# ChicyChen/LOCO-Edit

Measured on AMD Instinct MI355X. Metric: edit-directions/sec (top-5 PMP-Jacobian SVD @256^2) + vT cos-sim vs ref, higher is better.
Workload: dtype bf16x3 (split-bf16 MFMA operands, fp32 accumulate + fp32 storage); 1 GPU; CelebA-HQ DDPM 256x256 top-5 local basis (l_eye-sized mask, L=2400), t=0.6T, 12 power iterations, one GPU; multi_gpu_form=single, probes_total=5, probes_per_gpu=5, kept=5, n_iter=12, mask_L=2400, weights=synthetic seed 0, streams=2

## Files before the change

loco-edit_amd/csrc/conv_bf16.hip:

```cpp
#include "kernels.h"
#include <cstdio>
#include <cstdlib>

namespace loco {

enum : int { PR_BF16X3 = 0, PR_F16 = 1 };
template <int PR, int TAPS, int MODE> void launch_tile_b(const ConvArgs& a, hipStream_t st);
template <int PR, int MODE> void launch_kcat_b(const ConvArgs& a, hipStream_t st);
template <int PR, int MODE> void launch_pair_b(const ConvArgs& a, hipStream_t st);
template <int PR, int MODE> void launch_dual_b(const ConvArgs& a, hipStream_t st);
void launch_conv_gemm(const ConvArgs& a, hipStream_t st);

template <int PR>
static void launch_lowp(const ConvArgs& a, int taps, hipStream_t st) {
#ifdef LOCO_DIAG
    if (a.cot_d && (taps != 1 || a.gemm || a.nsplit > 1 || a.Cin2 > 0 || (a.Cout % conv_bf16_tile_couts(a)) != 0 || a.st_kind == ST_TAN || a.st_kind == ST_COT)) {
        fprintf(stderr, "loco: ConvArgs::cot_d on a launch whose epilogue has no norm-cotangent term (taps %d, gemm %d, nsplit %d, Cout %d, st_kind %d)\n",
                taps, a.gemm, a.nsplit, a.Cout, a.st_kind);
        abort();
    }
#endif
    if constexpr (PR == PR_BF16X3) {
        if (taps == 1 && a.gemm) { launch_conv_gemm(a, st); return; }
    }
    if (taps == 9 && a.Cin2 > 0) {
        if (a.mode == CM_GN_SILU) launch_kcat_b<PR, CM_GN_SILU>(a, st);
        else if (a.mode == CM_GN_GELU) launch_kcat_b<PR, CM_GN_GELU>(a, st);
        else launch_kcat_b<PR, CM_TAN_SILU>(a, st);
        return;
    }
#ifdef LOCO_DIAG
    if constexpr (PR == PR_BF16X3) {
        if (taps == 9 && a.dual) {
            switch (a.mode) {
                case CM_NONE: launch_dual_b<PR, CM_NONE>(a, st); break;
                case CM_GN_SILU: launch_dual_b<PR, CM_GN_SILU>(a, st); break;
                case CM_TAN_SILU: launch_dual_b<PR, CM_TAN_SILU>(a, st); break;
                default: launch_dual_b<PR, CM_COT_SILU>(a, st); break;
            }
            return;
        }
    }
#endif
    if constexpr (PR == PR_BF16X3) {
        if (taps == 9 && a.pair) {
            switch (a.mode) {
                case CM_NONE: launch_pair_b<PR, CM_NONE>(a, st); break;
                case CM_GN_SILU: launch_pair_b<PR, CM_GN_SILU>(a, st); break;
                case CM_TAN_SILU: launch_pair_b<PR, CM_TAN_SILU>(a, st); break;
                default: launch_pair_b<PR, CM_COT_SILU>(a, st); break;
            }
            return;
        }
    }
    if (taps == 9) {
        switch (a.mode) {
            case CM_NONE: launch_tile_b<PR, 9, CM_NONE>(a, st); break;
            case CM_GN_SILU: launch_tile_b<PR, 9, CM_GN_SILU>(a, st); break;
            case CM_GN_GELU: launch_tile_b<PR, 9, CM_GN_GELU>(a, st); break;
            case CM_TAN_SILU: launch_tile_b<PR, 9, CM_TAN_SILU>(a, st); break;
            case CM_COT_SILU: launch_tile_b<PR, 9, CM_COT_SILU>(a, st); break;
            default: launch_tile_b<PR, 9, CM_GN>(a, st); break;
        }
    } else {
        switch (a.mode) {
            case CM_NONE: launch_tile_b<PR, 1, CM_NONE>(a, st); break;
            default: launch_tile_b<PR, 1, CM_GN>(a, st); break;
        }
    }
}
void launch_conv_bf16x3(const ConvArgs& a, int taps, hipStream_t st) { launch_lowp<PR_BF16X3>(a, taps, st); }
void launch_conv_f16(const ConvArgs& a, int taps, hipStream_t st) { launch_lowp<PR_F16>(a, taps, st); }

}
```

loco-edit_amd/csrc/conv_bf16_kernel.h:

```cpp
#pragma once
#include "kernels.h"
#include <cstdlib>
#include <type_traits>

namespace loco {


typedef float f32x16 __attribute__((ext_vector_type(16)));
typedef float f32x4 __attribute__((ext_vector_type(4)));
typedef f32x4 f32x4_u __attribute__((aligned(4)));
typedef float f32x2 __attribute__((ext_vector_type(2)));
typedef f32x2 f32x2_u __attribute__((aligned(4)));
typedef __bf16 bf16x8 __attribute__((ext_vector_type(8)));
typedef _Float16 f16x8 __attribute__((ext_vector_type(8)));
typedef short s16x8 __attribute__((ext_vector_type(8)));

enum : int { PR_BF16X3 = 0, PR_F16 = 1 };

constexpr int BKC = 16;
constexpr bool LIVE_MASK = true;
constexpr bool EARLY_W = true;
constexpr int NDUMMY = 8;

__device__ __forceinline__ float sigmoidf2_(float y) { return __builtin_amdgcn_rcpf(1.0f + __expf(-y)); }

__device__ __forceinline__ int idiv_small(int n, int d) {
    int q = (int)((float)n * __builtin_amdgcn_rcpf((float)d));
    const int r = n - q * d;
    q += (r >= d) ? 1 : ((r < 0) ? -1 : 0);
    return q;
}
__device__ __forceinline__ void idivmod_small(int n, int d, int& q, int& r) { q = idiv_small(n, d); r = n - q * d; }

template <int PR>
__device__ __forceinline__ int rec_off(int p, int q) {
    if constexpr (PR == PR_F16) return p * 32 + ((q ^ ((p >> 3) & 1)) << 4);
    else return p * 64 + ((q ^ ((p >> 2) & 3)) << 4);
}
template <int PR> constexpr int halo_pitch() { return PR == PR_F16 ? 48 : 80; }
template <int PR> constexpr int rec_bytes() { return PR == PR_F16 ? 32 : 64; }
template <int PR>
__device__ __forceinline__ int hrec_off(int p, int q) { return p * halo_pitch<PR>() + (q << 4); }

template <int PR>
__device__ __forceinline__ void cvt2(float a, float b, unsigned& hi, unsigned& lo) {
    if constexpr (PR == PR_F16) {
        _Float16 ha = (_Float16)a, hb = (_Float16)b;
        hi = (unsigned)__builtin_bit_cast(unsigned short, ha) | ((unsigned)__builtin_bit_cast(unsigned short, hb) << 16);
        lo = 0;
    } else {
        typedef float f32x2_ __attribute__((ext_vector_type(2)));
        typedef __bf16 bf16x2_ __attribute__((ext_vector_type(2)));
        hi = __builtin_bit_cast(unsigned, __builtin_convertvector((f32x2_){a, b}, bf16x2_));
        const float ha = __builtin_bit_cast(float, hi << 16), hb = __builtin_bit_cast(float, hi & 0xffff0000u);
        float da = a - ha;
        asm volatile("" : "+v"(da));
        const float db = b - hb;
        lo = __builtin_bit_cast(unsigned, __builtin_convertvector((f32x2_){da, db}, bf16x2_));
    }
}

template <int PR>
__device__ __forceinline__ void split8(const float* v, uint4& hi, uint4& lo) {
    cvt2<PR>(v[0], v[1], hi.x, lo.x);
    cvt2<PR>(v[2], v[3], hi.y, lo.y);
    cvt2<PR>(v[4], v[5], hi.z, lo.z);
    cvt2<PR>(v[6], v[7], hi.w, lo.w);
}

constexpr int max_halo(int NT, int taps, bool s2) {
    if (taps == 1) return NT;
    if (NT >= 128) {
        int th = NT / 32;
        return s2 ? (2 * th + 1) * 65 : (th + 2) * 34;
    }
    return s2 ? 5 * 65 : 4 * 34;
}

constexpr int rs_steps(int n, int lw) { int s = 0; while ((1 << s) < lw && (n >> s) > 1) ++s; return s; }
template <int N, int M, int LW>
__device__ __forceinline__ void rs_reduce(float* av, const int lane) {
    if constexpr (M < LW && N > 1) {
        constexpr int H = N / 2;
        const bool up = (lane & M) != 0;
#pragma unroll
        for (int i = 0; i < H; ++i) {
            const float keep = up ? av[i + H] : av[i];
            const float send = up ? av[i] : av[i + H];
            av[i] = keep + __shfl_xor(send, M, 64);
        }
        rs_reduce<H, M * 2, LW>(av, lane);
    } else if constexpr (M < LW) {
#pragma unroll
        for (int i = 0; i < N; ++i) av[i] += __shfl_xor(av[i], M, 64);
        rs_reduce<N, M * 2, LW>(av, lane);
    }
}

constexpr int EPI_COT1 = 1, EPI_STATS = 2;
template <int WM, int WN, int TM, int TN, int EPI = EPI_STATS, class StageRound>
__device__ __forceinline__ void conv_lowp_epilogue_staged(const ConvArgs& a, StageRound&& stage_round, unsigned char* smem_b, const int co0,
                                                          const int oy0, const int ox0, const int TW, const int tile_id, const int b,
                                                          const int split);
template <int WM, int WN, int TM, int TN>
__device__ __forceinline__ void conv_lowp_epilogue_direct(const ConvArgs& a, f32x16 (&acc)[TM][TN], const int co0, const int oy0,
                                                          const int ox0, const int TW, const int b, const int split);
template <int WM, int WN, int TM, int TN, int EPI = EPI_STATS>
__device__ __forceinline__ void conv_lowp_epilogue(const ConvArgs& a, f32x16 (&acc)[TM][TN], unsigned char* smem_b, const int co0,
                                                   const int oy0, const int ox0, const int TW, const int tile_id, const int b,
                                                   const int split) {
    constexpr int NT = WN * TN * 32;
    const int lane = threadIdx.x & 63, wave = threadIdx.x >> 6;
    const int l31 = lane & 31, khalf = lane >> 5, wm = wave / WN, wn = wave % WN;
    if (co0 + WM * TM * 32 <= a.Cout) {
        conv_lowp_epilogue_staged<WM, WN, TM, TN, EPI>(a, [&](const int h, float* S) {
#pragma unroll
            for (int j = 0; j < TN; ++j)
#pragma unroll
                for (int r = 0; r < 16; ++r)
                    S[(wm * 32 + (r & 3) + 8 * (r >> 2) + 4 * khalf) * NT + (wn * TN + j) * 32 + l31] = acc[h][j][r];
        }, smem_b, co0, oy0, ox0, TW, tile_id, b, split);
        return;
    }
    conv_lowp_epilogue_direct<WM, WN, TM, TN>(a, acc, co0, oy0, ox0, TW, b, split);
}
template <int WM, int WN, int TM, int TN, int EPI, class StageRound>
__device__ __forceinline__ void conv_lowp_epilogue_staged(const ConvArgs& a, StageRound&& stage_round, unsigned char* smem_b, const int co0,
                                                          const int oy0, const int ox0, const int TW, const int tile_id, const int b,
                                                          const int split) {
    constexpr int NTHR = WM * WN * 64;
    constexpr bool COT1 = (EPI & EPI_COT1) != 0, STATS = (EPI & EPI_STATS) != 0;
    constexpr int MT = WM * TM * 32;
    constexpr int NT = WN * TN * 32;
    const int tid = threadIdx.x;
    const int lane = tid & 63;
    const int wave = tid >> 6;
    const int l31 = lane & 31;
    const int khalf = lane >> 5;
    const int wm = wave / WN, wn = wave % WN;
    const long out_plane = (long)a.Hout * a.Wout;
    {
        constexpr int SROWS = WM * 32, NQ = NT / 4, NTASK = (SROWS * NQ) / NTHR;
        static_assert((SROWS * NQ) % NTHR == 0 && (NQ & (NQ - 1)) == 0, "epilogue task split");
        float* const S = reinterpret_cast<float*>(smem_b);
        const bool part = a.nsplit > 1;
        float* const ob = part ? a.partial + (((long)split * a.B + b) * a.Cout) * out_plane : a.out + (long)b * a.out_bs;
        const float* const rb = (!part && a.res) ? a.res + (long)b * a.res_bs : nullptr;
        const float* const b2 = (!part && a.bias2) ? a.bias2 + (long)b * a.bias2_bs : nullptr;
        const float* const b1 = part ? nullptr : a.bias;
        const bool accu = !part && a.accumulate;
        const int twsh = 31 - __builtin_clz((unsigned)TW);
        const bool lin_st = STATS && (a.st_kind == ST_TAN || a.st_kind == ST_COT) && !part;
        const bool lin_cot = a.st_kind == ST_COT;
        const bool cot_ep = COT1 && a.cot_d && !part && !lin_st;
        const float* const cot_db = cot_ep ? a.cot_d + (long)b * a.cot_d_bs : nullptr;
        const f32x2* const cot_tb = cot_ep ? reinterpret_cast<const f32x2*>(a.cot_tc + (long)b * a.cot_tc_bs) : nullptr;
        constexpr int RSTEP = NTHR / NQ;
        static_assert(NTHR % NQ == 0 && 32 % RSTEP == 0, "epilogue task rows");
        const int row0 = tid / NQ, quad0 = tid & (NQ - 1);
        const unsigned pix0 = (unsigned)((oy0 + ((quad0 * 4) >> twsh)) * a.Wout + ox0 + ((quad0 * 4) & (TW - 1)));
        auto co_of = [&](int h, int q) -> int { return co0 + row0 + (((q * RSTEP) >> 5) * TM + h) * 32 + ((q * RSTEP) & 31); };
        auto off_of = [&](int h, int q) -> unsigned {
            const unsigned crow = (unsigned)((((q * RSTEP) >> 5) * TM + h) * 32 + ((q * RSTEP) & 31));
            return (unsigned)(co0 + row0) * (unsigned)out_plane + pix0 + crow * (unsigned)out_plane;
        };
        constexpr int NV = 2 * TM * NTASK;
        float av[STATS ? NV : 1];
#pragma unroll
        for (int h = 0; h < TM; ++h) {
            if (h > 0) {
                asm volatile("s_waitcnt lgkmcnt(0)" ::: "memory");
                __builtin_amdgcn_s_barrier();
            }
            stage_round(h, S);
            f32x4 xs[(STATS || COT1) ? NTASK : 1][2];
            f32x4 cd[COT1 ? NTASK : 1];
            if constexpr (COT1) {
                if (cot_ep) {
#pragma unroll
                    for (int q = 0; q < NTASK; ++q) {
                        const unsigned o = off_of(h, q);
                        cd[q] = *reinterpret_cast<const f32x4*>(cot_db + o);
                        const f32x4* sp4 = reinterpret_cast<const f32x4*>(a.cot_sx + o);
                        xs[q][0] = sp4[0];
                        xs[q][1] = sp4[1];
                    }
                }
            }
            if constexpr (STATS) if (lin_st) {
#pragma unroll
                for (int q = 0; q < NTASK; ++q) {
                    const unsigned o = off_of(h, q);
                    if (lin_cot) {
                        const f32x4* sp4 = reinterpret_cast<const f32x4*>(a.st_sx + o);
                        xs[q][0] = sp4[0];
                        xs[q][1] = sp4[1];
                    } else {
                        xs[q][0] = *reinterpret_cast<const f32x4*>(a.st_x + o);
                    }
                }
            }
            asm volatile("s_waitcnt lgkmcnt(0)" ::: "memory");
            __builtin_amdgcn_s_barrier();
            f32x4 v[NTASK], rv[NTASK];
#pragma unroll
            for (int q = 0; q < NTASK; ++q) v[q] = *reinterpret_cast<const f32x4*>(&S[(q * RSTEP + row0) * NT + quad0 * 4]);
            if (rb || accu) {
#pragma unroll
                for (int q = 0; q < NTASK; ++q) {
                    f32x4 t4 = {0.f, 0.f, 0.f, 0.f};
                    if (rb) t4 = a.res_scale * *reinterpret_cast<const f32x4*>(rb + off_of(h, q));
                    if (accu) t4 += *reinterpret_cast<const f32x4*>(ob + off_of(h, q));
                    rv[q] = t4;
                }
#pragma unroll
                for (int q = 0; q < NTASK; ++q) v[q] += rv[q];
            }
            if constexpr (COT1) {
                if (cot_ep) {
#pragma unroll
                    for (int q = 0; q < NTASK; ++q) {
                        const f32x2 tc2 = cot_tb[co_of(h, q)];
                        const float c1 = tc2[0], c2 = tc2[1];
                        v[q][0] += fmaf(xs[q][0][0], cd[q][0], -fmaf(xs[q][0][1], c2, c1));
                        v[q][1] += fmaf(xs[q][0][2], cd[q][1], -fmaf(xs[q][0][3], c2, c1));
                        v[q][2] += fmaf(xs[q][1][0], cd[q][2], -fmaf(xs[q][1][1], c2, c1));
                        v[q][3] += fmaf(xs[q][1][2], cd[q][3], -fmaf(xs[q][1][3], c2, c1));
                    }
                }
            }
#pragma unroll
            for (int q = 0; q < NTASK; ++q) {
                float add = 0.f;
                if (b1) add += b1[co_of(h, q)];
                if (b2) add += b2[co_of(h, q)];
                v[q] += add;
                __builtin_nontemporal_store(v[q], reinterpret_cast<f32x4*>(ob + off_of(h, q)));
            }
            if constexpr (STATS) if (lin_st) {
#pragma unroll
                for (int q = 0; q < NTASK; ++q) {
                    const f32x4 vv = v[q];
                    float s1, s2;
                    if (!lin_cot) {
                        const f32x4 xv = xs[q][0];
                        s1 = (vv[0] + vv[1]) + (vv[2] + vv[3]);
                        s2 = fmaf(xv[0], vv[0], xv[1] * vv[1]) + fmaf(xv[2], vv[2], xv[3] * vv[3]);
                    } else {
                        const float z0 = xs[q][0][0] * vv[0], z1 = xs[q][0][2] * vv[1], z2 = xs[q][1][0] * vv[2], z3 = xs[q][1][2] * vv[3];
                        s1 = (z0 + z1) + (z2 + z3);
                        s2 = fmaf(xs[q][0][1], z0, xs[q][0][3] * z1) + fmaf(xs[q][1][1], z2, xs[q][1][3] * z3);
                    }
                    av[(h * NTASK + q) * 2] = s1;
                    av[(h * NTASK + q) * 2 + 1] = s2;
                }
            }
            if (STATS && a.st_kind == ST_FWD && !part) {
                const int ntile = (a.Hout * a.Wout) / NT;
                float* const sp = a.st_part + (long)b * a.Cout * ntile * 2;
#pragma unroll
                for (int q = 0; q < NTASK; ++q) {
                    const float pivot = __shfl(v[q][0], lane & ~(NQ - 1) & 63, 64);
                    const float d0 = v[q][0] - pivot, d1 = v[q][1] - pivot, d2 = v[q][2] - pivot, d3 = v[q][3] - pivot;
                    float s1 = (d0 + d1) + (d2 + d3);
                    float s2 = (d0 * d0 + d1 * d1) + (d2 * d2 + d3 * d3);
#pragma unroll
                    for (int m = 1; m < (NQ < 64 ? NQ : 64); m <<= 1) {
                        s1 += __shfl_xor(s1, m, 64);
                        s2 += __shfl_xor(s2, m, 64);
                    }
                    const float m = s1 * (1.0f / NT);
                    const int t = q * NTHR + tid;
                    if ((t & (NQ - 1)) == 0)
                        *reinterpret_cast<f32x2*>(sp + ((long)co_of(h, q) * ntile + tile_id) * 2) = f32x2{pivot + m, s2 - s1 * m};
                }
            }
        }
        if constexpr (STATS) if (lin_st) {
            constexpr int LW = NQ < 64 ? NQ : 64, STEPS = rs_steps(NV, LW), LEFT = NV >> STEPS;
            static_assert((NV & (NV - 1)) == 0, "row sums per lane");
            rs_reduce<NV, 1, LW>(av, lane);
            const int gl = lane & (LW - 1);
            if (gl < (1 << STEPS)) {
                int base = 0;
#pragma unroll
                for (int sb = 0; sb < STEPS; ++sb) base += ((gl >> sb) & 1) * (NV >> (sb + 1));
                const int ntile = (a.Hout * a.Wout) / NT;
                float* const sp = a.st_part + (long)b * a.Cout * ntile * 2;
#pragma unroll
                for (int i = 0; i < LEFT; ++i) {
                    const int idx = base + i, hq = idx >> 1;
                    const int h = hq / NTASK, q = hq - h * NTASK;
                    const int row = (q * NTHR + tid) / NQ;
                    const int co = co0 + ((row >> 5) * TM + h) * 32 + (row & 31);
                    sp[((long)co * ntile + tile_id) * 2 + (idx & 1)] = av[i];
                }
            }
        }
    }
}
template <int WM, int WN, int TM, int TN>
__device__ __forceinline__ void conv_lowp_epilogue_direct(const ConvArgs& a, f32x16 (&acc)[TM][TN], const int co0, const int oy0,
                                                          const int ox0, const int TW, const int b, const int split) {
    const int lane = threadIdx.x & 63, wave = threadIdx.x >> 6;
    const int l31 = lane & 31, khalf = lane >> 5, wm = wave / WN, wn = wave % WN;
    const long out_plane = (long)a.Hout * a.Wout;
    const bool full_co = false;
#pragma unroll
    for (int j = 0; j < TN; ++j) {
        int p = (wn * TN + j) * 32 + l31;
        int ty = p / TW, tx = p - ty * TW;
        int oy = oy0 + ty, ox = ox0 + tx;
        const unsigned pix = (unsigned)(oy * a.Wout + ox);
#pragma unroll
        for (int i = 0; i < TM; ++i) {
            const int cob = co0 + (wm * TM + i) * 32 + 4 * khalf;
            if (a.nsplit > 1) {
                float* pb = a.partial + (((long)split * a.B + b) * a.Cout) * out_plane;
#pragma unroll
                for (int r = 0; r < 16; ++r) {
// ... 55 lines not shown
    const float* const rb = a.res ? a.res + (long)b * a.res_bs : nullptr;
    const float* const b2 = a.bias2 ? a.bias2 + (long)b * a.bias2_bs : nullptr;
    const bool accu = a.accumulate != 0;
    const int twsh = TW == 32 ? 5 : (TW == 16 ? 4 : 3);
    const int ntile = (a.Hout * a.Wout) / NT;
    float* const sp = (a.st_kind == ST_FWD) ? a.st_part + (long)b * a.Cout * ntile * 2 : nullptr;
#pragma unroll
    for (int h = 0; h < TM; ++h) {
#pragma unroll
        for (int g0 = 0; g0 < 4; g0 += NRB) {
#pragma unroll
            for (int j = 0; j < TN; ++j)
#pragma unroll
                for (int g = 0; g < NRB; ++g)
#pragma unroll
                    for (int r3 = 0; r3 < 4; ++r3)
                        S[(wm * RPW + g * 8 + 4 * khalf + r3) * NT + (wn * TN + j) * 32 + l31] = acc[h][j][(g0 + g) * 4 + r3];
            asm volatile("s_waitcnt lgkmcnt(0)" ::: "memory");
            __builtin_amdgcn_s_barrier();
            f32x4 v[NTASK];
            unsigned off[NTASK];
            int cos_[NTASK];
#pragma unroll
            for (int q = 0; q < NTASK; ++q) {
                const int t = q * NTHR + tid;
                const int srow = t / NQ, quad = t & (NQ - 1);
                v[q] = *reinterpret_cast<const f32x4*>(&S[srow * NT + quad * 4]);
                const int co = co0 + ((srow / RPW) * TM + h) * 32 + g0 * 8 + (srow % RPW);
                const int p = quad * 4;
                cos_[q] = co;
                off[q] = (unsigned)co * out_plane + (unsigned)((oy0 + (p >> twsh)) * a.Wout + ox0 + (p & (TW - 1)));
            }
            if (rb || accu) {
                f32x4 rv[NTASK];
#pragma unroll
                for (int q = 0; q < NTASK; ++q) {
                    f32x4 t4 = {0.f, 0.f, 0.f, 0.f};
                    if (rb) t4 = a.res_scale * *reinterpret_cast<const f32x4*>(rb + off[q]);
                    if (accu) t4 += *reinterpret_cast<const f32x4*>(ob + off[q]);
                    rv[q] = t4;
                }
#pragma unroll
                for (int q = 0; q < NTASK; ++q) v[q] += rv[q];
            }
#pragma unroll
            for (int q = 0; q < NTASK; ++q) {
                float add = 0.f;
                if (a.bias) add += a.bias[cos_[q]];
                if (b2) add += b2[cos_[q]];
                v[q] += add;
                __builtin_nontemporal_store(v[q], reinterpret_cast<f32x4*>(ob + off[q]));
            }
            if (sp) {
#pragma unroll
                for (int q = 0; q < NTASK; ++q) {
                    const float pivot = __shfl(v[q][0], 0, 64);
                    const float d0 = v[q][0] - pivot, d1 = v[q][1] - pivot, d2 = v[q][2] - pivot, d3 = v[q][3] - pivot;
                    float s1 = (d0 + d1) + (d2 + d3);
                    float s2 = (d0 * d0 + d1 * d1) + (d2 * d2 + d3 * d3);
#pragma unroll
                    for (int m = 1; m < 64; m <<= 1) {
                        s1 += __shfl_xor(s1, m, 64);
                        s2 += __shfl_xor(s2, m, 64);
                    }
                    const float m = s1 * (1.0f / NT);
                    if (lane == 0)
                        *reinterpret_cast<f32x2*>(sp + ((long)cos_[q] * ntile + tile_id) * 2) = f32x2{pivot + m, s2 - s1 * m};
                }
            }
            asm volatile("s_waitcnt lgkmcnt(0)" ::: "memory");
            __builtin_amdgcn_s_barrier();
        }
    }
}

template <int PR, int TAPS, int WM, int WN, int TM, int TN, int MODE, int STG, int PHASE = 0>
__device__ __forceinline__ void conv_lowp_body(const ConvArgs& a, f32x16 (&acc)[TM][TN]) {
    constexpr int NTHR = WM * WN * 64;
    constexpr int HP = halo_pitch<PR>();
    constexpr int RB = rec_bytes<PR>();
    constexpr int NPC = RB / 16;
    constexpr int MT = WM * TM * 32;
    constexpr int NT = WN * TN * 32;
    constexpr int KS = (TAPS == 9) ? 3 : 1;
    constexpr int NTS = KS;
    constexpr int NROW = (TAPS == 9) ? 3 : 1;
    constexpr bool NEEDP = (MODE == CM_TAN_SILU || MODE == CM_COT_SILU);
    constexpr bool PERS = (PHASE == 3);
    constexpr bool GEN = (STG == 1 || STG == 2);
    constexpr bool COMPACT = (STG == 3);
    constexpr int NITEM = GEN ? (2 * max_halo(NT, TAPS, STG == 2) + NTHR - 1) / NTHR : 1;
    constexpr int WTOT = NTS * MT * NPC;
    constexpr int NWV = (WTOT + NTHR - 1) / NTHR;
    constexpr bool XPF = (TAPS == 9 && STG != 2 && STG != 3);
    constexpr int NWB = XPF ? 3 : 2;
    constexpr bool DEEP1 = (TAPS == 1 && STG == 1 && !NEEDP);
    constexpr int DEEP_D = 4;

    extern __shared__ __attribute__((aligned(16))) unsigned char smem_b[];
#ifdef LOCO_DUAL_STAMP
#define LP_STAMP(i) do { if (threadIdx.x == 0 && PHASE == 0) reinterpret_cast<unsigned long long*>(a.partial)[blockIdx.x * 8 + (i)] = __builtin_amdgcn_s_memtime(); } while (0)
#else
#define LP_STAMP(i) do { } while (0)
#endif
    LP_STAMP(0);
    constexpr int WBYTES = NTS * MT * RB;
    unsigned char* const Wsb = smem_b;
    unsigned char* Hsb;
    unsigned char* Ws = smem_b;
    unsigned char* Hs = smem_b;

    const int tid = threadIdx.x;
    const int lane = tid & 63;
    const int wave = tid >> 6;
    const int l31 = lane & 31;
    const int khalf = lane >> 5;
    const int wm = wave / WN, wn = wave % WN;

    const int S = a.stride;
    const int TW = (TAPS == 1 && PHASE == 0 && a.stride == 1 && !a.upsample && !a.zins && (a.Wout & (a.Wout - 1)) == 0)
                       ? (a.Wout < NT ? a.Wout : NT) : (a.Wout < 32 ? a.Wout : 32);
    const int TH = NT / TW;
    const int tiles_x = a.Wout / TW;
    int tile_id, cot_id, zid;
    {
        const int ntile = (a.Hout * a.Wout) / NT, ncot = (a.Cout + MT - 1) / MT, Z = PERS ? a.pers_groups : a.B * a.nsplit;
        const int NTC = ntile * ncot, L = blockIdx.x;
        int T = 0;
        if ((ntile & 7) == 0) {
            int q = L >> 3, q2, t8;
            idivmod_small(q, ncot, q2, cot_id);
            idivmod_small(q2, Z, t8, zid);
            tile_id = t8 * 8 + (L & 7);
        } else {
            if ((NTC & 7) == 0) { int q = L >> 3, t8; idivmod_small(q, Z, t8, zid); T = t8 * 8 + (L & 7); }
            else idivmod_small(L, Z, T, zid);
            idivmod_small(T, ntile, cot_id, tile_id);
        }
        tile_id = __builtin_amdgcn_readfirstlane(tile_id);
        cot_id = __builtin_amdgcn_readfirstlane(cot_id);
        zid = __builtin_amdgcn_readfirstlane(zid);
    }
    int ty0_, tx0_;
    idivmod_small(tile_id, tiles_x, ty0_, tx0_);
    const int oy0 = __builtin_amdgcn_readfirstlane(ty0_ * TH);
    const int ox0 = __builtin_amdgcn_readfirstlane(tx0_ * TW);
    const int co0 = cot_id * MT;
    int zb_, zs_;
    idivmod_small(zid, a.nsplit, zb_, zs_);
    const int b = PERS ? zid : __builtin_amdgcn_readfirstlane(zb_);
    const int split = PERS ? 0 : __builtin_amdgcn_readfirstlane(zs_);
    const int pstep = PERS ? a.pers_groups : 1;
    const int np = PERS ? (a.B - b + pstep - 1) / pstep : 1;
    int pq = 0;

    if constexpr (XPF && PHASE != 2 && EARLY_W) {
        const int nchunks_ = (a.Cin + BKC - 1) / BKC;
        const int cps_ = __builtin_amdgcn_readfirstlane((nchunks_ + a.nsplit - 1) / a.nsplit);
        const int cbeg_ = split * cps_;
        const int cend_ = (cbeg_ + cps_ < nchunks_) ? cbeg_ + cps_ : nchunks_;
        if (cend_ > cbeg_) {
            typedef __attribute__((address_space(3))) unsigned char lds_u8_;
            typedef const __attribute__((address_space(1))) unsigned char glb_u8_;
            const int wpitch_ = (a.Cout + 31) & ~31;
            const unsigned char* wbase0 = reinterpret_cast<const unsigned char*>(a.wb) +
                                          (unsigned)(cbeg_ * TAPS) * ((unsigned)wpitch_ * (unsigned)RB);
#pragma unroll
            for (int st_ = 0; st_ < 2; ++st_)
#pragma unroll
                for (int i = 0; i < NWV; ++i) {
                    int e = tid + i * NTHR;
                    if (e >= WTOT) e = WTOT - 1;
                    const int tap = e / (MT * NPC), rem = e - tap * (MT * NPC);
                    int rec = co0 + rem / NPC;
                    if (rec >= wpitch_) rec = wpitch_ - 1;
                    const unsigned rel = (unsigned)(((st_ * NTS + tap) * wpitch_ + rec) * NPC + (rem % NPC)) * 16u;
                    const int e0 = wave * 64 + i * NTHR;
                    if ((WTOT % NTHR) == 0 || e0 < WTOT)
                        __builtin_amdgcn_global_load_lds((glb_u8_*)(wbase0 + rel), (lds_u8_*)(smem_b + st_ * WBYTES + e0 * 16), 16, 0, 0);
                }
        }
    }
    const int halo_w = (TW - 1) * S + KS;
    const int halo_h = (TH - 1) * S + KS;
    const int halo_sz = halo_h * halo_w;
    const int HBYTES = COMPACT ? halo_sz * HP + RB : (halo_sz + NDUMMY) * HP;
    Hsb = smem_b + NWB * WBYTES;

    const int LH = (a.upsample || a.zins) ? a.Hin * 2 : a.Hin;
    const int LW = (a.upsample || a.zins) ? a.Win * 2 : a.Win;
    const long in_plane = (long)a.Hin * a.Win;

    int ipos[NITEM], ioct[NITEM];
    unsigned ivoff[NITEM];
    bool ival[NITEM];
#pragma unroll
    for (int i = 0; i < NITEM; ++i) {
        int it = tid + i * NTHR;
        int oct, pos;
        idivmod_small(it, halo_sz, oct, pos);
        int off = -1;
        if (it < 2 * halo_sz) {
            int hy, hx;
            idivmod_small(pos, halo_w, hy, hx);
            int Y = oy0 * S - a.pad + hy, X = ox0 * S - a.pad + hx;
            if (Y >= 0 && Y < LH && X >= 0 && X < LW) {
                if (a.upsample) off = (Y >> 1) * a.Win + (X >> 1);
                else if (a.zins) off = ((Y | X) & 1) ? -1 : (Y >> 1) * a.Win + (X >> 1);
                else off = Y * a.Win + X;
            }
        } else {
            pos = -1; oct = 0;
        }
        ipos[i] = pos; ioct[i] = oct;
        ival[i] = off >= 0;
        ivoff[i] = (unsigned)(oct * 8 * (int)in_plane + (off >= 0 ? off : 0));
    }

    const int nseg = (halo_w + 3) >> 2;
    int v_q4 = 0, v_pos0 = -1, v_voff = 0, v_cnt = 0;
    unsigned v_pm = 0;
    int v_rec[4] = {0, 0, 0, 0};
    unsigned v_goff = 0;
    if constexpr (!GEN) {
        const int per_q = halo_h * nseg;
        const int nsg4 = (nseg + 3) >> 2, nhy2 = (halo_h + 1) >> 1;
        bool have = false;
        int hy = 0, sg = 0;
        if (32 * nsg4 * nhy2 <= NTHR) {
            const int hi = tid >> 5;
            v_q4 = (tid >> 3) & 3;
            int hq_, hr_;
            idivmod_small(hi, nsg4, hq_, hr_);
            sg = hr_ * 4 + (tid & 3);
            hy = hq_ * 2 + ((tid >> 2) & 1);
            have = hi < nsg4 * nhy2 && sg < nseg && hy < halo_h;
            if (!have) v_q4 = 0;
        } else if (tid < 4 * per_q) {
            int rem;
            idivmod_small(tid, per_q, v_q4, rem);
            idivmod_small(rem, nseg, hy, sg);
            have = true;
        }
        if (have) {
            int Y = oy0 - a.pad + hy, X0 = ox0 - a.pad + 4 * sg;
            bool rowok = (Y >= 0 && Y < a.Hin);
            v_pos0 = hy * halo_w + 4 * sg;
            v_cnt = halo_w - 4 * sg < 4 ? halo_w - 4 * sg : 4;
            v_voff = rowok ? Y * a.Win + X0 : 0;
#pragma unroll
            for (int pxi = 0; pxi < 4; ++pxi)
                if (rowok && X0 + pxi >= 0 && X0 + pxi < a.Win && pxi < v_cnt) v_pm |= 1u << pxi;
        }
#pragma unroll
        for (int pxi = 0; pxi < 4; ++pxi)
            v_rec[pxi] = (v_pos0 >= 0 && pxi < v_cnt) ? v_pos0 + pxi : (COMPACT ? halo_sz : halo_sz + (tid & (NDUMMY - 1)));
        v_goff = (unsigned)(((long)v_q4 * 4 * in_plane + v_voff + 16) * 4);
    }

    int hoff[TN];
#pragma unroll
    for (int j = 0; j < TN; ++j) {
        int p = (wn * TN + j) * 32 + l31;
        int ty, tx;
        idivmod_small(p, TW, ty, tx);
        hoff[j] = ty * S * halo_w + tx * S;
    }
    int hbyte[TN];
#pragma unroll
    for (int j = 0; j < TN; ++j) hbyte[j] = hrec_off<PR>(hoff[j], khalf);
    int aoff_hi[TM], aoff_lo[TM];
#pragma unroll
    for (int i = 0; i < TM; ++i) {
        int p = (wm * TM + i) * 32 + l31;
        aoff_hi[i] = rec_off<PR>(p, khalf);
        aoff_lo[i] = PR == PR_F16 ? 0 : rec_off<PR>(p, 2 + khalf);
    }

    if constexpr (PHASE != 2) {
#pragma unroll
        for (int i = 0; i < TM; ++i)
#pragma unroll
            for (int j = 0; j < TN; ++j)
#pragma unroll
                for (int r = 0; r < 16; ++r) acc[i][j][r] = 0.0f;
    }

    const int nchunks = (a.Cin + BKC - 1) / BKC;
    const int cps = __builtin_amdgcn_readfirstlane((nchunks + a.nsplit - 1) / a.nsplit);
    const int cbeg = split * cps;
    const int cend = (cbeg + cps < nchunks) ? cbeg + cps : nchunks;

    const float* inb = a.in + (long)b * a.in_bs;
    const float2* sxb = NEEDP ? a.sx : nullptr;
    const float* scb = (MODE == CM_GN_SILU || MODE == CM_GN || MODE == CM_GN_GELU) ? a.sc + (long)b * a.scsh_bs : nullptr;
    const float* shb = (MODE == CM_GN_SILU || MODE == CM_GN || MODE == CM_GN_GELU) ? a.sh + (long)b * a.scsh_bs : nullptr;
    const int wpitch = (a.Cout + 31) & ~31;
    const uint4* wg = reinterpret_cast<const uint4*>(a.wb);

    float hv[NITEM][8];
    float2 pv[NEEDP ? NITEM : 1][8];
    float cA[(MODE == CM_NONE) ? 1 : 16], cB[(MODE == CM_NONE) ? 1 : 16];
    const float* tcb = NEEDP ? a.tc + (long)b * a.tc_bs : nullptr;

    constexpr int NPART = (!GEN && NROW == 3) ? 2 : 1;
    constexpr int KP = 4 / NPART;
    struct HaloRegs {
        f32x4 dq[GEN ? 1 : KP];
        f32x4 sq[(!GEN && NEEDP) ? KP : 1][2];
        f32x4 cq[(!GEN && MODE != CM_NONE) ? (KP == 4 ? 2 : 1) : 1];
    };
    auto cq_a = [&](const HaloRegs& R, int kk) -> float {
        if constexpr (GEN || MODE == CM_NONE) return 0.f;
        else if constexpr (NEEDP) { if constexpr (KP == 4) return R.cq[kk >> 1][(kk & 1) * 2]; else return R.cq[0][kk * 2]; }
        else return R.cq[0][kk];
    };
    auto cq_b = [&](const HaloRegs& R, int kk) -> float {
        if constexpr (GEN || MODE == CM_NONE) return 0.f;
        else if constexpr (NEEDP) { if constexpr (KP == 4) return R.cq[kk >> 1][(kk & 1) * 2 + 1]; else return R.cq[0][kk * 2 + 1]; }
        else if constexpr (KP == 4) return R.cq[1][kk];
        else return R.cq[0][2 + kk];
    };
    HaloRegs hr;
    bool pf_live = true, dma_live = true;
    int pf_dq = 0;
#ifdef LOCO_DUAL_STAMP
    const bool wi_halo = (a.no_deep & 2) != 0, wi_dma = (a.no_deep & 4) != 0, wi_novalu = (a.no_deep & 8) != 0;
#endif
    auto prefetch_hv = [&](HaloRegs& R, int chunk, int part) {
        const unsigned cb = (unsigned)chunk * ((unsigned)(BKC * 4) * (unsigned)in_plane);
        const long pofs = PERS ? (long)(pq + pf_dq) * pstep : 0;
        const char* pk = reinterpret_cast<const char*>(inb + pofs * a.in_bs - 16) + cb;
        const char* sk = reinterpret_cast<const char*>(reinterpret_cast<const float*>(sxb) - 32) + 2u * cb;
        const unsigned pl = (unsigned)in_plane * 4u;
#pragma unroll
        for (int kk = 0; kk < KP; ++kk) {
#ifdef LOCO_DUAL_STAMP
            const unsigned po = (pf_live && !wi_halo) ? v_goff + (unsigned)(part * KP + kk) * pl : 64u;
#else
            const unsigned po = pf_live ? v_goff + (unsigned)(part * KP + kk) * pl : 64u;
#endif
            R.dq[kk] = *reinterpret_cast<const f32x4_u*>(pk + po);
            if constexpr (NEEDP) {
                R.sq[kk][0] = *reinterpret_cast<const f32x4_u*>(sk + 2u * po);
                R.sq[kk][1] = *reinterpret_cast<const f32x4_u*>(sk + 2u * po + 16);
            }
        }
        const int c0 = chunk * BKC + v_q4 * 4 + part * KP;
        if constexpr (MODE != CM_NONE) {
            if constexpr (NEEDP) {
                const float* tq = tcb + pofs * a.tc_bs;
                R.cq[0] = *reinterpret_cast<const f32x4_u*>(tq + 2 * c0);
                if constexpr (KP == 4) R.cq[1] = *reinterpret_cast<const f32x4_u*>(tq + 2 * c0 + 4);
            } else if constexpr (KP == 4) {
                R.cq[0] = *reinterpret_cast<const f32x4_u*>(scb + pofs * a.scsh_bs + c0);
                R.cq[1] = *reinterpret_cast<const f32x4_u*>(shb + pofs * a.scsh_bs + c0);
            } else {
                const float* sq_ = scb + pofs * a.scsh_bs;
                const float* hq_ = shb + pofs * a.scsh_bs;
                const f32x2 sa = *reinterpret_cast<const f32x2_u*>(sq_ + c0), sb = *reinterpret_cast<const f32x2_u*>(hq_ + c0);
                R.cq[0] = f32x4{sa[0], sa[1], sb[0], sb[1]};
            }
        }
    };
    auto stage_hv = [&](const HaloRegs& R, int part) {
#ifdef LOCO_DUAL_STAMP
        if (wi_novalu) return;
#endif
        const int oct = v_q4 >> 1, half = v_q4 & 1;
#pragma unroll
        for (int pxi = 0; pxi < 4; ++pxi) {
            float r[KP];
#pragma unroll
            for (int kk = 0; kk < KP; ++kk) {
                float d = R.dq[kk][pxi];
                float v = d;
                if constexpr (MODE == CM_GN_SILU) {
                    float y = fmaf(cq_a(R, kk), d, cq_b(R, kk));
                    v = y * sigmoidf2_(y);
                } else if constexpr (MODE == CM_GN_GELU) {
                    v = act_fwd(fmaf(cq_a(R, kk), d, cq_b(R, kk)), ACT_GELU);
                } else if constexpr (MODE == CM_GN) {
                    v = fmaf(cq_a(R, kk), d, cq_b(R, kk));
                } else if constexpr (NEEDP) {
                    const float Sv = R.sq[kk][pxi >> 1][(pxi & 1) * 2], xh = R.sq[kk][pxi >> 1][(pxi & 1) * 2 + 1];
                    if constexpr (MODE == CM_TAN_SILU) v = Sv * fmaf(-xh, cq_b(R, kk), d - cq_a(R, kk));
                    else v = fmaf(-xh, cq_b(R, kk), fmaf(Sv, d, -cq_a(R, kk)));
                }
                r[kk] = ((v_pm >> pxi) & 1u) ? v : 0.0f;
            }
            unsigned char* dst = Hs + hrec_off<PR>(v_rec[pxi], oct) + half * 8 + part * (KP * 2);
            if constexpr (KP == 4) {
                uint2 h, l;
                cvt2<PR>(r[0], r[1], h.x, l.x);
                cvt2<PR>(r[2], r[3], h.y, l.y);
                *reinterpret_cast<uint2*>(dst) = h;
                if constexpr (PR == PR_BF16X3) *reinterpret_cast<uint2*>(dst + 32) = l;
            } else {
                unsigned h, l;
                cvt2<PR>(r[0], r[1], h, l);
                *reinterpret_cast<unsigned*>(dst) = h;
                if constexpr (PR == PR_BF16X3) *reinterpret_cast<unsigned*>(dst + 32) = l;
            }
        }
    };
    auto load_consts = [&](int chunk) {
        const int c0 = chunk * BKC;
        if constexpr (MODE != CM_NONE) {
#pragma unroll
            for (int kk = 0; kk < 16; ++kk) {
                int c = c0 + kk < a.Cin ? c0 + kk : a.Cin - 1;
                if constexpr (NEEDP) { cA[kk] = tcb[2 * c]; cB[kk] = tcb[2 * c + 1]; }
                else { cA[kk] = scb[c]; cB[kk] = shb[c]; }
            }
        }
    };
    auto load_regs = [&](float (&hvd)[NITEM][8], int chunk) {
        const int c0 = chunk * BKC;
        if (c0 + BKC <= a.Cin) {
            if constexpr (TAPS == 9 && !NEEDP) {
                const unsigned lm = pf_live ? 0xffffffffu : 0u;
                const long pb4 = in_plane * 4;
                const unsigned char* pk = reinterpret_cast<const unsigned char*>(inb) + (long)c0 * pb4;
#pragma unroll
                for (int k = 0; k < 8; ++k) {
#pragma unroll
                    for (int i = 0; i < NITEM; ++i) hvd[i][k] = *reinterpret_cast<const float*>(pk + ((ivoff[i] * 4u) & lm));
                    pk += pb4;
                }
            } else {
#pragma unroll
            for (int k = 0; k < 8; ++k) {
                const float* pk = inb + (long)(c0 + k) * in_plane;
                const float2* sk = NEEDP ? sxb + (long)(c0 + k) * in_plane : nullptr;
#pragma unroll
                for (int i = 0; i < NITEM; ++i) {
                    hvd[i][k] = pk[pf_live ? ivoff[i] : 0u];
                    if constexpr (NEEDP) pv[i][k] = sk[pf_live ? ivoff[i] : 0u];
                }
            }
            }
        } else {
#pragma unroll
            for (int i = 0; i < NITEM; ++i) {
#pragma unroll
                for (int k = 0; k < 8; ++k) {
                    int c = c0 + ioct[i] * 8 + k;
                    int cc = c < a.Cin ? c : a.Cin - 1;
                    unsigned vo = ivoff[i] - (unsigned)(ioct[i] * 8 * (int)in_plane);
                    float v = inb[(long)cc * in_plane + vo];
                    hvd[i][k] = c < a.Cin ? v : 0.0f;
                    if constexpr (NEEDP) {
                        float2 pp = sxb[(long)cc * in_plane + vo];
                        pv[i][k] = c < a.Cin ? pp : make_float2(0.f, 0.f);
                    }
                }
            }
        }
    };
    auto prefetch_h = [&](int chunk, int part) {
        if constexpr (!GEN) { prefetch_hv(hr, chunk, part); return; }
        load_consts(chunk);
        load_regs(hv, chunk);
    };
    unsigned wrel[NWV];
#pragma unroll
    for (int i = 0; i < NWV; ++i) {
        int e = tid + i * NTHR;
        if (e >= WTOT) e = WTOT - 1;
        int tap = e / (MT * NPC), rem = e - tap * (MT * NPC);
        int rec = co0 + rem / NPC;
        if (rec >= wpitch) rec = wpitch - 1;
        wrel[i] = (unsigned)((tap * wpitch + rec) * NPC + (rem % NPC)) * 16u;
    }
    typedef __attribute__((address_space(3))) unsigned char lds_u8;
    typedef const __attribute__((address_space(1))) unsigned char glb_u8;
    auto dma_w = [&](int chunk, int row, unsigned char* Wdst) {
        const unsigned char* wbase = reinterpret_cast<const unsigned char*>(wg) +
                                     (unsigned)(chunk * TAPS + row * NTS) * ((unsigned)wpitch * (unsigned)RB);
#pragma unroll
        for (int i = 0; i < NWV; ++i) {
            const int e0 = (wave * 64 + i * NTHR);
            if ((WTOT % NTHR) == 0 || e0 < WTOT)
#ifdef LOCO_DUAL_STAMP
                __builtin_amdgcn_global_load_lds((glb_u8*)(wbase + ((dma_live && !wi_dma) ? wrel[i] : 0u)), (lds_u8*)(Wdst + e0 * 16), 16, 0, 0);
#else
                __builtin_amdgcn_global_load_lds((glb_u8*)(wbase + (dma_live ? wrel[i] : 0u)), (lds_u8*)(Wdst + e0 * 16), 16, 0, 0);
#endif
        }
    };
    auto stage_regs = [&](const float (&hvs)[NITEM][8], int chunk, unsigned char* Hd, auto whole_tag) {
        constexpr bool WHOLE = decltype(whole_tag)::value;
        const int c0 = chunk * BKC;
#pragma unroll
        for (int i = 0; i < NITEM; ++i) {
            if (ipos[i] < 0) continue;
            float v[8];
#pragma unroll
            for (int k = 0; k < 8; ++k) {
                int c = c0 + ioct[i] * 8 + k;
                float r = 0.0f;
                if (ival[i] && (WHOLE || c < a.Cin)) {
                    float d = hvs[i][k];
                    if constexpr (MODE == CM_NONE) {
                        r = d;
                    } else {
                        const float ca = ioct[i] ? cA[8 + k] : cA[k];
                        const float cb = ioct[i] ? cB[8 + k] : cB[k];
                        if constexpr (MODE == CM_GN_SILU) {
                            float y = fmaf(ca, d, cb);
                            r = y * sigmoidf2_(y);
                        } else if constexpr (MODE == CM_GN_GELU) {
                            r = act_fwd(fmaf(ca, d, cb), ACT_GELU);
                        } else if constexpr (MODE == CM_GN) {
                            r = fmaf(ca, d, cb);
                        } else {
                            float Sv = pv[i][k].x, xh = pv[i][k].y;
                            if constexpr (MODE == CM_TAN_SILU) r = Sv * fmaf(-xh, cb, d - ca);
                            else r = fmaf(-xh, cb, fmaf(Sv, d, -ca));
                        }
                    }
                }
                v[k] = r;
            }
            uint4 hi, lo;
            split8<PR>(v, hi, lo);
            *reinterpret_cast<uint4*>(Hd + hrec_off<PR>(ipos[i], ioct[i])) = hi;
            if constexpr (PR == PR_BF16X3) *reinterpret_cast<uint4*>(Hd + hrec_off<PR>(ipos[i], 2 + ioct[i])) = lo;
        }
    };
    auto stage_h = [&](int chunk, int part) {
        if constexpr (!GEN) { stage_hv(hr, part); return; }
        stage_regs(hv, chunk, Hs, std::false_type{});
    };

    constexpr int NLO = PR == PR_BF16X3 ? 1 : 0;
    struct Frag { s16x8 ah[TM], al[NLO ? TM : 1], bh[TN], bl[NLO ? TN : 1]; };
    auto load_frag = [&](Frag& f, int row, int tp) {
        const int tapoff = (TAPS == 9) ? row * halo_w + tp : 0;
#pragma unroll
        for (int i = 0; i < TM; ++i) {
            f.ah[i] = *reinterpret_cast<const s16x8*>(Ws + tp * MT * RB + aoff_hi[i]);
#if defined(LOCO_WI_NOLO)
            if constexpr (NLO) f.al[i] = f.ah[i];
#else
            if constexpr (NLO) f.al[i] = *reinterpret_cast<const s16x8*>(Ws + tp * MT * RB + aoff_lo[i]);
#endif
        }
#pragma unroll
        for (int j = 0; j < TN; ++j) {
            const unsigned char* hp = Hs + tapoff * HP + hbyte[j];
            f.bh[j] = *reinterpret_cast<const s16x8*>(hp);
#if defined(LOCO_WI_NOLO)
            if constexpr (NLO) f.bl[j] = f.bh[j];
#else
            if constexpr (NLO) f.bl[j] = *reinterpret_cast<const s16x8*>(hp + 32);
#endif
        }
    };
    auto mma_frag = [&](const Frag& f) {
#pragma unroll
        for (int i = 0; i < TM; ++i)
#pragma unroll
            for (int j = 0; j < TN; ++j) {
                if constexpr (PR == PR_F16) {
                    acc[i][j] = __builtin_amdgcn_mfma_f32_32x32x16_f16(__builtin_bit_cast(f16x8, f.ah[i]),
                                                                       __builtin_bit_cast(f16x8, f.bh[j]), acc[i][j], 0, 0, 0);
                } else {
                    const bf16x8 ah = __builtin_bit_cast(bf16x8, f.ah[i]), al = __builtin_bit_cast(bf16x8, f.al[i]);
                    const bf16x8 bh = __builtin_bit_cast(bf16x8, f.bh[j]), bl = __builtin_bit_cast(bf16x8, f.bl[j]);
                    acc[i][j] = __builtin_amdgcn_mfma_f32_32x32x16_bf16(al, bh, acc[i][j], 0, 0, 0);
                    acc[i][j] = __builtin_amdgcn_mfma_f32_32x32x16_bf16(ah, bl, acc[i][j], 0, 0, 0);
                    acc[i][j] = __builtin_amdgcn_mfma_f32_32x32x16_bf16(ah, bh, acc[i][j], 0, 0, 0);
                }
            }
    };

    auto mma_one = [&](const Frag& f, int i, int j) {
        if constexpr (PR == PR_F16) {
            acc[i][j] = __builtin_amdgcn_mfma_f32_32x32x16_f16(__builtin_bit_cast(f16x8, f.ah[i]),
                                                               __builtin_bit_cast(f16x8, f.bh[j]), acc[i][j], 0, 0, 0);
        } else {
            const bf16x8 ah = __builtin_bit_cast(bf16x8, f.ah[i]), al = __builtin_bit_cast(bf16x8, f.al[i]);
            const bf16x8 bh = __builtin_bit_cast(bf16x8, f.bh[j]), bl = __builtin_bit_cast(bf16x8, f.bl[j]);
#if defined(LOCO_WI_MFMA16)
            {
                f32x4 q0 = {acc[i][j][0], acc[i][j][1], acc[i][j][2], acc[i][j][3]}, q1 = {acc[i][j][4], acc[i][j][5], acc[i][j][6], acc[i][j][7]};
                f32x4 q2 = {acc[i][j][8], acc[i][j][9], acc[i][j][10], acc[i][j][11]}, q3 = {acc[i][j][12], acc[i][j][13], acc[i][j][14], acc[i][j][15]};
                q0 = __builtin_amdgcn_mfma_f32_16x16x32_bf16(al, bh, q0, 0, 0, 0);
                q1 = __builtin_amdgcn_mfma_f32_16x16x32_bf16(al, bh, q1, 0, 0, 0);
                q2 = __builtin_amdgcn_mfma_f32_16x16x32_bf16(ah, bl, q2, 0, 0, 0);
                q3 = __builtin_amdgcn_mfma_f32_16x16x32_bf16(ah, bl, q3, 0, 0, 0);
                q0 = __builtin_amdgcn_mfma_f32_16x16x32_bf16(ah, bh, q0, 0, 0, 0);
                q1 = __builtin_amdgcn_mfma_f32_16x16x32_bf16(ah, bh, q1, 0, 0, 0);
#pragma unroll
                for (int r = 0; r < 4; ++r) { acc[i][j][r] = q0[r]; acc[i][j][4 + r] = q1[r]; acc[i][j][8 + r] = q2[r]; acc[i][j][12 + r] = q3[r]; }
                return;
            }
#elif defined(LOCO_WI_2MFMA)
            acc[i][j] = __builtin_amdgcn_mfma_f32_32x32x16_bf16(ah, bl, acc[i][j], 0, 0, 0);
            acc[i][j] = __builtin_amdgcn_mfma_f32_32x32x16_bf16(ah, bh, acc[i][j], 0, 0, 0);
            (void)al;
            return;
#endif
            acc[i][j] = __builtin_amdgcn_mfma_f32_32x32x16_bf16(al, bh, acc[i][j], 0, 0, 0);
            acc[i][j] = __builtin_amdgcn_mfma_f32_32x32x16_bf16(ah, bl, acc[i][j], 0, 0, 0);
            acc[i][j] = __builtin_amdgcn_mfma_f32_32x32x16_bf16(ah, bh, acc[i][j], 0, 0, 0);
        }
    };
    auto mma_frag_head = [&](const Frag& f) { mma_one(f, 0, 0); };
    auto mma_frag_tail = [&](const Frag& f) {
#pragma unroll
        for (int i = 0; i < TM; ++i)
#pragma unroll
            for (int j = 0; j < TN; ++j)
                if (i + j > 0) mma_one(f, i, j);
    };

    const int nch = cend - cbeg;
    const int clast = cend - 1;
    auto cclamp = [&](int c) { return __builtin_amdgcn_readfirstlane(c < clast ? c : clast); };
    auto vres = [&](int x) -> int {
// ... 149 lines not shown
                for (int i = 0; i < NITEM; ++i) hvr[sl][i][k] = *reinterpret_cast<const float*>(pk + (ivoffb[i] & lm));
                pk += plane_bytes;
            }
            const unsigned char* wbase = wgb + (unsigned)(chunk * TAPS) * ((unsigned)wpitch * (unsigned)RB);
#pragma unroll
            for (int i = 0; i < NWV; ++i) wr[sl][i] = *reinterpret_cast<const f32x4*>(wbase + (wrel[i] & lm));
        };
        auto commit = [&](auto stag, int chunk, unsigned char* Hd, unsigned char* Wd) {
            constexpr int sl = decltype(stag)::value;
            if constexpr (MODE != CM_NONE) load_consts(chunk);
            stage_regs(hvr[sl], chunk, Hd, std::true_type{});
#pragma unroll
            for (int i = 0; i < NWV; ++i)
                if ((WTOT % NTHR) == 0 || tid + i * NTHR < WTOT)
                    *reinterpret_cast<f32x4*>(Wd + (tid + i * NTHR) * 16) = wr[sl][i];
        };
        using S0 = std::integral_constant<int, 0>; using S1 = std::integral_constant<int, 1>;
        using S2 = std::integral_constant<int, 2>; using S3 = std::integral_constant<int, 3>;
        static_assert(D == 4, "ring slots are spelled out below");
        if (nch > 0) {
            issue(S0{}, cbeg);
            issue(S1{}, cbeg + 1);
            issue(S2{}, cbeg + 2);
            issue(S3{}, cbeg + 3);
            commit(S0{}, cbeg, Hsb, Wsb);
            issue(S0{}, cbeg + 4);
            stage_end();
        }
        auto body = [&](auto stag, const int ci) {
            const int chunk = cbeg + ci;
            unsigned char* const Wcur = Wsb + (ci & 1) * WBYTES;
            unsigned char* const Wnxt = Wsb + ((ci + 1) & 1) * WBYTES;
            unsigned char* const Hcur = Hsb + (ci & 1) * HBYTES;
            unsigned char* const Hnxt = Hsb + ((ci + 1) & 1) * HBYTES;
            Ws = Wcur; Hs = Hcur;
            Frag f0;
            load_frag(f0, 0, 0);
            __builtin_amdgcn_sched_barrier(0);
            mma_frag(f0);
            commit(stag, cclamp(chunk + 1), Hnxt, Wnxt);
            issue(stag, chunk + 1 + D);
            stage_end();
        };
        int ci = 0;
        for (; ci + D <= nch; ci += D) {
            body(S1{}, ci); body(S2{}, ci + 1); body(S3{}, ci + 2); body(S0{}, ci + 3);
        }
        if (ci < nch) body(S1{}, ci);
        if (ci + 1 < nch) body(S2{}, ci + 1);
        if (ci + 2 < nch) body(S3{}, ci + 2);
      }
    }
    if (!deep_done) {
    if (nch > 0) {
        dma_w(cbeg, 0, Wsb);
        Hs = Hsb;
        if constexpr (!GEN && NPART == 2) {
            HaloRegs hr2;
            prefetch_hv(hr, cbeg, 0);
            prefetch_hv(hr2, cbeg, 1);
            stage_hv(hr, 0);
            stage_hv(hr2, 1);
        } else {
#pragma unroll
            for (int part = 0; part < NPART; ++part) {
                prefetch_h(cbeg, part);
                stage_h(cbeg, part);
            }
        }
        asm volatile("s_waitcnt vmcnt(0)" ::: "memory");
        if (NROW == 1 || NPART == 2) prefetch_h(cclamp(cbeg + 1), 0);
        stage_end();
    }
    for (int ci = 0; ci < nch; ++ci) {
        const int chunk = cbeg + ci;
#pragma unroll
        for (int row = 0; row < NROW; ++row) {
            const int s_ = ci * NROW + row;
            unsigned char* const Wcur = Wsb + (s_ & 1) * WBYTES;
            unsigned char* const Wnxt = Wsb + ((s_ + 1) & 1) * WBYTES;
            unsigned char* const Hcur = Hsb + (ci & 1) * HBYTES;
            unsigned char* const Hnxt = Hsb + ((ci + 1) & 1) * HBYTES;
            constexpr bool one = (NROW == 1);
            const int st_part = one ? 0 : (NPART == 2 ? (row == 0 ? 0 : row == 1 ? 1 : -1) : (row == 2 ? 0 : -1));
            const int ld_part = one ? 0 : (NPART == 2 ? (row == 0 ? 1 : row == 1 ? 0 : -1) : (row == 0 ? 0 : -1));
            const int ld_chunk = one ? chunk + 2 : ((NPART == 2 && row == 1) ? chunk + 2 : chunk + 1);
            constexpr bool MIDLOAD = !GEN;
            constexpr int NLD = KP + (NEEDP ? 2 * KP + 1 : (MODE != CM_NONE ? 2 : 0));
            {
                const int r1 = (row + 1) % NROW, dc = (row + 1) / NROW;
                dma_live = LIVE_MASK ? (chunk + dc <= clast) : true;
                dma_w(cclamp(chunk + dc), r1, Wnxt);
                dma_live = true;
            }
            Ws = Wcur; Hs = Hcur;
            Frag f0, f1;
            load_frag(f0, row, 0);
            if (NTS > 1) load_frag(f1, row, 1);
            __builtin_amdgcn_sched_barrier(0);
            mma_frag(f0);
            __builtin_amdgcn_sched_barrier(0);
            if (NTS > 2) load_frag(f0, row, 2);
            __builtin_amdgcn_sched_barrier(0);
            if (NTS > 1) mma_frag(f1);
            if (st_part >= 0) { Hs = Hnxt; stage_h(cclamp(chunk + 1), st_part); Hs = Hcur; }
            if (MIDLOAD && ld_part >= 0) { pf_live = LIVE_MASK ? (ld_chunk <= clast) : true; prefetch_h(cclamp(ld_chunk), ld_part); pf_live = true; }
            if (NTS > 2) mma_frag(f0);
            __builtin_amdgcn_sched_barrier(0);
            if (MIDLOAD && ld_part >= 0) {
                asm volatile("s_waitcnt vmcnt(%0)" :: "n"(NLD) : "memory");
            } else {
                asm volatile("s_waitcnt vmcnt(0)" ::: "memory");
                if (!MIDLOAD && ld_part >= 0) { pf_live = LIVE_MASK ? (ld_chunk <= clast) : true; prefetch_h(cclamp(ld_chunk), ld_part); pf_live = true; }
            }
            stage_end();
        }
    }
    }

    }

    if constexpr (PHASE == 1) {
        asm volatile("s_waitcnt lgkmcnt(0)" ::: "memory");
        __builtin_amdgcn_s_barrier();
        return;
    }
    LP_STAMP(3);
    conv_lowp_epilogue<WM, WN, TM, TN, (TAPS == 1 && PHASE == 0) ? (EPI_COT1 | EPI_STATS) : EPI_STATS>(a, acc, smem_b, co0, oy0, ox0, TW, tile_id, b, split);
    LP_STAMP(4);
#undef LP_STAMP
}

constexpr int lowp_min_waves(int taps, int nthr, int stg) { return (stg == 3 || (taps == 1 && nthr <= 256)) ? 2 : 1; }
template <int TAPS, int WM, int WN, int TM, int TN, int MODE, int STG>
__global__ __launch_bounds__(WM * WN * 64, lowp_min_waves(TAPS, WM * WN * 64, STG)) void conv_mfma_bf16x3(ConvArgs a) {
    f32x16 acc[TM][TN];
    conv_lowp_body<PR_BF16X3, TAPS, WM, WN, TM, TN, MODE, STG>(a, acc);
}
template <int TAPS, int WM, int WN, int TM, int TN, int MODE, int STG>
__global__ __launch_bounds__(WM * WN * 64, lowp_min_waves(TAPS, WM * WN * 64, STG)) void conv_mfma_f16(ConvArgs a) {
    f32x16 acc[TM][TN];
    conv_lowp_body<PR_F16, TAPS, WM, WN, TM, TN, MODE, STG>(a, acc);
}

#ifdef LOCO_DIAG
template <int TAPS, int WM, int WN, int TM, int TN, int MODE, int STG>
__global__ __launch_bounds__(WM * WN * 64, 1) void conv_pers_bf16x3(ConvArgs a) {
    f32x16 acc[TM][TN];
    conv_lowp_body<PR_BF16X3, TAPS, WM, WN, TM, TN, MODE, STG, 3>(a, acc);
}
#endif

template <int PR, int WM, int WN, int TM, int TN, int MODE>
__device__ __forceinline__ void conv_lowp_kcat(const ConvArgs& a) {
    f32x16 acc[TM][TN];
    conv_lowp_body<PR, 9, WM, WN, TM, TN, MODE, 0, 1>(a, acc);
    ConvArgs a2 = a;
    a2.in = a.in2; a2.in_bs = a.in2_bs; a2.Cin = a.Cin2; a2.wb = a.wb2; a2.mode = CM_NONE; a2.pad = 0; a2.in_padded = a.in2_padded;
    conv_lowp_body<PR, 1, WM, WN, TM, TN, CM_NONE, 1, 2>(a2, acc);
}
template <int WM, int WN, int TM, int TN, int MODE>
__global__ __launch_bounds__(WM * WN * 64) void conv_kcat_bf16x3(ConvArgs a) { conv_lowp_kcat<PR_BF16X3, WM, WN, TM, TN, MODE>(a); }
template <int WM, int WN, int TM, int TN, int MODE>
__global__ __launch_bounds__(WM * WN * 64) void conv_kcat_f16(ConvArgs a) { conv_lowp_kcat<PR_F16, WM, WN, TM, TN, MODE>(a); }

template <int PR, int TAPS, int WM, int WN, int TM, int TN, int MODE, int STG>
static void launch_one_b2(const ConvArgs& a, hipStream_t st) {
    constexpr int MT = WM * TM * 32, NT = WN * TN * 32;
    constexpr int KS = (TAPS == 9) ? 3 : 1;
    int TW = a.Wout < 32 ? a.Wout : 32;
    int TH = NT / TW;
    int halo_w = (TW - 1) * a.stride + KS, halo_h = (TH - 1) * a.stride + KS;
    const int nwb = (TAPS == 9 && STG != 2 && STG != 3) ? 3 : 2;
    size_t lds = (size_t)nwb * KS * MT * rec_bytes<PR>() + 2 * ((size_t)halo_w * halo_h + NDUMMY) * halo_pitch<PR>();
    if (STG == 3) lds = (size_t)nwb * KS * MT * rec_bytes<PR>() + 2 * ((size_t)halo_w * halo_h * halo_pitch<PR>() + rec_bytes<PR>());
    const size_t stage_bytes = (size_t)WM * 32 * NT * 4;
    if (lds < stage_bytes) lds = stage_bytes;
    dim3 grid(((a.Hout * a.Wout) / NT) * ((a.Cout + MT - 1) / MT) * a.B * a.nsplit);
#ifdef LOCO_DIAG
    if constexpr (PR == PR_BF16X3 && TAPS == 9 && STG == 0 && WM == 2 && WN == 4 && TM == 2 && TN == 2) {
        if (a.pers_groups > 0) {
            auto pk = &conv_pers_bf16x3<TAPS, WM, WN, TM, TN, MODE, STG>;
            static DeviceOnce ponce;
            if (first_on_device(ponce))
                (void)hipFuncSetAttribute(reinterpret_cast<const void*>(pk), hipFuncAttributeMaxDynamicSharedMemorySize, 160 * 1024);
            const size_t plds = (size_t)nwb * KS * MT * rec_bytes<PR>() + 2 * ((size_t)halo_w * halo_h + NDUMMY) * halo_pitch<PR>() +
                                (size_t)WM * 16 * NT * 4;
            dim3 pgrid(((a.Hout * a.Wout) / NT) * ((a.Cout + MT - 1) / MT) * a.pers_groups);
            hipLaunchKernelGGL(pk, pgrid, dim3(WM * WN * 64), plds, st, a);
            return;
        }
    }
#endif
    void (*kern)(ConvArgs);
    if constexpr (PR == PR_F16) kern = &conv_mfma_f16<TAPS, WM, WN, TM, TN, MODE, STG>;
    else kern = &conv_mfma_bf16x3<TAPS, WM, WN, TM, TN, MODE, STG>;
    if (lds > 64 * 1024) {
        static DeviceOnce once;
        if (first_on_device(once)) {
            (void)hipFuncSetAttribute(reinterpret_cast<const void*>(kern), hipFuncAttributeMaxDynamicSharedMemorySize,
                                      160 * 1024);
        }
    }
    hipLaunchKernelGGL(kern, grid, dim3(WM * WN * 64), lds, st, a);
}

template <int PR, int TAPS, int WM, int WN, int TM, int TN, int MODE>
static void launch_one_b(const ConvArgs& a, hipStream_t st) {
    const bool general = a.stride != 1 || a.upsample || a.zins || (a.Cin % BKC) != 0 || !a.in_padded;
    if constexpr (MODE == CM_NONE) {
        if (a.stride == 2) launch_one_b2<PR, TAPS, WM, WN, TM, TN, MODE, 2>(a, st);
        else if (TAPS == 9 && !general) launch_one_b2<PR, TAPS, WM, WN, TM, TN, MODE, 0>(a, st);
        else launch_one_b2<PR, TAPS, WM, WN, TM, TN, MODE, 1>(a, st);
        return;
    }
    if constexpr (MODE == CM_GN_SILU || MODE == CM_TAN_SILU || MODE == CM_GN_GELU) {
        if (general) { launch_one_b2<PR, TAPS, WM, WN, TM, TN, MODE, 1>(a, st); return; }
    }
    launch_one_b2<PR, TAPS, WM, WN, TM, TN, MODE, 0>(a, st);
}


template <int PR, int MODE>
void launch_kcat_b(const ConvArgs& a, hipStream_t st) {
    constexpr int WM = 2, WN = 4, TM = 2, TN = 2, MT = 128, NT = 256;
    const int TW = a.Wout < 32 ? a.Wout : 32, TH = NT / TW;
    size_t lds = (size_t)3 * 3 * MT * rec_bytes<PR>() + 2 * ((size_t)(TW + 2) * (TH + 2) + NDUMMY) * halo_pitch<PR>();
    dim3 grid(((a.Hout * a.Wout) / NT) * ((a.Cout + MT - 1) / MT) * a.B * a.nsplit);
    void (*kern)(ConvArgs);
    if constexpr (PR == PR_F16) kern = &conv_kcat_f16<WM, WN, TM, TN, MODE>;
    else kern = &conv_kcat_bf16x3<WM, WN, TM, TN, MODE>;
    static DeviceOnce once;
    if (first_on_device(once))
        (void)hipFuncSetAttribute(reinterpret_cast<const void*>(kern), hipFuncAttributeMaxDynamicSharedMemorySize, 160 * 1024);
    hipLaunchKernelGGL(kern, grid, dim3(WM * WN * 64), lds, st, a);
}

template <int PR, int TAPS, int MODE>
void launch_tile_b(const ConvArgs& a, hipStream_t st) {
    switch (a.tile) {
        case 5:
            launch_one_b<PR, TAPS, 2, 4, 2, 2, MODE>(a, st);
            break;
#ifdef LOCO_DIAG
        case 6:
            if constexpr (TAPS == 9) { launch_one_b2<PR, TAPS, 2, 2, 2, 2, MODE, 3>(a, st); break; }
            launch_one_b<PR, TAPS, 2, 2, 2, 2, MODE>(a, st);
            break;
#endif
        case 0: launch_one_b<PR, TAPS, 2, 2, 2, 2, MODE>(a, st); break;
        case 1: launch_one_b<PR, TAPS, 4, 1, 1, 2, MODE>(a, st); break;
        case 2: launch_one_b<PR, TAPS, 1, 4, 1, 1, MODE>(a, st); break;
        default: launch_one_b<PR, TAPS, 2, 2, 1, 1, MODE>(a, st); break;
    }
}


}
```

loco-edit_amd/csrc/conv_plan.hip:

```cpp
#include "kernels.h"
#include <cstdio>
#include <cstdlib>

namespace loco {

constexpr int BKC = 16;
constexpr int BKF = 8;

static const int kMT[7] = {128, 128, 32, 64, 128, 128, 128}, kNT[7] = {128, 64, 128, 64, 256, 256, 128};

static int env_int(const char* name, int dflt) {
    const char* e = getenv(name);
    return e ? atoi(e) : dflt;
}
static int diag_switch(const char* name) {
#ifdef LOCO_DIAG
    return env_int(name, 0);
#else
    (void)name;
    return 0;
#endif
}

static int pick_tile(int Cout, int HW) {
// ... 70 lines not shown

static bool conv_pair_ok(const ConvArgs& a) {
    static const bool on = env_int("LOCO_CONV_PAIR", 1) != 0;
    if (!on || a.Hout * a.Wout < 16384 || a.taps != 9 || a.Cin2 > 0 || a.nsplit != 1 || a.stride != 1 || a.upsample || a.zins ||
        a.pad != 1 || !a.in_padded || (a.Cin % (2 * BKC)) != 0 || (a.Cout % 128) != 0 || (a.Wout % 32) != 0 || (a.Hout % 8) != 0 ||
        a.pers_groups || a.dual)
        return false;
    if (!(a.mode == CM_NONE || a.mode == CM_GN_SILU || a.mode == CM_TAN_SILU || a.mode == CM_COT_SILU)) return false;
    return a.tile == 5;
}

static bool conv_dual_ok(const ConvArgs& a) {
    static const bool on = diag_switch("LOCO_CONV_DUAL") != 0;
    if (!on || a.taps != 9 || a.Cin2 > 0 || a.nsplit != 1 || a.stride != 1 || a.upsample || a.zins || a.pad != 1 || (a.Cin % BKC) != 0 ||
        !a.in_padded || a.Wout < 32 || (a.Wout % 32) != 0 || (a.Hout % 8) != 0 || (a.Cout % 128) != 0 || a.B < 2 || a.cot_d)
        return false;
    if (!(a.mode == CM_NONE || a.mode == CM_GN_SILU || a.mode == CM_TAN_SILU || a.mode == CM_COT_SILU)) return false;
    if (a.tile != 5) return false;
    const long units = (long)((a.Hout * a.Wout) / 256) * (a.Cout / 128) * (a.B / 2);
    return units >= 192;
}

static ConvArgs conv_shift_batch(const ConvArgs& a, int nb) {
    ConvArgs t = a;
    t.B = a.B - nb;
    t.in += (long)nb * a.in_bs; t.out += (long)nb * a.out_bs;
    if (t.prim) t.prim += (long)nb * a.prim_bs;
    if (t.bias2) t.bias2 += (long)nb * a.bias2_bs;
    if (t.res) t.res += (long)nb * a.res_bs;
    if (t.sc) { t.sc += (long)nb * a.scsh_bs; t.sh += (long)nb * a.scsh_bs; }
    if (t.mr) t.mr += (long)nb * a.mr_bs;
    if (t.tst) t.tst += (long)nb * a.tst_bs;
    if (t.tc) t.tc += (long)nb * a.tc_bs;
    if (t.in2) t.in2 += (long)nb * a.in2_bs;
    if (t.cot_d) { t.cot_d += (long)nb * a.cot_d_bs; t.cot_tc += (long)nb * a.cot_tc_bs; }
    if (t.st_part) t.st_part += (long)nb * a.Cout * ((a.Hout * a.Wout) / conv_bf16_tile_pixels(a)) * 2;
    return t;
}

static void conv_pers_plan(ConvArgs& a) {
    a.pers_groups = 0;
    static const int on = diag_switch("LOCO_CONV_PERS");
    if (!on || a.taps != 9 || a.Cin2 > 0 || a.nsplit != 1 || a.stride != 1 || a.upsample || a.zins || a.pad != 1 || !a.in_padded ||
        (a.Cin % (2 * BKC)) != 0 || (a.Cout % 128) != 0 || a.B < 2 || a.cot_d || bf16_tile_of(a) != 5)
        return;
    if (!(a.mode == CM_NONE || a.mode == CM_GN_SILU || a.mode == CM_GN_GELU ||
          (on == 2 && (a.mode == CM_TAN_SILU || a.mode == CM_COT_SILU)))) return;
    const long wg0 = (long)((a.Hout * a.Wout) / 256) * (a.Cout / 128);
    int G = wg0 >= 256 ? 1 : (int)(256 / wg0);
    if (G > a.B) G = a.B;
    const int per = (a.B + G - 1) / G;
    if (per < 2 || a.B * 10 < G * per * 8 || wg0 * G < 192) return;
    a.pers_groups = G;
}

static void conv_gemm_plan(ConvArgs& a) {
    static const bool on = env_int("LOCO_CONV_GEMM", 1) != 0;
    a.gemm = 0;
    const long HW = (long)a.Hout * a.Wout;
    if (!on || a.stride != 1 || a.upsample || a.zins || (a.Cin % BKC) != 0 || a.Cin < 320 || (HW % 256) != 0 || (a.Wout % 16) != 0 ||
        a.Cout < 128 || !a.partial || a.Cin2 > 0 || !(a.mode == CM_NONE || a.mode == CM_GN) || a.cot_d)
        return;
    {
        const int TW = a.Wout < 32 ? a.Wout : 32;
        if ((256 % TW) != 0 || (a.Wout % TW) != 0 || (a.Hout % (256 / TW)) != 0) return;
    }
    static const int all_shapes = env_int("LOCO_GEMM_ALL", 0);
    if (!all_shapes && !(a.Cout >= 640 && (a.Cout >= 4 * a.Cin || a.Cin >= 2560))) return;
    const int pad256 = (a.Cout + 255) / 256 * 256;
    const int tm = (pad256 * 10 <= a.Cout * 11) ? 4 : 2;
    const int mt = 64 * tm;
    const long tiles = (HW / 256) * ((a.Cout + mt - 1) / mt) * a.B;
    const size_t rec_floats = (size_t)a.B * a.Cin * HW;
    int ns = 1;
    if (tiles < 192) {
        const int nchunks = a.Cin / BKC;
        ns = (int)((256 + tiles - 1) / tiles);
        if (ns > 8) ns = 8;
        while (ns > 1 && nchunks / ns < 8) --ns;
        while (ns > 1 && (size_t)ns * a.B * a.Cout * HW + rec_floats > a.partial_floats) --ns;
    }
    if ((ns > 1 ? (size_t)ns * a.B * a.Cout * HW : 0) + rec_floats > a.partial_floats) return;
    a.gemm = 1; a.gemm_tm = tm; a.nsplit = ns;
}

void conv_plan_family(ConvArgs& a, int prec) {
    if (prec == 1 && a.taps == 1) conv_gemm_plan(a);
    if (prec == 1 && a.taps == 9) conv_pers_plan(a);
}

int conv_plan_parts(ConvArgs& a, int prec, int tile_override, ConvArgs parts[2]) {
    a.dual = 0;
    a.tile = tile_for(a, prec, tile_override);
    a.pair = 0;
    parts[0] = a;
    int n = 1;
    if (prec == 1 && a.taps == 9 && conv_dual_ok(a)) {
        parts[0].B = a.B & ~1;
        parts[0].dual = 1;
        if (a.B & 1) {
            parts[1] = conv_shift_batch(a, a.B - 1);
            parts[1].pers_groups = 0;
            n = 2;
        }
    }
    for (int i = 0; i < n; ++i) {
        ConvArgs& p = parts[i];
        p.tile = tile_for(p, prec, tile_override);
        p.pair = prec == 1 && conv_pair_ok(p);
    }
    return n;
}

static bool short_tail(long per_probe, int B) {
    const long total = per_probe * B, r = total % 256;
    return total > 256 && r > 0 && r <= 160;
}

static int tail_split(const ConvArgs& a, size_t partial_floats, int* split) {
    const long per_probe = (long)((a.Hout * a.Wout) / conv_bf16_tile_pixels(a)) * ((a.Cout + 127) / 128);
    const long r = per_probe * a.B % 256;
    if (!short_tail(per_probe, a.B) || per_probe <= 0 || r % per_probe != 0 || r / per_probe >= a.B) return 0;
    int s = (int)(256 / r);
    if (s > 4) s = 4;
    const int nchunks = (a.Cin + 15) / 16;
    while (s > 1 && nchunks / s < 4) --s;
    const size_t one = (size_t)(r / per_probe) * a.Cout * a.Hout * a.Wout;
    while (s > 1 && (size_t)s * one > partial_floats) --s;
    *split = s;
    return s > 1 ? (int)(r / per_probe) : 0;
}

static int stats_route(const ConvEnv& e, const StatAsk* q, bool want, ConvArgs& x, int s0, int B, int* keep_ntile) {
    if (!q || q->kind == ST_NONE) return SR_NONE;
    const int alone = q->norm ? SR_ALONE : SR_NONE;
    if (!want) return alone;
    if (x.nsplit > 1) return !q->norm ? SR_NONE : ((x.Hout * x.Wout) % 4 == 0 ? SR_SPLITK : SR_ALONE);
    const int ntile = (x.Hout * x.Wout) / conv_bf16_tile_pixels(x);
    const size_t need = (size_t)x.B * x.Cout * ntile * 2;
    const int epi = q->norm ? SR_EPI : SR_KEEP;
    const bool kept = q->keep && s0 == 0 && x.B == B && need <= q->keep_floats;
    if (q->kind == ST_FWD && conv_lowp_can_fuse_stats(x) && (kept || (q->norm && need <= e.stpart_floats))) {
        x.st_part = kept ? q->keep : e.stpart; x.st_kind = ST_FWD;
        if (kept) *keep_ntile = ntile;
        return epi;
    }
    const bool cot_cache = q->kind == ST_COT && q->norm && q->sx;
    if ((q->kind == ST_TAN || cot_cache) && e.fuse_lin && !x.cot_d && conv_lowp_can_fuse_stats(x) && !x.pers_groups &&
        !conv_dual_ok(x)) {
        const size_t lane_off = (size_t)e.lane_s0 * (q->keep_floats / e.max_batch);
        const bool keptl = q->kind == ST_TAN && q->keep && s0 == 0 && x.B == B && lane_off + need <= q->keep_floats;
        if (keptl || (q->norm && need <= e.stpart_floats)) {
            x.st_part = keptl ? q->keep + lane_off : e.stpart; x.st_kind = q->kind; x.st_x = q->prim;
            if (q->kind == ST_COT) x.st_sx = q->sx;
            if (keptl) *keep_ntile = ntile;
            return epi;
        }
    }
    return alone;
}

static ConvLaunch plan_launch(const ConvEnv& e, const StatAsk* q, bool want, const ConvArgs& x, int s0, int B, int* keep_ntile) {
    ConvLaunch l;
    l.args = x;
    l.s0 = s0;
    l.args.tile = tile_for(x, e.prec, -1);
    l.stats = stats_route(e, q, want, l.args, s0, B, keep_ntile);
    if (l.stats == SR_EPI || l.stats == SR_KEEP) l.ntile = (x.Hout * x.Wout) / conv_bf16_tile_pixels(l.args);
    l.nparts = conv_plan_parts(l.args, e.prec, -1, l.parts);
    return l;
}

ConvPlan plan_conv(const ConvEnv& e, const ConvArgs& a0, int taps, const StatAsk* q, const ConvArgs* sc) {
    ConvPlan p;
    ConvArgs a = a0;
    a.taps = taps;
    a.dual = 0; a.pers_groups = 0; a.gemm = 0;
    if (sc) {
        ConvArgs t = a;
        t.nsplit = e.prec >= 1 ? conv_bf16_pick_nsplit(a.Cin, a.Cout, a.Hout, a.Wout, a.B, e.chip_share, 9, e.lanes) : 2;
        t.in2 = sc->in; t.in2_bs = sc->in_bs; t.Cin2 = sc->Cin;
        const long per_probe = (long)((a.Hout * a.Wout) / 256) * ((a.Cout + 127) / 128);
        if (e.prec >= 1 && taps == 9 && !short_tail(per_probe, a.B) && !a.bias2 && conv_lowp_can_kcat(t)) {
            a.in2 = sc->in; a.in2_bs = sc->in_bs; a.Cin2 = sc->Cin; a.in2_padded = sc->in_padded;
            a.wb2 = e.prec == 2 ? sc->wh : sc->wb;
            a.bias2 = sc->bias; a.bias2_bs = 0;
            a.res = nullptr;
        } else {
            p.sc_first = true;
            a.res = sc->out; a.res_bs = sc->out_bs;
        }
    }
    if (e.prec == 2) a.wb = a.wh;
    a.no_deep = e.deep1 ? 0 : 1;
    a.nsplit = e.prec >= 1 ? conv_bf16_pick_nsplit(a.Cin, a.Cout, a.Hout, a.Wout, a.B, e.chip_share, taps, e.lanes)
                           : conv_pick_nsplit(a.Cin, a.Cout, a.Hout, a.Wout, a.B);
    if (a.cot_d) {
        ConvArgs t = a;
        t.tile = bf16_tile_of(t);
        const long per_probe = (long)((a.Hout * a.Wout) / conv_bf16_tile_pixels(t)) * ((a.Cout + 127) / 128);
        p.cot = e.prec >= 1 && taps == 1 && a.nsplit == 1 && !short_tail(per_probe, a.B) && conv_lowp_can_fuse_stats(t);
        if (!p.cot) { a.cot_d = nullptr; a.cot_d_bs = 0; a.cot_sx = nullptr; a.cot_tc = nullptr; a.cot_tc_bs = 0; }
    }
    while (a.nsplit > 1 && (size_t)a.nsplit * a.B * a.Cout * a.Hout * a.Wout > e.partial_floats) a.nsplit >>= 1;
    if (a.nsplit < 1) a.nsplit = 1;
    a.partial = e.partial;
    a.partial_floats = e.partial_floats;
    conv_plan_family(a, e.prec);
    a.tile = tile_for(a, e.prec, -1);
    int split = 1;
    const int tail = e.prec >= 1 && a.nsplit == 1 && a.B >= 2 && !a.gemm && !a.pers_groups ? tail_split(a, e.partial_floats, &split) : 0;
    const bool want = q && q->kind != ST_NONE && e.prec >= 1 && e.fuse_stats;
    if (!tail) {
        p.l[0] = plan_launch(e, q, want, a, 0, a.B, &p.keep_ntile);
        return p;
    }
    const bool per_part = want && q->norm && (q->kind == ST_FWD || (e.fuse_lin && (a.Hout * a.Wout) % 4 == 0));
    p.stats_all = !per_part && q && q->kind != ST_NONE && q->norm;
    const StatAsk* ql = per_part ? q : nullptr;
    const int nb = a.B - tail;
    ConvArgs m = a, t = conv_shift_batch(a, nb);
    m.B = nb;
    t.nsplit = split;
    p.nl = 2;
    p.l[0] = plan_launch(e, ql, want, m, 0, a.B, &p.keep_ntile);
    p.l[1] = plan_launch(e, ql, want, t, nb, a.B, &p.keep_ntile);
    return p;
}

const char* conv_variant_name(const ConvArgs& a, int taps, int prec) {
    static const char* tiles[6] = {"2,2,2,2", "4,1,1,2", "1,4,1,1", "2,2,1,1", "2,2,2,4", "2,4,2,2"};
    static char names[3][2][6][6][56];
    static char others[5][3][6][40];
    const int mode = (a.mode < 0 || a.mode > 5) ? 2 : a.mode;
    const char* other = nullptr;
    int k = 0, v = mode;
    if (prec && taps == 9 && a.Cin2 > 0) other = prec == 1 ? "conv_kcat_bf16x3<2,4,2,2,%d>" : "conv_kcat_f16<2,4,2,2,%d>";
    else if (prec == 1 && taps == 1 && a.gemm) { k = 1; other = "conv_gemm_bf16x3<%d>"; v = a.gemm_tm; }
    else if (prec == 1 && taps == 9 && a.pers_groups > 0 && !a.dual) { k = 2; other = "conv_pers_bf16x3<9,2,4,2,2,%d>"; }
    else if (prec == 1 && taps == 9 && a.pair) { k = 3; other = "conv_pair_bf16x3<%d>"; }
    else if (prec == 1 && taps == 9 && a.dual) { k = 4; other = "conv_dual_bf16x3<%d>"; }
    if (other) {
        char* n = others[k][prec][v];
        if (!n[0]) snprintf(n, 40, other, v);
        return n;
    }
    int t = a.tile == 6 ? 0 : a.tile;
    if (t < 0 || t > 5) t = 0;
    int m = mode;
    if (taps != 9 && m != CM_NONE) m = CM_GN;
    if (!prec && m == CM_GN_GELU) m = CM_GN_SILU;
    char* n = names[prec][taps == 9 ? 0 : 1][t][m];
    static const char* kn[3] = {"conv_mfma_f32", "conv_mfma_bf16x3", "conv_mfma_f16"};
    if (!n[0]) snprintf(n, 56, "%s<%d,%s,%d>", kn[prec], taps, tiles[t], m);
    return n;
}

}
```

loco-edit_amd/csrc/engine.hip:

```cpp
#include <hip/hip_runtime.h>

#include <algorithm>
#include <array>
#include <cmath>
#include <cstdio>
#include <cstdlib>
#include <cstring>
#include <map>
#include <memory>
#include <thread>
#include <atomic>
#include <string>
#include <vector>

#include "../../include/loco_hip.h"
#ifdef LOCO_DIAG
#include "../../include/loco_hip_diag.h"
#endif
#include "kernels.h"
#include "program.h"
#ifdef LOCO_DIAG
#include "conv_plan_text.h"
#endif

using namespace loco;


#define HIPCHK(ctx, call)                                                                    \
    do {                                                                                     \
        hipError_t e_ = (call);                                                              \
        if (e_ != hipSuccess) {                                                              \
            (ctx)->err = std::string(#call) + ": " + hipGetErrorString(e_);                  \
            return -1;                                                                       \
        }                                                                                    \
    } while (0)

namespace {

struct ConvP {
    float* wf = nullptr;
    float* wd = nullptr;
    float* wbf = nullptr;
    float* wbd = nullptr;
    float* whf = nullptr;
    float* whd = nullptr;
    float* bias = nullptr;
    int cin = 0, cout = 0, taps = 0;
};
struct NormW { float* gamma = nullptr; float* beta = nullptr; };

struct OpWeights {
    ConvP c1, c2, nin, qkvc, proj, conv;
    ConvP xqc, xproj;
    ConvP pj_in, to_out1, to_out2, ff1, ff2, pj_out;
    NormW g1, g2, gx;
    float *xkw = nullptr, *xkb = nullptr, *xvw = nullptr, *xvb = nullptr;
    float *xng = nullptr, *xnb = nullptr;
    float *lng[3] = {nullptr, nullptr, nullptr}, *lnb[3] = {nullptr, nullptr, nullptr};
    long tproj_off = 0;
};
struct Weights {
    std::vector<OpWeights> op;
    float *freq = nullptr, *td0w = nullptr, *td0b = nullptr, *td1w = nullptr, *td1b = nullptr;
    float* tcw = nullptr;
    float *tp_w = nullptr, *tp_b = nullptr;
    long tproj_total = 0;
    double flops = 0.0;
};

struct Tens : TensPlan {
    float* keep = nullptr; size_t keep_floats = 0; int keep_ntile = 0;
};
struct NormP : NormPlan, NormW {
    bool ready = false;
};
struct Op : OpPlan, OpWeights {
    NormP n1, n2, nx;
    float *xK = nullptr, *xV = nullptr;
};

struct HostParam { std::vector<float> data; std::vector<int64_t> shape; bool loaded = false; };

}


struct loco_ctx {
    loco_unet_cfg cfg;
    std::string err;
    std::map<std::string, HostParam> params;
    bool finalized = false;

    std::shared_ptr<const Program> prog;
    std::shared_ptr<Weights> wts;
    std::vector<Tens> tens;
    std::vector<Op> ops;


    float *arenaP = nullptr, *arenaT = nullptr;
    float *statsP = nullptr, *statsT = nullptr;
    double* red = nullptr;
    bool fuse_cot = true;
    float *stpart = nullptr, *stpart2 = nullptr;
    size_t stpart_floats = 0;
    bool fuse_stats = true;
    bool fuse_xattn = true;
    bool deep1 = true;
    bool flash_attn = true;
    float* attn_delta = nullptr;
    float* partial = nullptr;
    size_t partial_floats = 0;
    const float* bench_out = nullptr; int64_t bench_out_count = 0;
#ifdef LOCO_DIAG
    std::string* plan_log = nullptr;
#endif
    float *tact = nullptr, *tproj = nullptr;
    float* eps_buf = nullptr;
    float* gx0 = nullptr;
    float* ge = nullptr;
    float* tmpA = nullptr;
    double *G = nullptr, *Q = nullptr, *W = nullptr, *gscratch = nullptr;
    float* alphas = nullptr;
    float* ctx_colbias = nullptr;
    bool has_ctx = false;
    float* cond_add = nullptr;
    float* ctx_norm = nullptr;
    bool has_cond = false;
    float* cond_in = nullptr;
    bool has_tcond = false;
// ... 58 lines not shown
    *p = reinterpret_cast<T*>(q);
    c->owned.push_back(reinterpret_cast<float*>(q));
    c->bytes += count * sizeof(T);
    return 0;
}

inline float eps_of(const loco_ctx* c, const NormP& n) { return n.eps > 0.f ? n.eps : c->cfg.gn_eps; }


int upload(loco_ctx* c, float** dst, const std::vector<float>& h) {
    if (dalloc(c, dst, h.size() ? h.size() : 1)) return -1;
    HIPCHK(c, hipMemcpy(*dst, h.data(), h.size() * sizeof(float), hipMemcpyHostToDevice));
    return 0;
}

static inline uint16_t f2bf(float f) {
    uint32_t u; std::memcpy(&u, &f, 4);
    u += 0x7FFFu + ((u >> 16) & 1u);
    return (uint16_t)(u >> 16);
}
static inline float bf2f(uint16_t h) {
    uint32_t u = (uint32_t)h << 16; float f; std::memcpy(&f, &u, 4); return f;
}
template <typename F>
static void parallel_for(int n, size_t work, F fn) {
    unsigned nt = std::thread::hardware_concurrency();
    if (nt > 16) nt = 16;
    if ((int)nt > n) nt = (unsigned)n;
    if (nt <= 1 || work < ((size_t)1 << 18)) { for (int i = 0; i < n; ++i) fn(i); return; }
    std::atomic<int> next{0};
    std::vector<std::thread> th;
    for (unsigned t = 0; t < nt; ++t)
        th.emplace_back([&]() { int i; while ((i = next.fetch_add(1)) < n) fn(i); });
    for (auto& t : th) t.join();
}

template <typename F>
static std::vector<float> build_records(int nin, int nout, int taps, F get) {
    int nch = (nin + 15) / 16, noutP = (nout + 31) & ~31;
    std::vector<uint16_t> rec((size_t)nch * taps * noutP * 32, 0);
    parallel_for(nch, (size_t)nin * nout * taps, [&](int ck) {
        for (int t = 0; t < taps; ++t)
            for (int o = 0; o < nout; ++o) {
                uint16_t* r = rec.data() + (((size_t)ck * taps + t) * noutP + o) * 32;
                int sw = (o >> 2) & 3;
                for (int k = 0; k < 16; ++k) {
                    int i = ck * 16 + k;
                    float v = (i < nin) ? get(o, i, t) : 0.f;
                    uint16_t h = f2bf(v);
                    uint16_t l = f2bf(v - bf2f(h));
                    int qh = (k >> 3) ^ sw, ql = (2 + (k >> 3)) ^ sw;
                    r[qh * 8 + (k & 7)] = h;
                    r[ql * 8 + (k & 7)] = l;
                }
            }
    });
    std::vector<float> out(rec.size() / 2);
    std::memcpy(out.data(), rec.data(), rec.size() * 2);
    return out;
}

template <typename F>
static std::vector<float> build_records_f16(int nin, int nout, int taps, F get) {
    int nch = (nin + 15) / 16, noutP = (nout + 31) & ~31;
    std::vector<_Float16> rec((size_t)nch * taps * noutP * 16, (_Float16)0.f);
    parallel_for(nch, (size_t)nin * nout * taps, [&](int ck) {
        for (int t = 0; t < taps; ++t)
            for (int o = 0; o < nout; ++o) {
                _Float16* r = rec.data() + (((size_t)ck * taps + t) * noutP + o) * 16;
                int sw = (o >> 3) & 1;
                for (int k = 0; k < 16; ++k) {
                    int i = ck * 16 + k;
                    float v = (i < nin) ? get(o, i, t) : 0.f;
                    r[((k >> 3) ^ sw) * 8 + (k & 7)] = (_Float16)v;
                }
            }
    });
    std::vector<float> out(rec.size() / 2);
    std::memcpy(out.data(), rec.data(), rec.size() * 2);
    return out;
}

int make_conv(loco_ctx* c, const std::vector<const HostParam*>& ws, const std::vector<const HostParam*>& bs,
              ConvP* out, int row_limit = -1) {
    int cin = (int)ws[0]->shape[1], k = ws[0]->shape.size() > 2 ? (int)ws[0]->shape[2] : 1;
    int taps = ws[0]->shape.size() == 4 ? k * k : k;
    int cout = 0;
    for (auto* w : ws) cout += (int)w->shape[0];
    if (row_limit > 0 && ws.size() == 1 && row_limit < cout) cout = row_limit;
    int coutP = (cout + 31) & ~31, cinP = (cin + 31) & ~31;
    std::vector<float> wf((size_t)cin * taps * coutP, 0.f), wd((size_t)cout * taps * cinP, 0.f), bias(cout);
    int co0 = 0;
    for (size_t wi = 0; wi < ws.size(); ++wi) {
        const HostParam* w = ws[wi];
        int co_n = (int)w->shape[0];
        if (co_n > cout - co0) co_n = cout - co0;
        parallel_for(co_n, (size_t)co_n * cin * taps, [&](int co) {
            for (int ci = 0; ci < cin; ++ci)
                for (int t = 0; t < taps; ++t)
                    wd[((size_t)(co0 + co) * taps + (taps - 1 - t)) * cinP + ci] = w->data[((size_t)co * cin + ci) * taps + t];
        });
        parallel_for(cin, (size_t)co_n * cin * taps, [&](int ci) {
            for (int t = 0; t < taps; ++t)
                for (int co = 0; co < co_n; ++co)
                    wf[((size_t)ci * taps + t) * coutP + co0 + co] = w->data[((size_t)co * cin + ci) * taps + t];
        });
        for (int co = 0; co < co_n; ++co) bias[co0 + co] = bs[wi]->data[co];
        co0 += co_n;
    }
    out->cin = cin; out->cout = cout; out->taps = taps;
    if (upload(c, &out->wf, wf) || upload(c, &out->wd, wd) || upload(c, &out->bias, bias)) return -1;
    auto fwd = [&](int o, int i, int t) { return wf[((size_t)i * taps + t) * coutP + o]; };
    auto dgr = [&](int o, int i, int t) { return wd[((size_t)i * taps + t) * cinP + o]; };
    std::vector<float> rf = build_records(cin, cout, taps, fwd);
    std::vector<float> rd = build_records(cout, cin, taps, dgr);
    if (upload(c, &out->wbf, rf) || upload(c, &out->wbd, rd)) return -1;
    std::vector<float> hf = build_records_f16(cin, cout, taps, fwd);
    std::vector<float> hd = build_records_f16(cout, cin, taps, dgr);
    if (upload(c, &out->whf, hf) || upload(c, &out->whd, hd)) return -1;
    return 0;
}
int make_conv1(loco_ctx* c, const std::string& name, ConvP* out, int row_limit = -1) {
    return make_conv(c, {&c->params[name + ".weight"]}, {&c->params[name + ".bias"]}, out, row_limit);
}
int make_conv1_scaled(loco_ctx* c, const std::string& name, ConvP* out, float s) {
    if (s == 1.f) return make_conv1(c, name, out);
    HostParam w = c->params[name + ".weight"], b = c->params[name + ".bias"];
    for (float& v : w.data) v *= s;
    for (float& v : b.data) v *= s;
    return make_conv(c, {&w}, {&b}, out);
}
int make_norm(loco_ctx* c, const std::string& name, NormW* n) {
    if (upload(c, &n->gamma, c->params[name + ".weight"].data)) return -1;
    if (upload(c, &n->beta, c->params[name + ".bias"].data)) return -1;
    return 0;
}

int bind_weights(loco_ctx* c) {
    const Weights& W = *c->wts;
    for (size_t i = 0; i < c->ops.size(); ++i) {
        Op& v = c->ops[i];
        static_cast<OpWeights&>(v) = W.op[i];
        static_cast<NormW&>(v.n1) = v.g1; static_cast<NormW&>(v.n2) = v.g2; static_cast<NormW&>(v.nx) = v.gx;
    }
    if (dalloc(c, &c->tact, (size_t)c->cfg.ch * 4) || dalloc(c, &c->tproj, (size_t)(W.tproj_total > 0 ? W.tproj_total : 1))) return -1;
    c->finalized = true;
    return 0;
}

int finalize_params(loco_ctx* c) {
    if (c->finalized) return 0;
    for (const ParamDecl& d : c->prog->params)
        if (!c->params[d.name].loaded) { c->err = "parameter not loaded: " + d.name; return -1; }
    Weights& W = *c->wts;
    const loco_unet_cfg& cfg = c->cfg;
    int temb_ch = cfg.ch * 4;
    const bool adm = cfg.arch == 1;
    const std::string te0 = adm ? "time_embed.0" : "temb.dense.0", te1 = adm ? "time_embed.2" : "temb.dense.1";
    if (cfg.arch < 2) {
        if (upload(c, &W.td0w, c->params[te0 + ".weight"].data)) return -1;
        if (upload(c, &W.td0b, c->params[te0 + ".bias"].data)) return -1;
        if (upload(c, &W.td1w, c->params[te1 + ".weight"].data)) return -1;
        if (upload(c, &W.td1b, c->params[te1 + ".bias"].data)) return -1;
        if (cfg.time_cond_proj_dim > 0 && upload(c, &W.tcw, c->params["time_embed.cond_proj.weight"].data)) return -1;
    }
    {
        int half = cfg.ch / 2;
        std::vector<float> f(half);
        for (int i = 0; i < half; ++i) {
            float x;
            if (adm) x = ((float)(-std::log(10000.0)) * (float)i) / (float)half;
            else x = (float)i * (float)(-(std::log(10000.0) / (double)(half - 1)));
            f[i] = (float)std::exp((double)x);
        }
        if (upload(c, &W.freq, f)) return -1;
    }
    std::vector<float> tpw, tpb;
    for (size_t oi = 0; oi < W.op.size(); ++oi) {
        const OpPlan& op = c->prog->ops[oi];
        OpWeights& ow = W.op[oi];
        switch (op.kind) {
            case OP_CONV_IN: case OP_CONV: if (make_conv1(c, op.pn_conv, &ow.conv)) return -1; break;
            case OP_RES: {
                if (make_norm(c, op.pn_n1, &ow.g1) || make_norm(c, op.pn_n2, &ow.g2)) return -1;
                if (make_conv1(c, op.pn_c1, &ow.c1) || make_conv1_scaled(c, op.pn_c2, &ow.c2, c->prog->res_scale)) return -1;
                if (op.has_nin && make_conv1_scaled(c, op.pn_skip, &ow.nin, c->prog->res_scale)) return -1;
                if (!op.has_temb) break;
                ow.tproj_off = (long)tpb.size();
                auto& w = c->params[op.pn_emb + ".weight"].data;
                auto& b = c->params[op.pn_emb + ".bias"].data;
                tpw.insert(tpw.end(), w.begin(), w.end());
                tpb.insert(tpb.end(), b.begin(), b.end());
                break;
            }
            case OP_ATTN: {
                if (make_norm(c, op.pn_n1, &ow.g1)) return -1;
                if (adm) {
                    if (make_conv1(c, op.pn_qkv, &ow.qkvc)) return -1;
                } else if (make_conv(c, {&c->params[op.name + ".q.weight"], &c->params[op.name + ".k.weight"],
                                         &c->params[op.name + ".v.weight"]},
                                     {&c->params[op.name + ".q.bias"], &c->params[op.name + ".k.bias"],
                                      &c->params[op.name + ".v.bias"]}, &ow.qkvc)) return -1;
                if (make_conv1(c, op.pn_proj, &ow.proj)) return -1;
                if (op.added_kv) {
                    const int C = c->tens[op.in].C, NH = op.heads, CH = C / NH, D = c->cfg.context_dim;
                    const HostParam& w = c->params[op.name + ".encoder_kv.weight"];
                    const HostParam& b = c->params[op.name + ".encoder_kv.bias"];
                    std::vector<float> kw((size_t)C * D), vw((size_t)C * D), kb(C), vb(C);
                    for (int h = 0; h < NH; ++h)
                        for (int i = 0; i < CH; ++i) {
                            const size_t rk = (size_t)h * 2 * CH + i, rv = rk + CH, r = (size_t)h * CH + i;
                            std::copy(w.data.begin() + rk * D, w.data.begin() + (rk + 1) * D, kw.begin() + r * D);
                            std::copy(w.data.begin() + rv * D, w.data.begin() + (rv + 1) * D, vw.begin() + r * D);
                            kb[r] = b.data[rk]; vb[r] = b.data[rv];
                        }
                    if (upload(c, &ow.xkw, kw) || upload(c, &ow.xkb, kb) || upload(c, &ow.xvw, vw) || upload(c, &ow.xvb, vb) ||
                        upload(c, &ow.xng, c->params[op.name + ".norm_encoder.weight"].data) ||
                        upload(c, &ow.xnb, c->params[op.name + ".norm_encoder.bias"].data)) return -1;
                }
                if (op.has_x) {
                    const std::string x = op.name + ".xattn";
                    if (make_norm(c, x + ".norm", &ow.gx) || make_conv1(c, x + ".q", &ow.xqc) ||
                        make_conv1(c, x + ".proj_out", &ow.xproj)) return -1;
                    if (upload(c, &ow.xkw, c->params[x + ".k.weight"].data) || upload(c, &ow.xkb, c->params[x + ".k.bias"].data) ||
                        upload(c, &ow.xvw, c->params[x + ".v.weight"].data) || upload(c, &ow.xvb, c->params[x + ".v.bias"].data))
                        return -1;
                }
                break;
            }
            case OP_DOWN: case OP_UP: if (make_conv1(c, op.pn_conv, &ow.conv)) return -1; break;
            case OP_XFMR: {
                const int C = c->tens[op.in].C, NH = op.heads, CH = C / NH;
                const std::string b = op.name + ".transformer_blocks.0";
                HostParam zb; zb.shape = {8 * C}; zb.data.assign((size_t)8 * C, 0.f);
                auto nobias = [&](const std::string& w, ConvP* out) { return make_conv(c, {&c->params[w + ".weight"]}, {&zb}, out); };
                if (make_norm(c, op.pn_n1, &ow.g1) || make_conv1(c, op.name + ".proj_in", &ow.pj_in) ||
                    make_conv1(c, op.name + ".proj_out", &ow.pj_out)) return -1;
                const char* lnn[3] = {".norm1", ".norm2", ".norm3"};
                for (int i = 0; i < 3; ++i)
                    if (upload(c, &ow.lng[i], c->params[b + lnn[i] + ".weight"].data) ||
                        upload(c, &ow.lnb[i], c->params[b + lnn[i] + ".bias"].data)) return -1;
                {
                    HostParam w; w.shape = {3 * C, C}; w.data.resize((size_t)3 * C * C);
                    const char* nm[3] = {".attn1.to_q.weight", ".attn1.to_k.weight", ".attn1.to_v.weight"};
                    for (int which = 0; which < 3; ++which) {
                        const std::vector<float>& src = c->params[b + nm[which]].data;
                        for (int h = 0; h < NH; ++h)
                            for (int j = 0; j < CH; ++j)
                                std::memcpy(&w.data[((size_t)(h * 3 + which) * CH + j) * C], &src[(size_t)(h * CH + j) * C], (size_t)C * 4);
                    }
                    if (make_conv(c, {&w}, {&zb}, &ow.qkvc)) return -1;
                }
                if (make_conv1(c, b + ".attn1.to_out.0", &ow.to_out1) || nobias(b + ".attn2.to_q", &ow.xqc) ||
                    make_conv1(c, b + ".attn2.to_out.0", &ow.to_out2) || make_conv1(c, b + ".ff.net.0.proj", &ow.ff1) ||
                    make_conv1(c, b + ".ff.net.2", &ow.ff2)) return -1;
                std::vector<float> z0((size_t)C, 0.f);
                if (upload(c, &ow.xkw, c->params[b + ".attn2.to_k.weight"].data) || upload(c, &ow.xkb, z0) ||
                    upload(c, &ow.xvw, c->params[b + ".attn2.to_v.weight"].data) || upload(c, &ow.xvb, z0)) return -1;
                break;
            }
            case OP_OUT:
                if (make_norm(c, op.pn_n1, &ow.g1) || make_conv1(c, op.pn_conv, &ow.conv, cfg.out_ch)) return -1;
                break;
        }
    }
    W.tproj_total = (long)tpb.size();
    if (upload(c, &W.tp_w, tpw) || upload(c, &W.tp_b, tpb)) return -1;
    double fl = 0.0;
    for (size_t oi = 0; oi < W.op.size(); ++oi) {
        const OpPlan& op = c->prog->ops[oi];
        const OpWeights& ow = W.op[oi];
        auto convf = [&](const ConvP& p, int H, int W) { fl += 2.0 * p.cin * p.cout * p.taps * (double)H * W; };
        const Tens& to = c->tens[op.out];
        switch (op.kind) {
            case OP_CONV_IN: case OP_CONV: case OP_DOWN: case OP_UP: case OP_OUT: convf(ow.conv, to.H, to.W); break;
            case OP_RES:
                convf(ow.c1, to.H, to.W); convf(ow.c2, to.H, to.W);
                if (op.has_nin) convf(ow.nin, to.H, to.W);
                break;
            case OP_XFMR: {
                for (const ConvP* p : {&ow.pj_in, &ow.qkvc, &ow.to_out1, &ow.xqc, &ow.to_out2, &ow.ff1, &ow.ff2, &ow.pj_out}) convf(*p, to.H, to.W);
                double T = (double)to.H * to.W;
                fl += 2.0 * 2.0 * T * T * to.C + 2.0 * 2.0 * T * c->cfg.context_len * to.C;
                break;
            }
            case OP_ATTN: {
                convf(ow.qkvc, to.H, to.W); convf(ow.proj, to.H, to.W);
                double T = (double)to.H * to.W;
                fl += 2.0 * 2.0 * T * T * to.C;
                if (op.has_x) {
                    convf(ow.xqc, to.H, to.W); convf(ow.xproj, to.H, to.W);
                    fl += 2.0 * 2.0 * T * c->cfg.context_len * to.C;
                }
                break;
            }
        }
    }
    W.flops = fl;
    for (auto& kv : c->params) { std::vector<float>().swap(kv.second.data); }
    return bind_weights(c);
}

struct Pass {
    loco_ctx* c;
    hipStream_t st;
    int B;
    float* arena;
    float* stats;
    float* T(int id) const { return arena + c->tens[id].off; }
    long bs() const { return c->prog->per_sample; }
};

static void drop_graphs(loco_ctx* c) {
    for (auto& kv : c->fwd_graphs) {
        if (kv.second.exec) (void)hipGraphExecDestroy(kv.second.exec);
        if (kv.second.graph) (void)hipGraphDestroy(kv.second.graph);
    }
    c->fwd_graphs.clear();
}
inline unsigned char* gemm_ws_get(loco_ctx* c, size_t need, hipStream_t st) {
    const int l = c->lane;
    if (c->gemm_ws_bytes[l] >= need) return c->gemm_ws[l];
    hipStreamCaptureStatus cs = hipStreamCaptureStatusNone;
    if (hipStreamIsCapturing(st, &cs) != hipSuccess || cs != hipStreamCaptureStatusNone) return nullptr;
    if (c->gemm_ws[l]) {
        (void)hipDeviceSynchronize();
        drop_graphs(c);
        (void)hipFree(c->gemm_ws[l]);
        c->bytes -= c->gemm_ws_bytes[l];
        c->gemm_ws[l] = nullptr; c->gemm_ws_bytes[l] = 0;
    }
    void* p = nullptr;
    if (hipMalloc(&p, need) != hipSuccess) { (void)hipGetLastError(); return nullptr; }
    c->gemm_ws[l] = static_cast<unsigned char*>(p); c->gemm_ws_bytes[l] = need; c->bytes += need;
    return c->gemm_ws[l];
}
inline bool attn_gemm_rec(const loco_ctx* c, const GemmArgs& g) { return c->prec >= 1 && c->gemm_lowp && gemm_rec_eligible(g); }
inline void attn_gemm(loco_ctx* c, const GemmArgs& g, hipStream_t st) {
    if (attn_gemm_rec(c, g)) {
        if (unsigned char* ws = gemm_ws_get(c, gemm_rec_ws_bytes(g), st)) { launch_gemm_rec(g, ws, st); return; }
    }
    if (c->prec >= 1 && c->gemm_lowp && gemm_prefers_bf16x3(g)) launch_gemm_bf16x3(g, st); else launch_gemm(g, st);
}

void conv_defaults(ConvArgs& a) {
    std::memset(&a, 0, sizeof(a));
    a.stride = 1; a.pad = 1; a.nsplit = 1; a.mode = CM_NONE; a.res_scale = 1.f;
}

struct NS { float *sc, *sh, *mr, *tst, *tc; };
NS nstats(const loco_ctx* c, float* base, const NormP& n) {
    NS s;
    s.sc = base + n.soff; s.sh = s.sc + n.C; s.mr = s.sh + n.C; s.tst = s.mr + 2 * c->cfg.gn_groups;
    s.tc = s.tst + 2 * c->cfg.gn_groups;
    return s;
}

struct StatReq {
    int kind = ST_NONE;
    NormP* n = nullptr;
    float* stats = nullptr;
    const float* prim = nullptr;
    const float* ss_scale = nullptr; const float* ss_shift = nullptr;
    float* keep = nullptr; size_t keep_floats = 0; int* keep_ntile = nullptr;
};

void stats_standalone(loco_ctx* c, const StatReq& rq, const float* x, long xbs, int B, int HW, int s0, hipStream_t st) {
    const NormP& n = *rq.n;
    const long SB = c->prog->stats_per_sample;
    const int G = c->cfg.gn_groups;
    if (rq.kind == ST_FWD) {
        NS s = nstats(c, rq.stats + (long)s0 * SB, n);
        launch_gn_stats(x, xbs, B, n.C, HW, G, eps_of(c, n), n.gamma, n.beta, s.mr, s.sc, s.sh, SB, c->red, st, rq.ss_scale,
                        rq.ss_shift);
    } else {
        NS sp = nstats(c, c->statsP, n);
        NS stt = nstats(c, rq.stats + (long)s0 * SB, n);
        launch_gn_tstats(x, xbs, rq.prim, 0, B, n.C, HW, G, sp.sc, sp.sh, sp.mr, 0, 0, rq.kind == ST_TAN ? 0 : 1, stt.tst,
                         stt.tc, SB, c->red, st, c->cfg.act);
    }
}

bool run_conv(loco_ctx* c, const ConvArgs& a0, int taps, hipStream_t st, const StatReq* rq = nullptr,
              const ConvArgs* second = nullptr) {
    const size_t span = (size_t)c->cfg.max_batch * c->prog->per_sample;
    auto padded = [&](const float* p) { return (p >= c->arenaP && p < c->arenaP + span) || (p >= c->arenaT && p < c->arenaT + span); };
    ConvArgs a = a0, sc;
    a.act = c->cfg.act;
    if (a.mode == CM_GN_SILU && c->cfg.act == ACT_GELU) a.mode = CM_GN_GELU;
    a.in_padded = padded(a.in);
    if (second) { sc = *second; sc.in_padded = padded(sc.in); }
    ConvEnv e;
    e.prec = c->prec; e.chip_share = c->chip_share; e.lanes = c->lanes_active; e.lane_s0 = c->lane_s0;
    e.partial = c->partial; e.partial_floats = c->partial_floats; e.stpart = c->stpart; e.stpart_floats = c->stpart_floats;
    e.fuse_stats = c->fuse_stats; e.fuse_lin = c->fuse_lin; e.deep1 = c->deep1; e.max_batch = c->cfg.max_batch;
    StatAsk q;
    if (rq) {
        q.kind = rq->kind; q.norm = rq->n != nullptr; q.prim = rq->prim; q.keep = rq->keep; q.keep_floats = rq->keep_floats;
        if (rq->n && rq->n->sx_off >= 0 && c->sxcache) q.sx = c->sxcache + rq->n->sx_off;
    }
    const ConvPlan p = plan_conv(e, a, taps, rq ? &q : nullptr, second ? &sc : nullptr);
    if (p.sc_first) run_conv(c, *second, 1, st);
#ifdef LOCO_DIAG
    if (c->plan_log) conv_plan_text(p, taps, c->prec, *c->plan_log);
#endif
    if (rq && rq->kind != ST_NONE && rq->n) rq->n->ready = true;
    if (rq && rq->keep_ntile) *rq->keep_ntile = p.keep_ntile;
    const int HWo = a.Hout * a.Wout, Gn = c->cfg.gn_groups;
    const long SBs = c->prog->stats_per_sample;
    auto timed = [&](const char* name, double flops, const ConvArgs& y, auto&& launch) {
        loco_ctx::ProfRec r;
        if (c->prof_on) {
            r.name = name; r.flops = flops;
            r.cin = y.Cin; r.cout = y.Cout; r.h = y.Hout; r.b = y.B; r.ns = y.nsplit; r.mode = y.mode; r.taps = taps;
            r.e0 = c->next_event(); r.e1 = c->next_event();
            (void)hipEventRecord(r.e0, st);
        }
        launch();
        if (c->prof_on) { (void)hipEventRecord(r.e1, st); c->prof.push_back(r); }
    };
    for (int li = 0; li < p.nl; ++li) {
        const ConvLaunch& l = p.l[li];
        const ConvArgs& x = l.args;
        for (int pi = 0; pi < l.nparts; ++pi) {
            const ConvArgs& y = l.parts[pi];
            double flops = 2.0 * (y.Cin * taps + y.Cin2) * y.Cout * (double)y.Hout * y.Wout * y.B;
            if (y.zins) flops *= 0.25;
            timed(c->prof_on ? conv_variant_name(y, taps, c->prec) : nullptr, flops, y, [&] {
                if (c->prec == 1) launch_conv_bf16x3(y, taps, st);
                else if (c->prec == 2) launch_conv_f16(y, taps, st);
                else launch_conv(y, taps, st);
            });
        }
        if (x.nsplit > 1) {
            timed("conv_splitk_reduce", 0.0, x, [&] {
                if (l.stats != SR_SPLITK) { launch_conv_splitk_reduce(x, st); return; }
                const NormP& n = *rq->n;
                NS sp = nstats(c, c->statsP, n);
                NS so = nstats(c, rq->stats + (long)l.s0 * SBs, n);
                launch_conv_splitk_reduce_stats(x, rq->kind, Gn, eps_of(c, n), n.gamma, n.beta, so.mr, so.sc, so.sh, SBs, rq->ss_scale,
                                                rq->ss_shift, rq->prim, sp.sc, sp.sh, sp.mr, so.tst, so.tc, SBs, c->red, st);
            });
        }
        if (l.stats == SR_ALONE) stats_standalone(c, *rq, x.out, x.out_bs, x.B, HWo, l.s0, st);
        if (l.stats == SR_EPI) {
            const NormP& n = *rq->n;
            NS so = nstats(c, rq->stats + (long)l.s0 * SBs, n);
            if (rq->kind != ST_FWD) {
                NS sp = nstats(c, c->statsP, n);
                launch_gn_lin_fused_finalize(rq->kind, x.st_part, n.C, l.ntile, nullptr, 0, x.B, n.C, HWo, Gn, sp.mr, so.tst, so.tc,
                                             SBs, st);
            } else {
                launch_gn_fused_finalize(x.st_part, l.ntile, x.B, n.C, HWo, Gn, eps_of(c, n), n.gamma, n.beta, so.mr, so.sc, so.sh,
                                         SBs, rq->ss_scale, rq->ss_shift, st);
            }
        }
    }
    if (p.stats_all) stats_standalone(c, *rq, a.out, a.out_bs, a.B, HWo, 0, st);
    return p.cot;
}

inline void setw(ConvArgs& a, const ConvP& p, bool dgrad) {
    a.w = dgrad ? p.wd : p.wf;
    a.wb = dgrad ? (const void*)p.wbd : (const void*)p.wbf;
    a.wh = dgrad ? (const void*)p.whd : (const void*)p.whf;
}

NormP* consumer_norm(loco_ctx* c, int tid) {
    const Tens& t = c->tens[tid];
    if (t.cons_op < 0) return nullptr;
    Op& op = c->ops[t.cons_op];
    return t.cons_norm == 2 ? &op.nx : &op.n1;
}
StatReq req_fwd(NormP* n, float* stats, const float* ss_scale = nullptr, const float* ss_shift = nullptr) {
    StatReq r;
    if (n) { r.kind = ST_FWD; r.n = n; r.stats = stats; r.ss_scale = ss_scale; r.ss_shift = ss_shift; }
    return r;
}
StatReq req_lin(loco_ctx* c, int kind, NormP* n, const float* prim) {
    StatReq r;
    if (n) { r.kind = kind; r.n = n; r.stats = c->statsT; r.prim = prim; }
    return r;
}
void clear_ready(loco_ctx* c) {
    for (auto& op : c->ops) op.n1.ready = op.n2.ready = op.nx.ready = false;
    for (auto& t : c->tens) t.keep_ntile = 0;
}
StatReq req_fwd_of(loco_ctx* c, int tid, float* stats) {
    StatReq r = req_fwd(consumer_norm(c, tid), stats);
    Tens& t = c->tens[tid];
    if (t.cat_of >= 0 && t.keep) {
        r.kind = ST_FWD; r.stats = stats;
        r.keep = t.keep; r.keep_floats = t.keep_floats; r.keep_ntile = &t.keep_ntile;
    }
    return r;
}
bool cat_fused_stats(loco_ctx* c, const NormP& n, int tid, float* stats, int B, hipStream_t st) {
    const Tens& q = c->tens[tid];
    if (q.cat_a < 0 || c->prec < 1 || !c->fuse_stats) return false;
    const Tens& A = c->tens[q.cat_a];
    const Tens& Bt = c->tens[q.cat_b];
    if (A.keep_ntile <= 0 || Bt.keep_ntile <= 0) return false;
    NS s = nstats(c, stats, n);
    launch_gn_fused_finalize_cat(A.keep, A.C, A.keep_ntile, Bt.keep, Bt.keep_ntile, B, q.C, q.H * q.W, c->cfg.gn_groups,
                                 eps_of(c, n), n.gamma, n.beta, s.mr, s.sc, s.sh, c->prog->stats_per_sample, st);
    return true;
}

bool cat_fused_tstats(loco_ctx* c, const NormP& n, int tid, int B, hipStream_t st) {
    const Tens& q = c->tens[tid];
    if (q.cat_a < 0 || c->prec < 1 || !c->fuse_stats || !c->fuse_lin) return false;
    const Tens& A = c->tens[q.cat_a];
    const Tens& Bt = c->tens[q.cat_b];
    if (A.keep_ntile <= 0 || Bt.keep_ntile <= 0) return false;
    NS sp = nstats(c, c->statsP, n);
    NS stt = nstats(c, c->statsT, n);
    const size_t MB = c->cfg.max_batch;
    launch_gn_lin_fused_finalize(ST_TAN, A.keep + c->lane_s0 * (A.keep_floats / MB), A.C, A.keep_ntile,
                                 Bt.keep + c->lane_s0 * (Bt.keep_floats / MB), Bt.keep_ntile, B, q.C, q.H * q.W,
                                 c->cfg.gn_groups, sp.mr, stt.tst, stt.tc, c->prog->stats_per_sample, st);
    return true;
}

void gn_forward_stats(const Pass& p, const NormP& n, const float* x, long xbs, int HW) {
    NS s = nstats(p.c, p.stats, n);
    launch_gn_stats(x, xbs, p.B, n.C, HW, p.c->cfg.gn_groups, eps_of(p.c, n), n.gamma, n.beta, s.mr, s.sc, s.sh,
                    p.c->prog->stats_per_sample, p.c->red, p.st);
}


struct XA {
    loco_ctx* c; const Op* op; hipStream_t st; int B; int C, T, NH, CH, Lp;
    float scale;
};
XA xa_of(loco_ctx* c, const Op& op, int B, hipStream_t st) {
    XA x; x.c = c; x.op = &op; x.st = st; x.B = B;
    const Tens& t = c->tens[op.in];
    x.C = t.C; x.T = t.H * t.W; x.NH = op.heads; x.CH = x.C / x.NH; x.Lp = c->prog->ctx_Lp;
    x.scale = 1.0f / std::sqrt((float)x.CH);
    return x;
}
void xa_scores(const XA& x, const float* X, long x_bs, const float* K, float* S, long s_bs, float alpha, bool mask) {
    GemmArgs g; std::memset(&g, 0, sizeof(g));
    g.A = X; g.sam = 1; g.sak = x.T; g.sab = x_bs; g.sah = (long)x.CH * x.T;
    g.Bm = K; g.sbk = x.Lp; g.sbn = 1; g.sbb = 0; g.sbh = (long)x.CH * x.Lp;
    g.C = S; g.scm = x.Lp; g.scn = 1; g.scb = s_bs; g.sch = (long)x.T * x.Lp;
    g.M = x.T; g.N = x.Lp; g.K = x.CH; g.batch = x.B; g.batch2 = x.NH; g.alpha = alpha; g.beta = 0.f;
    g.colbias = mask ? x.c->ctx_colbias : nullptr;
// ... 346 lines not shown
                h.Bm = p.T(op.S); h.sbk = 1; h.sbn = T; h.sbb = p.bs(); h.sbh = (long)T * T;
                h.C = p.T(op.o); h.scm = T; h.scn = 1; h.scb = p.bs(); h.sch = (long)CH * T;
                h.M = CH; h.N = T; h.K = T; h.batch = B; h.batch2 = NH; h.alpha = 1.f; h.beta = 0.f;
                attn_gemm(c, h, st);
                }
                ConvArgs pr; conv_defaults(pr);
                pr.in = p.T(op.o); pr.in_bs = p.bs(); pr.Cin = C; pr.Hin = to.H; pr.Win = to.W;
                setw(pr, op.proj, false); pr.bias = op.proj.bias; pr.pad = 0;
                pr.res = p.T(op.in); pr.res_bs = p.bs();
                pr.out = p.T(op.has_x ? op.xmid : op.out); pr.out_bs = p.bs(); pr.Cout = C; pr.Hout = to.H; pr.Wout = to.W; pr.B = B;
                {
                    const StatReq rq = next_fwd(op.has_x ? op.xmid : op.out);
                    run_conv(c, pr, 1, st, &rq);
                }
                if (op.has_x) {
                    if (!c->has_ctx) { c->err = "this architecture has cross-attention stages: call loco_set_context first"; return -1; }
                    const XA x = xa_of(c, op, B, st);
                    if (!op.nx.ready) gn_forward_stats(p, op.nx, p.T(op.xmid), p.bs(), HW);
                    op.nx.ready = false;
                    NS sx = nstats(c, stats, op.nx);
                    ConvArgs qa; conv_defaults(qa);
                    qa.in = p.T(op.xmid); qa.in_bs = p.bs(); qa.Cin = C; qa.Hin = to.H; qa.Win = to.W;
                    setw(qa, op.xqc, false); qa.bias = op.xqc.bias; qa.pad = 0;
                    qa.mode = CM_GN; qa.sc = sx.sc; qa.sh = sx.sh; qa.scsh_bs = SB;
                    qa.out = p.T(op.xq); qa.out_bs = p.bs(); qa.Cout = C; qa.Hout = to.H; qa.Wout = to.W; qa.B = B;
                    run_conv(c, qa, 1, st);
                    if (!xa_fused(x, 0, p.T(op.xq), p.bs(), op.xK, op.xV, p.T(op.xS), p.bs(), p.T(op.xo), p.bs())) {
                        xa_scores(x, p.T(op.xq), p.bs(), op.xK, p.T(op.xS), p.bs(), x.scale, true);
                        launch_softmax_rows(p.T(op.xS), (long)NH * T, x.Lp, st, B, p.bs());
                        xa_values(x, op.xV, p.T(op.xS), p.bs(), p.T(op.xo), p.bs());
                    }
                    const StatReq rqx = next_fwd(op.out);
                    xa_conv1x1(c, op.xproj, false, p.T(op.xo), p.bs(), p.T(op.out), p.bs(), C, to.H, to.W, B,
                               p.T(op.xmid), p.bs(), true, st, &rqx);
                }
                break;
            }
            case OP_XFMR: {
                if (!c->has_ctx) { c->err = "this architecture has cross-attention stages: call loco_set_context first"; return -1; }
                const int C = to.C, T = HW, NH = op.heads, H = to.H, W = to.W;
                const long PSb = p.bs();
                auto X = [&](int i) { return p.T(op.xt[i]); };
                if (!op.n1.ready) gn_forward_stats(p, op.n1, p.T(op.in), PSb, HW);
                op.n1.ready = false;
                NS s = nstats(c, stats, op.n1);
                {
                    ConvArgs a; conv_defaults(a);
                    a.in = p.T(op.in); a.in_bs = PSb; a.Cin = C; a.Hin = H; a.Win = W;
                    setw(a, op.pj_in, false); a.bias = op.pj_in.bias; a.pad = 0;
                    a.mode = CM_GN; a.sc = s.sc; a.sh = s.sh; a.scsh_bs = SB;
                    a.out = X(X_H0); a.out_bs = PSb; a.Cout = C; a.Hout = H; a.Wout = W; a.B = B;
                    run_conv(c, a, 1, st);
                }
                const SA sa{c, &op, B, T, NH, C / NH, st};
                const XA xa = xa_of(c, op, B, st);
                launch_ln_fwd(X(X_H0), PSb, B, C, T, op.lng[0], op.lnb[0], 1e-5f, X(X_A1), PSb, X(X_LN1), PSb, st);
                lin1x1(c, op.qkvc, false, X(X_A1), PSb, C, X(X_QKV), PSb, 3 * C, H, W, B, nullptr, 0, false, st);
                sa_forward(sa, arena);
                lin1x1(c, op.to_out1, false, X(X_O), PSb, C, X(X_H1), PSb, C, H, W, B, X(X_H0), PSb, true, st);
                launch_ln_fwd(X(X_H1), PSb, B, C, T, op.lng[1], op.lnb[1], 1e-5f, X(X_A2), PSb, X(X_LN2), PSb, st);
                lin1x1(c, op.xqc, false, X(X_A2), PSb, C, X(X_XQ), PSb, C, H, W, B, nullptr, 0, false, st);
                if (!xa_fused(xa, 0, X(X_XQ), PSb, op.xK, op.xV, X(X_XS), PSb, X(X_XO), PSb)) {
                    xa_scores(xa, X(X_XQ), PSb, op.xK, X(X_XS), PSb, xa.scale, true);
                    launch_softmax_rows(X(X_XS), (long)NH * T, xa.Lp, st, B, PSb);
                    xa_values(xa, op.xV, X(X_XS), PSb, X(X_XO), PSb);
                }
                lin1x1(c, op.to_out2, false, X(X_XO), PSb, C, X(X_H2), PSb, C, H, W, B, X(X_H1), PSb, true, st);
                launch_ln_fwd(X(X_H2), PSb, B, C, T, op.lng[2], op.lnb[2], 1e-5f, X(X_A3), PSb, X(X_LN3), PSb, st);
                lin1x1(c, op.ff1, false, X(X_A3), PSb, C, X(X_F), PSb, 8 * C, H, W, B, nullptr, 0, true, st);
                launch_geglu(0, X(X_F), PSb, nullptr, B, 4L * C * T, X(X_GG), PSb, st);
                lin1x1(c, op.ff2, false, X(X_GG), PSb, 4 * C, X(X_H3), PSb, C, H, W, B, X(X_H2), PSb, true, st);
                const StatReq rq = next_fwd(op.out);
                lin1x1(c, op.pj_out, false, X(X_H3), PSb, C, p.T(op.out), PSb, C, H, W, B, p.T(op.in), PSb, true, st, &rq);
                break;
            }
            case OP_DOWN: case OP_UP: {
                const Tens& ti = c->tens[op.in];
                ConvArgs a; conv_defaults(a);
                a.in = p.T(op.in); a.in_bs = p.bs(); a.Cin = ti.C; a.Hin = ti.H; a.Win = ti.W;
                setw(a, op.conv, false); a.bias = op.conv.bias;
                if (op.kind == OP_DOWN) { a.stride = 2; a.pad = op.sym_down ? 1 : 0; } else { a.upsample = 1; }
                a.out = p.T(op.out); a.out_bs = p.bs(); a.Cout = to.C; a.Hout = to.H; a.Wout = to.W; a.B = B;
                const StatReq rq = next_fwd(op.out);
                run_conv(c, a, 9, st, &rq);
                break;
            }
            case OP_OUT: {
                const Tens& ti = c->tens[op.in];
                if (!op.n1.ready) gn_forward_stats(p, op.n1, p.T(op.in), p.bs(), ti.H * ti.W);
                op.n1.ready = false;
                NS s = nstats(c, stats, op.n1);
                ConvArgs a; conv_defaults(a);
                a.in = p.T(op.in); a.in_bs = p.bs(); a.Cin = ti.C; a.Hin = ti.H; a.Win = ti.W;
                setw(a, op.conv, false); a.bias = op.conv.bias;
                a.mode = CM_GN_SILU; a.sc = s.sc; a.sh = s.sh; a.scsh_bs = SB;
                a.out = p.T(op.out); a.out_bs = p.bs(); a.Cout = to.C; a.Hout = to.H; a.Wout = to.W; a.B = B;
                run_conv(c, a, 9, st);
                break;
            }
        }
    }
    return 0;
}

void tangent_stats(loco_ctx* c, const NormP& n, const float* d, long dbs, const float* x, int HW, int B,
                   hipStream_t st) {
    NS sp = nstats(c, c->statsP, n);
    NS stt = nstats(c, c->statsT, n);
    launch_gn_tstats(d, dbs, x, 0, B, n.C, HW, c->cfg.gn_groups, sp.sc, sp.sh, sp.mr, 0, 0, 0, stt.tst,
                     stt.tc, c->prog->stats_per_sample, c->red, st);
}
void set_tan(loco_ctx* c, ConvArgs& a, const NormP& n, const float* prim) {
    NS sp = nstats(c, c->statsP, n);
    NS stt = nstats(c, c->statsT, n);
    a.mode = CM_TAN_SILU; a.prim = prim; a.prim_bs = 0;
    a.sc = sp.sc; a.sh = sp.sh; a.scsh_bs = 0; a.mr = sp.mr; a.mr_bs = 0; a.gamma_ = n.gamma;
    a.tst = stt.tst; a.tst_bs = c->prog->stats_per_sample; a.cpg = n.C / c->cfg.gn_groups;
    a.tc = stt.tc; a.tc_bs = c->prog->stats_per_sample;
    a.sx = (n.sx_off >= 0 && c->sxcache) ? c->sxcache + n.sx_off : nullptr;
}

constexpr size_t RED_BYTES = (size_t)4 << 20;

int tangent_pass(loco_ctx* c, const float* V, int B, hipStream_t st) {
    const loco_unet_cfg& cfg = c->cfg;
    const long PS = c->prog->per_sample;
    auto TP = [&](int id) { return c->arenaP + c->tens[id].off; };
    auto TT = [&](int id) { return c->arenaT + c->tens[id].off; };
    clear_ready(c);
    auto next_tan = [&](int tid) {
        StatReq r = req_lin(c, ST_TAN, consumer_norm(c, tid), TP(tid));
        Tens& t = c->tens[tid];
        if (t.cat_of >= 0 && t.keep && c->fuse_lin) {
            r.kind = ST_TAN; r.stats = c->statsT; r.prim = TP(tid);
            r.keep = t.keep; r.keep_floats = t.keep_floats; r.keep_ntile = &t.keep_ntile;
        }
        return r;
    };
    for (auto& op : c->ops) {
        const Tens& to = c->tens[op.out];
        const int HW = to.H * to.W;
        switch (op.kind) {
            case OP_CONV_IN: {
                ConvArgs a; conv_defaults(a);
                a.in = V; a.in_bs = c->prog->n_in; a.Cin = cfg.in_channels; a.Hin = cfg.resolution; a.Win = cfg.resolution;
                setw(a, op.conv, false);
                a.out = TT(op.out); a.out_bs = PS; a.Cout = to.C; a.Hout = to.H; a.Wout = to.W; a.B = B;
                if (op.ksize == 1) a.pad = 0;
                const StatReq rq = next_tan(op.out);
                run_conv(c, a, op.ksize == 1 ? 1 : 9, st, &rq);
                break;
            }
            case OP_CONV: {
                const Tens& ti = c->tens[op.in];
                ConvArgs a; conv_defaults(a);
                a.in = TT(op.in); a.in_bs = PS; a.Cin = ti.C; a.Hin = ti.H; a.Win = ti.W;
                setw(a, op.conv, false);
                a.out = TT(op.out); a.out_bs = PS; a.Cout = to.C; a.Hout = to.H; a.Wout = to.W; a.B = B;
                if (op.ksize == 1) a.pad = 0;
                const StatReq rq = next_tan(op.out);
                run_conv(c, a, op.ksize == 1 ? 1 : 9, st, &rq);
                break;
            }
            case OP_RES: {
                const Tens& ti = c->tens[op.in];
                const int HWi = ti.H * ti.W;
                if (!op.n1.ready && !cat_fused_tstats(c, op.n1, op.in, B, st)) tangent_stats(c, op.n1, TT(op.in), PS, TP(op.in), HWi, B, st);
// ... 77 lines not shown
                if (!flash) {
                attn_gemm(c, g, st);
                if (!kcat) { g.A = q; g.sab = 0; g.Bm = dk; g.sbb = PS; g.beta = 1.f; attn_gemm(c, g, st); }
                launch_softmax_jac(TT(op.S), TP(op.S), (long)NH * T, T, (long)NH * T, 1.0f / std::sqrt((float)CH), st, B, PS);
                }
                GemmArgs h; std::memset(&h, 0, sizeof(h));
                h.A = dv; h.sam = T; h.sak = 1; h.sab = PS; h.sah = HS;
                h.Bm = TP(op.S); h.sbk = 1; h.sbn = T; h.sbb = 0; h.sbh = SS;
                h.C = TT(op.o); h.scm = T; h.scn = 1; h.scb = PS; h.sch = (long)CH * T;
                h.M = CH; h.N = T; h.K = T; h.batch = B; h.batch2 = NH; h.alpha = 1.f; h.beta = 0.f;
                if (kcat) { h.A2 = v; h.sab2 = 0; h.Bm2 = TT(op.S); h.sbb2 = PS; }
                if (!flash) {
                attn_gemm(c, h, st);
                if (!kcat) { h.A = v; h.sab = 0; h.Bm = TT(op.S); h.sbb = PS; h.beta = 1.f; attn_gemm(c, h, st); }
                }
                ConvArgs pr; conv_defaults(pr);
                pr.in = TT(op.o); pr.in_bs = PS; pr.Cin = C; pr.Hin = to.H; pr.Win = to.W;
                setw(pr, op.proj, false); pr.pad = 0; pr.res = TT(op.in); pr.res_bs = PS;
                pr.out = TT(op.has_x ? op.xmid : op.out); pr.out_bs = PS; pr.Cout = C; pr.Hout = to.H; pr.Wout = to.W; pr.B = B;
                {
                    const StatReq rq = next_tan(op.has_x ? op.xmid : op.out);
                    run_conv(c, pr, 1, st, &rq);
                }
                if (op.has_x) {
                    const XA x = xa_of(c, op, B, st);
                    if (!op.nx.ready) tangent_stats(c, op.nx, TT(op.xmid), PS, TP(op.xmid), HW, B, st);
                    op.nx.ready = false;
                    NS spx = nstats(c, c->statsP, op.nx);
                    NS stx = nstats(c, c->statsT, op.nx);
                    launch_gn_apply(1, TT(op.xmid), PS, TP(op.xmid), 0, nullptr, 0, TT(op.xhn), PS, 0, B, C, HW,
                                    cfg.gn_groups, spx.sc, spx.sh, spx.mr, 0, 0, stx.tst, c->prog->stats_per_sample, st);
                    xa_conv1x1(c, op.xqc, false, TT(op.xhn), PS, TT(op.xq), PS, C, to.H, to.W, B, nullptr, 0, false, st);
                    if (!xa_fused(x, 1, TT(op.xq), PS, op.xK, op.xV, TP(op.xS), 0, TT(op.xo), PS)) {
                        xa_scores(x, TT(op.xq), PS, op.xK, TT(op.xS), PS, 1.f, false);
                        launch_softmax_jac(TT(op.xS), TP(op.xS), (long)NH * T, x.Lp, (long)NH * T, x.scale, st, B, PS);
                        xa_values(x, op.xV, TT(op.xS), PS, TT(op.xo), PS);
                    }
                    const StatReq rqx = next_tan(op.out);
                    xa_conv1x1(c, op.xproj, false, TT(op.xo), PS, TT(op.out), PS, C, to.H, to.W, B, TT(op.xmid), PS, false, st, &rqx);
                }
                break;
            }
            case OP_XFMR: {
                const int C = to.C, T = HW, NH = op.heads, H = to.H, W = to.W;
                auto XP = [&](int i) { return TP(op.xt[i]); };
                auto XT_ = [&](int i) { return TT(op.xt[i]); };
                if (!op.n1.ready) tangent_stats(c, op.n1, TT(op.in), PS, TP(op.in), HW, B, st);
                op.n1.ready = false;
                NS sp = nstats(c, c->statsP, op.n1);
                NS stt = nstats(c, c->statsT, op.n1);
                launch_gn_apply(1, TT(op.in), PS, TP(op.in), 0, nullptr, 0, XT_(X_G0), PS, 0, B, C, HW,
                                cfg.gn_groups, sp.sc, sp.sh, sp.mr, 0, 0, stt.tst, c->prog->stats_per_sample, st);
                lin1x1(c, op.pj_in, false, XT_(X_G0), PS, C, XT_(X_H0), PS, C, H, W, B, nullptr, 0, false, st);
                const SA sa{c, &op, B, T, NH, C / NH, st};
                const XA xa = xa_of(c, op, B, st);
                launch_ln_tan(XT_(X_H0), PS, XP(X_H0), XP(X_LN1), B, C, T, op.lng[0], XT_(X_A1), PS, st);
                lin1x1(c, op.qkvc, false, XT_(X_A1), PS, C, XT_(X_QKV), PS, 3 * C, H, W, B, nullptr, 0, false, st);
                sa_tangent(sa);
                lin1x1(c, op.to_out1, false, XT_(X_O), PS, C, XT_(X_H1), PS, C, H, W, B, XT_(X_H0), PS, false, st);
                launch_ln_tan(XT_(X_H1), PS, XP(X_H1), XP(X_LN2), B, C, T, op.lng[1], XT_(X_A2), PS, st);
                lin1x1(c, op.xqc, false, XT_(X_A2), PS, C, XT_(X_XQ), PS, C, H, W, B, nullptr, 0, false, st);
                if (!xa_fused(xa, 1, XT_(X_XQ), PS, op.xK, op.xV, XP(X_XS), 0, XT_(X_XO), PS)) {
                    xa_scores(xa, XT_(X_XQ), PS, op.xK, XT_(X_XS), PS, 1.f, false);
                    launch_softmax_jac(XT_(X_XS), XP(X_XS), (long)NH * T, xa.Lp, (long)NH * T, xa.scale, st, B, PS);
                    xa_values(xa, op.xV, XT_(X_XS), PS, XT_(X_XO), PS);
                }
                lin1x1(c, op.to_out2, false, XT_(X_XO), PS, C, XT_(X_H2), PS, C, H, W, B, XT_(X_H1), PS, false, st);
                launch_ln_tan(XT_(X_H2), PS, XP(X_H2), XP(X_LN3), B, C, T, op.lng[2], XT_(X_A3), PS, st);
                lin1x1(c, op.ff1, false, XT_(X_A3), PS, C, XT_(X_F), PS, 8 * C, H, W, B, nullptr, 0, false, st);
                launch_geglu(1, XT_(X_F), PS, XP(X_F), B, 4L * C * T, XT_(X_GG), PS, st);
                lin1x1(c, op.ff2, false, XT_(X_GG), PS, 4 * C, XT_(X_H3), PS, C, H, W, B, XT_(X_H2), PS, false, st);
                const StatReq rq = next_tan(op.out);
                lin1x1(c, op.pj_out, false, XT_(X_H3), PS, C, TT(op.out), PS, C, H, W, B, TT(op.in), PS, false, st, &rq);
                break;
            }
            case OP_DOWN: case OP_UP: {
                const Tens& ti = c->tens[op.in];
                ConvArgs a; conv_defaults(a);
                a.in = TT(op.in); a.in_bs = PS; a.Cin = ti.C; a.Hin = ti.H; a.Win = ti.W;
                setw(a, op.conv, false);
                if (op.kind == OP_DOWN) { a.stride = 2; a.pad = op.sym_down ? 1 : 0; } else { a.upsample = 1; }
                a.out = TT(op.out); a.out_bs = PS; a.Cout = to.C; a.Hout = to.H; a.Wout = to.W; a.B = B;
                const StatReq rq = next_tan(op.out);
                run_conv(c, a, 9, st, &rq);
                break;
            }
            case OP_OUT: {
                const Tens& ti = c->tens[op.in];
                if (!op.n1.ready) tangent_stats(c, op.n1, TT(op.in), PS, TP(op.in), ti.H * ti.W, B, st);
                op.n1.ready = false;
                ConvArgs a; conv_defaults(a);
                a.in = TT(op.in); a.in_bs = PS; a.Cin = ti.C; a.Hin = ti.H; a.Win = ti.W;
                setw(a, op.conv, false);
                set_tan(c, a, op.n1, TP(op.in));
                a.out = TT(op.out); a.out_bs = PS; a.Cout = to.C; a.Hout = to.H; a.Wout = to.W; a.B = B;
                run_conv(c, a, 9, st);
                break;
            }
        }
    }
    return 0;
}

void cot_stats(loco_ctx* c, const NormP& n, const float* d, long dbs, const float* x, int HW, int B, int kind,
               hipStream_t st) {
    NS sp = nstats(c, c->statsP, n);
    NS stt = nstats(c, c->statsT, n);
    launch_gn_tstats(d, dbs, x, 0, B, n.C, HW, c->cfg.gn_groups, sp.sc, sp.sh, sp.mr, 0, 0, kind, stt.tst,
                     stt.tc, c->prog->stats_per_sample, c->red, st, c->cfg.act);
}

int cotangent_pass(loco_ctx* c, const float* ge, const float* gx0, float* Aout, int B, hipStream_t st) {
    const loco_unet_cfg& cfg = c->cfg;
    const long PS = c->prog->per_sample;
    const int G = cfg.gn_groups;
    auto TP = [&](int id) { return c->arenaP + c->tens[id].off; };
    auto TG = [&](int id) { return c->arenaT + c->tens[id].off; };
    auto GO = [&](const Op& o) -> const float* { return o.out == c->prog->eps_t ? ge : TG(o.out); };
    auto GOS = [&](const Op& o) -> long { return o.out == c->prog->eps_t ? (long)c->prog->n_out : PS; };
    clear_ready(c);
    for (int oi = (int)c->ops.size() - 1; oi >= 0; --oi) {
        Op& op = c->ops[oi];
        const Tens& to = c->tens[op.out];
        const int HW = to.H * to.W;
        switch (op.kind) {
            case OP_OUT: {
                const Tens& ti = c->tens[op.in];
                ConvArgs a; conv_defaults(a);
                a.in = GO(op); a.in_bs = GOS(op); a.Cin = to.C; a.Hin = to.H; a.Win = to.W;
                setw(a, op.conv, true);
                a.out = TG(op.a1); a.out_bs = PS; a.Cout = ti.C; a.Hout = ti.H; a.Wout = ti.W; a.B = B;
                {
                    const StatReq rq = req_lin(c, ST_COT, &op.n1, TP(op.in));
                    run_conv(c, a, 9, st, &rq);
                    op.n1.ready = false;
                }
                NS sp = nstats(c, c->statsP, op.n1);
                NS stt = nstats(c, c->statsT, op.n1);
                launch_gn_apply(2, TG(op.a1), PS, TP(op.in), 0, nullptr, 0, TG(op.in), PS, 0, B, ti.C, ti.H * ti.W, G,
                                sp.sc, sp.sh, sp.mr, 0, 0, stt.tst, c->prog->stats_per_sample, st, cfg.act);
                break;
            }
            case OP_UP: {
                const Tens& ti = c->tens[op.in];
                ConvArgs a; conv_defaults(a);
                a.in = TG(op.out); a.in_bs = PS; a.Cin = to.C; a.Hin = to.H; a.Win = to.W;
                setw(a, op.conv, true);
                a.out = TG(op.up); a.out_bs = PS; a.Cout = ti.C; a.Hout = to.H; a.Wout = to.W; a.B = B;
                run_conv(c, a, 9, st);
                launch_pool2x2_sum(TG(op.up), PS, TG(op.in), PS, 0, B, ti.C, ti.H, ti.W, st);
                break;
            }
            case OP_DOWN: {
                const Tens& ti = c->tens[op.in];
                ConvArgs a; conv_defaults(a);
                a.in = TG(op.out); a.in_bs = PS; a.Cin = to.C; a.Hin = to.H; a.Win = to.W;
                setw(a, op.conv, true); a.zins = 1; a.pad = op.sym_down ? 1 : 2; a.accumulate = op.in_is_skip ? 1 : 0;
                a.out = TG(op.in); a.out_bs = PS; a.Cout = ti.C; a.Hout = ti.H; a.Wout = ti.W; a.B = B;
                run_conv(c, a, 9, st);
                break;
            }
            case OP_RES: {
                const Tens& ti = c->tens[op.in];
                const int HWi = ti.H * ti.W;
                ConvArgs a; conv_defaults(a);
                a.in = TG(op.out); a.in_bs = PS; a.Cin = to.C; a.Hin = to.H; a.Win = to.W;
                setw(a, op.c2, true);
                a.out = TG(op.h1); a.out_bs = PS; a.Cout = to.C; a.Hout = to.H; a.Wout = to.W; a.B = B;
                {
                    const StatReq rq2 = req_lin(c, ST_COT, &op.n2, TP(op.h1));
                    run_conv(c, a, 9, st, &rq2);
                    op.n2.ready = false;
                }
                ConvArgs b; conv_defaults(b);
                b.in = TG(op.h1); b.in_bs = PS; b.Cin = to.C; b.Hin = to.H; b.Win = to.W;
                setw(b, op.c1, true);
                set_tan(c, b, op.n2, TP(op.h1));
                b.mode = CM_COT_SILU;
                b.out_bs = PS; b.Cout = ti.C; b.Hout = to.H; b.Wout = to.W; b.B = B;
                if (op.updown == 0) {
                    b.out = TG(op.a1);
                    const StatReq rq1 = req_lin(c, ST_COT, &op.n1, TP(op.in));
                    run_conv(c, b, 9, st, &rq1);
                } else if (op.updown == 1) {
                    b.out = TG(op.ap);
                    run_conv(c, b, 9, st);
                    launch_upsample2x(TG(op.ap), PS, TG(op.a1), PS, 0, 0.25f, B, ti.C, to.H, to.W, st);
                } else {
                    b.out = TG(op.xu);
                    run_conv(c, b, 9, st);
                    launch_pool2x2_sum(TG(op.xu), PS, TG(op.a1), PS, 0, B, ti.C, ti.H, ti.W, st);
                }
                if (!op.n1.ready) cot_stats(c, op.n1, TG(op.a1), PS, TP(op.in), HWi, B, 1, st);
                op.n1.ready = false;
                NS sp = nstats(c, c->statsP, op.n1);
                NS stt = nstats(c, c->statsT, op.n1);
                int acc = op.in_is_skip ? 1 : 0;
                const float* gsk = TG(op.out);
                bool cot_in_epilogue = false;
                if (op.has_nin) {
                    ConvArgs n; conv_defaults(n);
                    n.in = TG(op.out); n.in_bs = PS; n.Cin = to.C; n.Hin = to.H; n.Win = to.W;
                    setw(n, op.nin, true); n.pad = 0;
                    n.Cout = ti.C; n.Hout = to.H; n.Wout = to.W; n.B = B; n.out_bs = PS;
                    n.out = TG(op.in); n.accumulate = acc;
                    if (op.updown == 0 && c->prec >= 1 && c->fuse_cot && op.n1.sx_off >= 0 && c->sxcache) {
                        n.cot_d = TG(op.a1); n.cot_d_bs = PS; n.cot_sx = c->sxcache + op.n1.sx_off;
                        n.cot_tc = stt.tc; n.cot_tc_bs = c->prog->stats_per_sample;
                    }
                    cot_in_epilogue = run_conv(c, n, 1, st);
                    gsk = nullptr;
                }
                if (op.updown == 0) {
                    if (cot_in_epilogue) {  }
                    else if (op.has_nin)
                        launch_gn_apply(2, TG(op.a1), PS, TP(op.in), 0, nullptr, 0, TG(op.in), PS, 1, B, ti.C, HWi, G,
                                        sp.sc, sp.sh, sp.mr, 0, 0, stt.tst, c->prog->stats_per_sample, st, cfg.act);
                    else
                        launch_gn_apply(2, TG(op.a1), PS, TP(op.in), 0, gsk, PS, TG(op.in), PS, acc, B, ti.C, HWi, G,
                                        sp.sc, sp.sh, sp.mr, 0, 0, stt.tst, c->prog->stats_per_sample, st, cfg.act, c->prog->res_scale);
                } else {
                    launch_gn_apply(2, TG(op.a1), PS, TP(op.in), 0, nullptr, 0, TG(op.in), PS, acc, B, ti.C, HWi, G,
                                    sp.sc, sp.sh, sp.mr, 0, 0, stt.tst, c->prog->stats_per_sample, st, cfg.act);
                    if (op.updown == 1) launch_upsample2x(gsk, PS, TG(op.in), PS, 1, 0.25f * c->prog->res_scale, B, ti.C, to.H, to.W, st);
                    else launch_pool2x2_sum(gsk, PS, TG(op.in), PS, 1, B, ti.C, ti.H, ti.W, st, c->prog->res_scale);
                }
                break;
            }
            case OP_ATTN: {
                const int C = to.C, T = HW, NH = op.heads, CH = C / NH;
                const long HS = 3L * CH * T, SS = (long)T * T, OS = (long)CH * T;
                float* q = TP(op.qkv); float* k = q + (long)CH * T; float* v = k + (long)CH * T;
                float* gq = TG(op.qkv); float* gk = gq + (long)CH * T; float* gv = gk + (long)CH * T;
                const int so = op.has_x ? op.xmid : op.out;
                if (op.has_x) {
                    const XA x = xa_of(c, op, B, st);
                    xa_conv1x1(c, op.xproj, true, TG(op.out), PS, TG(op.xo), PS, C, to.H, to.W, B, nullptr, 0, false, st);
                    if (!xa_fused(x, 1, TG(op.xo), PS, op.xV, op.xK, TP(op.xS), 0, TG(op.xq), PS)) {
                        xa_scores(x, TG(op.xo), PS, op.xV, TG(op.xS), PS, 1.f, false);
                        launch_softmax_jac(TG(op.xS), TP(op.xS), (long)NH * T, x.Lp, (long)NH * T, x.scale, st, B, PS);
                        xa_values(x, op.xK, TG(op.xS), PS, TG(op.xq), PS);
                    }
// ... 753 lines not shown
                       int32_t rule, float* m_out, uint8_t* mask_out, void* stream) {
    if (!c) return -2;
    if (!eps_a || !eps_b || !mask_out || B < 1 || C < 1 || HW < 1) { c->err = "diffedit_mask: bad arguments"; return -2; }
    if (rule != 0 && rule != 1) { c->err = "diffedit_mask: rule is 0 (reference) or 1 (intended)"; return -2; }
    float* ws = reinterpret_cast<float*>(c->gscratch);
    const size_t cap = 2 * ((((size_t)c->prog->n_in + 255) / 256) * 64 * 64 + 4096);
    float* m = m_out;
    if (!m) {
        if (1024 + (size_t)HW > cap) { c->err = "diffedit_mask: map larger than the reduction workspace; pass m_out"; return -2; }
        m = ws + 1024;
    }
    hipStream_t st = (hipStream_t)stream;
    launch_diffedit_mask(eps_a, eps_b, scale, B, C, (long)HW, rule, m, mask_out, ws, ws + 768, st);
    HIPCHK(c, hipGetLastError());
    float status[3] = {0.f, 0.f, 0.f};
    HIPCHK(c, hipMemcpyAsync(status, ws + 768, sizeof(status), hipMemcpyDeviceToHost, st));
    HIPCHK(c, hipStreamSynchronize(st));
    if (status[0] == 1.f) {
        c->err = "diffedit_mask: constant map (max == min = " + std::to_string(status[1]) + "): the two noise predictions do not differ";
        return -4;
    }
    if (status[0] != 0.f) { c->err = "diffedit_mask: non-finite map"; return -5; }
    return 0;
}

int loco_cfg_masked_step(loco_ctx* c, const float* x, const float* eps_for, const float* eps_edit, const float* eps_null,
                         float g, float at, float at_next, const uint8_t* mask, int32_t B, int64_t n, float* x_next,
                         void* stream) {
    if (!c) return -2;
    if (!x || !eps_for || !eps_edit || !eps_null || !mask || !x_next || B < 1 || n < 1) {
        c->err = "cfg_masked_step: bad arguments";
        return -2;
    }
    float s1, s2, s3, ce, cn;
    sched_coeffs(at, at_next, 0.f, &s1, &s2, &s3, &ce, &cn);
    launch_cfg_masked_step(x, eps_for, eps_edit, eps_null, mask, x_next, B, (long)n, g, s2, s1, s3, ce, (hipStream_t)stream);
    HIPCHK(c, hipGetLastError());
    return 0;
}

int loco_lcm_step(loco_ctx* c, const float* x, const float* eps, float at, float at_prev, float c_skip, float c_out,
                  const float* noise, int64_t count, float* x_prev, float* denoised, void* stream) {
    if (!c) return -2;
    if (!x || !eps || count < 1 || (!x_prev && !denoised)) { c->err = "lcm_step: bad arguments"; return -2; }
    if (!(at > 0.f && at <= 1.f) || !(at_prev >= 0.f && at_prev <= 1.f)) { c->err = "lcm_step: alpha-bar outside (0, 1]"; return -2; }
    launch_lcm_step(x, eps, noise, x_prev, denoised, (long)count, std::sqrt(at), std::sqrt(1.0f - at), std::sqrt(at_prev),
                    std::sqrt(1.0f - at_prev), c_skip, c_out, (hipStream_t)stream);
    HIPCHK(c, hipGetLastError());
    return 0;
}

#ifdef LOCO_DIAG
}
__global__ void diag_fill_records(unsigned char* rec, long nrec, int wpitch, unsigned seed, float scale) {
    const long r = (long)blockIdx.x * 256 + threadIdx.x;
    if (r >= nrec) return;
    const int idx = (int)(r % wpitch);
    unsigned short hi[16], lo[16];
    for (int k = 0; k < 16; ++k) {
        unsigned h = (unsigned)(r * 16 + k) * 2654435761u + seed * 40503u;
        h ^= h >> 15; h *= 2246822519u; h ^= h >> 13; h *= 3266489917u; h ^= h >> 16;
        const float v = scale * ((float)(h & 0xffffff) * (1.0f / 8388608.0f) - 1.0f);
        const __bf16 hb = (__bf16)v;
        const __bf16 lb = (__bf16)(v - (float)hb);
        hi[k] = __builtin_bit_cast(unsigned short, hb);
        lo[k] = __builtin_bit_cast(unsigned short, lb);
    }
    const int sw = (idx >> 2) & 3;
    unsigned short* base = reinterpret_cast<unsigned short*>(rec + r * 64);
    for (int k = 0; k < 8; ++k) {
        base[((0 ^ sw) << 3) + k] = hi[k];
        base[((1 ^ sw) << 3) + k] = hi[8 + k];
        base[((2 ^ sw) << 3) + k] = lo[k];
        base[((3 ^ sw) << 3) + k] = lo[8 + k];
    }
}
extern "C" {
int loco_bench_conv(loco_ctx* c, int32_t cin, int32_t cout, int32_t H, int32_t W, int32_t B, int32_t mode,
                    int32_t taps, int32_t tile, int32_t iters, float* ms_avg, void* stream) {
    if (!c) return -2;
    if (finalize_params(c)) return -3;
    hipStream_t st = (hipStream_t)stream;
    const long HW = (long)H * W;
    const long in_e = (long)cin * HW, out_e = (long)cout * HW;
    if ((in_e + out_e) * B > (long)c->cfg.max_batch * c->prog->per_sample || 2 * in_e > (long)c->prog->per_sample ||
        in_e > c->prog->sx_total) { c->err = "bench_conv: shape exceeds the arenas"; return -2; }
    float* in = c->arenaT;
    float* out = c->arenaT + in_e * B;
    const int bz = getenv("LOCO_BENCH_ZERO") ? atoi(getenv("LOCO_BENCH_ZERO")) : 0;
    const float zs = (bz & 1) ? 0.0f : 1.0f, zw = (bz & 2) ? 0.0f : 1.0f;
    launch_fill_random(in, in_e * B, 1u, zs, st);
    launch_fill_random(c->arenaP, in_e, 2u, zs, st);
    launch_fill_random(reinterpret_cast<float*>(c->sxcache), 2 * in_e, 3u, zs, st);
    launch_fill_random(c->statsP, c->prog->stats_per_sample, 4u, 1.0f, st);
    launch_fill_random(c->statsT, c->prog->stats_per_sample * B, 5u, 0.01f, st);
    size_t wfl = (size_t)((cin + 15) / 16) * 16 * taps * ((cout + 31) & ~31);
    if (wfl * 2 > c->partial_floats) { c->err = "bench_conv: weights exceed workspace"; return -2; }
    float* wf = c->partial + c->partial_floats - wfl * 2;
    launch_fill_random(wf, (long)wfl * 2, 6u, 0.05f * zw, st);
    if (c->prec == 1) {
        const long nrec = (long)((cin + 15) / 16) * taps * ((cout + 31) & ~31);
        hipLaunchKernelGGL(diag_fill_records, dim3((unsigned)((nrec + 255) / 256)), dim3(256), 0, st,
                           reinterpret_cast<unsigned char*>(wf), nrec, (cout + 31) & ~31, 7u, 0.05f * zw);
    }
    ConvArgs a; conv_defaults(a);
    a.in = in; a.in_bs = in_e; a.Cin = cin; a.Hin = H; a.Win = W;
    a.prim = c->arenaP; a.prim_bs = 0; a.sx = c->sxcache;
    a.w = wf; a.wb = wf; a.wh = wf;
    a.out = out; a.out_bs = out_e; a.Cout = cout; a.Hout = H; a.Wout = W; a.B = B;
    a.mode = mode; a.pad = taps == 9 ? 1 : 0; a.in_padded = 1; a.taps = taps;
    a.sc = c->statsP; a.sh = c->statsP + cin; a.scsh_bs = 0; a.mr = c->statsP + 2 * cin; a.mr_bs = 0;
    a.gamma_ = c->statsP; a.tst = c->statsT; a.tst_bs = c->prog->stats_per_sample; a.cpg = cin / c->cfg.gn_groups;
    a.tc = c->statsT + 64; a.tc_bs = c->prog->stats_per_sample;
    if (a.cpg < 1) a.cpg = 1;
    a.nsplit = 1; a.partial = c->partial;
    a.partial_floats = c->partial_floats - wfl * 2;
    if (getenv("LOCO_BENCH_COT") && atoi(getenv("LOCO_BENCH_COT")) && taps == 1) {
        if ((in_e + 2 * out_e) * B > (long)c->cfg.max_batch * c->prog->per_sample || out_e > c->prog->sx_total ||
            2L * cout > c->prog->stats_per_sample) { c->err = "bench_conv: cot operands exceed the arenas"; return -2; }
        launch_fill_random(out + out_e * B, out_e * B, 8u, zs, st);
        if (out_e > in_e) launch_fill_random(reinterpret_cast<float*>(c->sxcache), 2 * out_e, 3u, zs, st);
        a.cot_d = out + out_e * B; a.cot_d_bs = out_e; a.cot_sx = c->sxcache; a.cot_tc = c->statsT; a.cot_tc_bs = c->prog->stats_per_sample;
    }
    if (getenv("LOCO_BENCH_ACC") && atoi(getenv("LOCO_BENCH_ACC"))) a.accumulate = 1;
    conv_plan_family(a, c->prec);
    if (const char* e = getenv("LOCO_DUAL_WHATIF")) a.no_deep = atoi(e);
    ConvArgs parts[2];
    const int nparts = conv_plan_parts(a, c->prec, tile, parts);
    auto run = [&]() {
        for (int pi = 0; pi < nparts; ++pi) {
            if (c->prec == 1) launch_conv_bf16x3(parts[pi], taps, st);
            else if (c->prec == 2) launch_conv_f16(parts[pi], taps, st);
            else launch_conv(parts[pi], taps, st);
        }
        launch_conv_splitk_reduce(a, st);
    };
    run();
    HIPCHK(c, hipEventRecord(c->ev0, st));
    for (int i = 0; i < iters; ++i) run();
    HIPCHK(c, hipEventRecord(c->ev1, st));
    HIPCHK(c, hipEventSynchronize(c->ev1));
    c->bench_out = out; c->bench_out_count = (int64_t)out_e * B;
    float ms = 0.f;
    HIPCHK(c, hipEventElapsedTime(&ms, c->ev0, c->ev1));
    *ms_avg = ms / iters;
    HIPCHK(c, hipGetLastError());
    return 0;
}

}
__global__ void diag_scale_tc(const float* tc, const float* mr, int C, int cpg, long n, int by_rstd, float* out) {
    const long i = (long)blockIdx.x * 256 + threadIdx.x;
    if (i >= n) return;
    const float f = by_rstd ? mr[2 * (int)((i % C) / cpg) + 1] : 1.0f;
    out[2 * i] = f * tc[2 * i];
    out[2 * i + 1] = f * tc[2 * i + 1];
}
extern "C" {
int loco_debug_conv(loco_ctx* c, const loco_conv_desc* d, char* plan, int64_t cap, void* stream) {
    if (!c) return -2;
    if (!d || d->struct_size != (int32_t)sizeof(loco_conv_desc)) { c->err = "debug_conv: descriptor size mismatch"; return -2; }
    if (finalize_params(c)) return -3;
    hipStream_t st = (hipStream_t)stream;
    const int taps = d->taps, k = taps == 9 ? 3 : 1, B = d->B;
    if ((taps != 9 && taps != 1) || d->Cin < 1 || d->Cout < 1 || d->Hin < 1 || d->Win < 1 || B < 1 || (d->stride != 1 && d->stride != 2) ||
        d->mode < CM_NONE || d->mode > CM_GN_GELU || (d->upsample && d->zins) || (d->stride == 2 && (d->upsample || d->zins)) ||
        !d->weight || !d->in || !d->out) { c->err = "debug_conv: bad descriptor"; return -2; }
    if (d->stride == 2 && ((d->Hin | d->Win) & 1)) { c->err = "debug_conv: stride 2 needs an even map"; return -2; }
    const bool lin = d->mode == CM_TAN_SILU || d->mode == CM_COT_SILU;
    if (d->mode != CM_NONE && (!d->sc || !d->sh)) { c->err = "debug_conv: the prologue modes need sc / sh"; return -2; }
    if (lin && (!d->prim || !d->mr || !d->gamma || !d->tst || !d->tc || d->cpg < 1 || d->Cin % d->cpg)) {
        c->err = "debug_conv: modes 3 / 4 need prim, mr, gamma, tst, tc and cpg"; return -2;
    }
    if (d->Cin2 > 0 && (!d->in2 || !d->w2)) { c->err = "debug_conv: the second operator needs in2 and w2"; return -2; }
    if (d->Cin2 > 0 && (d->res || d->accumulate || taps != 9)) {
        c->err = "debug_conv: the second operator goes with a 3x3 conv without res / accumulate"; return -2;
    }
    if (d->cot_d && (!d->cot_prim || !d->cot_sc || !d->cot_sh || !d->cot_mr || !d->cot_tc || d->cot_cpg < 1 || d->Cout % d->cot_cpg)) {
        c->err = "debug_conv: the norm-cotangent term needs cot_prim, cot_sc, cot_sh, cot_mr, cot_tc and cot_cpg"; return -2;
    }
    const int Hout = d->stride == 2 ? d->Hin / 2 : (d->upsample || d->zins) ? 2 * d->Hin : d->Hin;
    const int Wout = d->stride == 2 ? d->Win / 2 : (d->upsample || d->zins) ? 2 * d->Win : d->Win;
    {
        auto pow2 = [](int v) { return v >= 8 && (v & (v - 1)) == 0; };
        if (!((pow2(Hout) && pow2(Wout)) || (Wout % 32 == 0 && Hout % 8 == 0 && ((long)Hout * Wout) % 256 == 0))) {
            c->err = "debug_conv: output map outside the tile geometry of the conv kernels"; return -2;
        }
    }
    const long in_e = (long)d->Cin * d->Hin * d->Win, out_e = (long)d->Cout * Hout * Wout, in2_e = (long)d->Cin2 * Hout * Wout;
    if ((in_e | out_e | in2_e) & 3) { c->err = "debug_conv: planes must be whole 16-byte units"; return -2; }
    auto up64 = [](long v) { return (v + 63) & ~63L; };
    const long offT_in2 = d->in_arena ? up64(in_e * B) : 0, offT_cot = offT_in2 + up64(in2_e * B);
    const long needT = offT_cot + (d->cot_d ? out_e * B : 0);
    const long sx_cot = lin ? up64(in_e) : 0, need_sx = sx_cot + (d->cot_d ? out_e : 0);
    if (needT > (long)c->cfg.max_batch * c->prog->per_sample || (lin && in_e > (long)c->cfg.max_batch * c->prog->per_sample) ||
        need_sx > c->prog->sx_total) { c->err = "debug_conv: shape exceeds the arenas"; return -2; }
    const int G = lin ? d->Cin / d->cpg : 0;
    const long tbs = up64(2L * G) + up64(2L * d->Cin);
    const long small_n = (lin ? (long)B * tbs : 0) + (d->cot_d ? (long)B * up64(2L * d->Cout) : 0) + 64;
    const size_t owned0 = c->owned.size();
    const size_t bytes0 = c->bytes;
    auto release = [&]() {
        (void)hipStreamSynchronize(st);
        while (c->owned.size() > owned0) { (void)hipFree(c->owned.back()); c->owned.pop_back(); }
        c->bytes = bytes0;
    };
    auto host_param = [&](const float* p, std::vector<int64_t> shape) {
        HostParam h; h.shape = shape; h.loaded = true;
        size_t n = 1; for (int64_t s : shape) n *= (size_t)s;
        if (p) h.data.assign(p, p + n); else h.data.assign(n, 0.f);
        return h;
    };
    const int m_out = d->transposed ? d->Cin : d->Cout, m_in = d->transposed ? d->Cout : d->Cin;
    HostParam w = host_param(d->weight, {m_out, m_in, k, k}), wb0 = host_param(nullptr, {m_out});
    HostParam w2 = host_param(d->Cin2 > 0 ? d->w2 : nullptr, {d->Cout, d->Cin2 > 0 ? d->Cin2 : 1, 1, 1}), wb2 = host_param(nullptr, {d->Cout});
    ConvP cp, cp2;
    float *bias_d = nullptr, *bias2nd_d = nullptr, *small = nullptr;
    int rc = make_conv(c, {&w}, {&wb0}, &cp);
    if (!rc && d->Cin2 > 0) rc = make_conv(c, {&w2}, {&wb2}, &cp2);
    if (!rc && d->bias) rc = upload(c, &bias_d, std::vector<float>(d->bias, d->bias + d->Cout));
    if (!rc && d->Cin2 > 0 && d->bias2nd) rc = upload(c, &bias2nd_d, std::vector<float>(d->bias2nd, d->bias2nd + d->Cout));
    if (!rc) rc = dalloc(c, &small, (size_t)small_n);
    if (rc) { release(); return -1; }
    auto copy = [&](float* dst, const float* src, long n) {
        return hipMemcpyAsync(dst, src, (size_t)n * sizeof(float), hipMemcpyDeviceToDevice, st);
    };
    hipError_t he = hipSuccess;
    ConvArgs a; conv_defaults(a);
    if (d->in_arena) { he = copy(c->arenaT, d->in, in_e * B); a.in = c->arenaT; } else a.in = d->in;
    a.in_bs = in_e; a.Cin = d->Cin; a.Hin = d->Hin; a.Win = d->Win;
    setw(a, cp, d->transposed != 0);
    a.bias = bias_d;
    a.out = d->out; a.out_bs = out_e; a.Cout = d->Cout; a.Hout = Hout; a.Wout = Wout; a.B = B;
    a.bias2 = d->bias2; a.bias2_bs = d->Cout;
    a.res = d->res; a.res_bs = out_e; a.res_scale = d->res_scale;
    a.mode = d->mode; a.stride = d->stride; a.upsample = d->upsample; a.zins = d->zins; a.accumulate = d->accumulate;
    a.pad = d->pad >= 0 ? d->pad : taps == 1 ? 0 : d->zins ? 2 : d->stride == 2 ? 0 : 1;
    a.sc = d->sc; a.sh = d->sh; a.scsh_bs = 0; a.cpg = d->cpg;
    if (lin) {
        if (he == hipSuccess) he = copy(c->arenaP, d->prim, in_e);
        a.prim = c->arenaP; a.prim_bs = 0;
        a.mr = d->mr; a.mr_bs = 0; a.gamma_ = d->gamma;
        for (int b = 0; b < B && he == hipSuccess; ++b) he = copy(small + b * tbs, d->tst + (long)b * 2 * G, 2L * G);
        a.tst = small; a.tst_bs = tbs;
        for (int b = 0; b < B; ++b)
            hipLaunchKernelGGL(diag_scale_tc, dim3((unsigned)((d->Cin + 255) / 256)), dim3(256), 0, st, d->tc + (long)b * 2 * d->Cin, d->mr,
                               d->Cin, d->cpg, (long)d->Cin, d->mode == CM_COT_SILU ? 1 : 0, small + b * tbs + up64(2L * G));
        a.tc = small + up64(2L * G); a.tc_bs = tbs;
        launch_gn_cache(c->arenaP, d->Cin, d->Hin * d->Win, d->cpg, d->sc, d->sh, d->mr, c->sxcache, st, ACT_SILU);
        a.sx = c->sxcache;
    }
    ConvArgs n2; conv_defaults(n2);
    if (d->Cin2 > 0) {
        float* in2 = c->arenaT + offT_in2;
        if (he == hipSuccess) he = copy(in2, d->in2, in2_e * B);
        n2.in = in2; n2.in_bs = in2_e; n2.Cin = d->Cin2; n2.Hin = Hout; n2.Win = Wout;
        setw(n2, cp2, false); n2.bias = bias2nd_d; n2.pad = 0;
        n2.out = d->out; n2.out_bs = out_e; n2.Cout = d->Cout; n2.Hout = Hout; n2.Wout = Wout; n2.B = B;
        a.res = d->out; a.res_bs = out_e;
    }
    if (d->cot_d) {
        float* cd = c->arenaT + offT_cot;
        float* ctc = small + (lin ? (long)B * tbs : 0);
        const long cbs = up64(2L * d->Cout);
        if (he == hipSuccess) he = copy(cd, d->cot_d, out_e * B);
        for (int b = 0; b < B; ++b)
            hipLaunchKernelGGL(diag_scale_tc, dim3((unsigned)((d->Cout + 255) / 256)), dim3(256), 0, st, d->cot_tc + (long)b * 2 * d->Cout,
                               d->cot_mr, d->Cout, d->cot_cpg, (long)d->Cout, 1, ctc + b * cbs);
        launch_gn_cache(d->cot_prim, d->Cout, Hout * Wout, d->cot_cpg, d->cot_sc, d->cot_sh, d->cot_mr, c->sxcache + sx_cot, st, ACT_SILU);
        a.cot_d = cd; a.cot_d_bs = out_e; a.cot_sx = c->sxcache + sx_cot; a.cot_tc = ctc; a.cot_tc_bs = cbs;
    }
    if (he != hipSuccess) { c->err = std::string("debug_conv: ") + hipGetErrorString(he); release(); return -1; }
    std::string text;
    const int act0 = c->cfg.act;
    if (d->mode == CM_GN_GELU) c->cfg.act = ACT_GELU;
    c->plan_log = &text;
    const bool rode = run_conv(c, a, taps, st, nullptr, d->Cin2 > 0 ? &n2 : nullptr);
    c->plan_log = nullptr;
    c->cfg.act = act0;
    he = hipGetLastError();
    release();
    if (he == hipSuccess) he = hipGetLastError();
    if (he != hipSuccess) { c->err = std::string("debug_conv: ") + hipGetErrorString(he); return -1; }
    if (plan && cap > 0) {
        if ((int64_t)text.size() + 1 > cap) { c->err = "debug_conv: plan buffer too small"; return -4; }
        std::memcpy(plan, text.c_str(), text.size() + 1);
    }
    if (d->cot_d && !rode) { c->err = "debug_conv: norm-cotangent term declined"; return 1; }
    return 0;
}

#endif

int loco_set_streams(loco_ctx* c, int32_t n) {
    if (!c || (n != 1 && n != 2)) return -2;
    c->n_streams = n;
    return 0;
}

int loco_set_chip_share(loco_ctx* c, int32_t n) {
    if (!c || n < 1 || n > 8) return -2;
    c->chip_share = n;
    return 0;
}

int loco_set_side_stream(loco_ctx* c, void* stream) {
    if (!c) return -2;
    c->st2_user = (hipStream_t)stream;
    return 0;
}

int loco_profile_enable(loco_ctx* c, int32_t on) {
    if (!c) return -2;
    c->prof_on = on != 0;
    c->prof_shapes = on == 2;
    if (on) { c->prof.clear(); c->ev_used = 0; }
    return 0;
}

int loco_profile_report(loco_ctx* c, char* buf, int64_t cap) {
    if (!c || !buf || cap < 1) return -2;
    HIPCHK(c, hipDeviceSynchronize());
    std::map<std::string, std::array<double, 3>> agg;
    for (auto& r : c->prof) {
        float ms = 0.f;
        if (hipEventElapsedTime(&ms, r.e0, r.e1) != hipSuccess) continue;
        std::string key = r.name;
        if (c->prof_shapes) {
            char sb[96];
            snprintf(sb, sizeof(sb), "|t%d_m%d_ci%d_co%d_h%d_b%d_s%d", r.taps, r.mode, r.cin, r.cout, r.h, r.b, r.ns);
            key += sb;
        }
        auto& a = agg[key];
        a[0] += 1.0; a[1] += ms; a[2] += r.flops;
    }
    std::string out;
    char line[256];
    for (auto& kv : agg) {
        snprintf(line, sizeof(line), "%s %.0f %.6f %.6e\n", kv.first.c_str(), kv.second[0], kv.second[1], kv.second[2]);
        out += line;
    }
    if ((int64_t)out.size() + 1 > cap) { c->err = "profile buffer too small"; return -4; }
    std::memcpy(buf, out.c_str(), out.size() + 1);
    return 0;
}

#ifdef LOCO_DIAG
int64_t loco_debug_tensor(loco_ctx* c, const char* name, float* dst, int64_t cap, void* stream) {
    if (!c) return -2;
    std::string nm(name);
    if (nm == "bench_out") {
        if (!c->bench_out) { c->err = "no loco_bench_conv yet"; return -3; }
        int64_t cnt = cap < c->bench_out_count ? cap : c->bench_out_count;
        HIPCHK(c, hipMemcpyAsync(dst, c->bench_out, (size_t)cnt * sizeof(float), hipMemcpyDeviceToDevice, (hipStream_t)stream));
        return cnt;
    }
    if (nm == "workspace") {
        int64_t cnt = cap < (int64_t)c->partial_floats ? cap : (int64_t)c->partial_floats;
        HIPCHK(c, hipMemcpyAsync(dst, c->partial, (size_t)cnt * sizeof(float), hipMemcpyDeviceToDevice, (hipStream_t)stream));
        return cnt;
// ... 25 lines not shown
```

loco-edit_amd/csrc/kernels.h:

```cpp
#pragma once
#include <hip/hip_runtime.h>
#include <stdint.h>

namespace loco {

struct DeviceOnce { bool seen[64] = {}; };
inline bool first_on_device(DeviceOnce& f) {
    int d = 0;
    (void)hipGetDevice(&d);
    d &= 63;
    if (f.seen[d]) return false;
    f.seen[d] = true;
    return true;
}


enum ConvMode : int {
    CM_NONE = 0,
    CM_GN_SILU = 1,
    CM_GN = 2,
    CM_TAN_SILU = 3,
    CM_COT_SILU = 4,
    CM_GN_GELU = 5,
};
enum ActKind : int { ACT_SILU = 0, ACT_GELU = 1 };
__device__ __forceinline__ float act_fwd(float y, int act) {
    if (act == ACT_GELU) return 0.5f * y * (1.0f + erff(y * 0.70710678118654752f));
    return y * (1.0f / (1.0f + __expf(-y)));
}
__device__ __forceinline__ float act_der(float y, int act) {
    if (act == ACT_GELU) return 0.5f * (1.0f + erff(y * 0.70710678118654752f)) + y * 0.39894228040143268f * __expf(-0.5f * y * y);
    const float sg = 1.0f / (1.0f + __expf(-y));
    return sg * (1.0f + y * (1.0f - sg));
}

enum StatKind : int { ST_NONE = 0, ST_FWD = 1, ST_TAN = 2, ST_COT = 3 };

struct ConvArgs {
    const float* in; long in_bs; int Cin, Hin, Win;
    const float* prim; long prim_bs;
    const float* w;
    const void* wb;
    const void* wh;
    const float2* sx;
    float* out; long out_bs; int Cout, Hout, Wout;
    const float* bias;
    const float* bias2; long bias2_bs;
    const float* res; long res_bs;
    const float* sc; const float* sh; long scsh_bs;
    const float* mr; long mr_bs;
    const float* gamma_;
    const float* tst; long tst_bs;
    const float* tc; long tc_bs;
    int cpg;
    int mode;
    int stride;
    int pad;
    int upsample;
    int zins;
    int in_padded;
    int accumulate;
    int nsplit;
    int taps;
    int no_deep;
    float* partial;
    int B;
    float* st_part; int st_kind;
    const float* st_x; const float2* st_sx;
    const float* in2; long in2_bs; int Cin2; int in2_padded;
    const void* wb2;
    const float* cot_d; long cot_d_bs; const float2* cot_sx; const float* cot_tc; long cot_tc_bs;
    int act;
    float res_scale;
    int dual;
    int gemm, gemm_tm;
    size_t partial_floats;
    int pers_groups;
    int tile, pair;
};

void launch_conv(const ConvArgs& a, int taps, hipStream_t st);
void launch_conv_bf16x3(const ConvArgs& a, int taps, hipStream_t st);
void launch_conv_f16(const ConvArgs& a, int taps, hipStream_t st);
void launch_conv_splitk_reduce(const ConvArgs& a, hipStream_t st);

struct ConvEnv {
    int prec = 1;
    int chip_share = 1;
    int lanes = 1, lane_s0 = 0;
    float* partial = nullptr; size_t partial_floats = 0;
    float* stpart = nullptr; size_t stpart_floats = 0;
    bool fuse_stats = true, fuse_lin = true, deep1 = true;
    int max_batch = 1;
};

struct StatAsk {
    int kind = ST_NONE;
    bool norm = false;
    const float2* sx = nullptr;
    const float* prim = nullptr;
    float* keep = nullptr; size_t keep_floats = 0;
};

enum StatRoute : int {
    SR_NONE = 0,
    SR_EPI = 1,
    SR_SPLITK = 2,
    SR_ALONE = 3,
    SR_KEEP = 4,
};

struct ConvLaunch {
    ConvArgs args;
    ConvArgs parts[2]; int nparts = 1;
    int s0 = 0;
    int stats = SR_NONE;
    int ntile = 0;
};

struct ConvPlan {
    bool sc_first = false;
    int nl = 1;
    ConvLaunch l[2];
    bool stats_all = false;
    int keep_ntile = 0;
    bool cot = false;
};

ConvPlan plan_conv(const ConvEnv& env, const ConvArgs& a, int taps, const StatAsk* ask, const ConvArgs* shortcut);
void conv_plan_family(ConvArgs& a, int prec);
int conv_plan_parts(ConvArgs& a, int prec, int tile_override, ConvArgs parts[2]);

int conv_bf16_tile_couts(const ConvArgs& a);
const char* conv_variant_name(const ConvArgs& a, int taps, int prec);

void launch_fill_random(float* p, long count, unsigned seed, float scale, hipStream_t st);
void launch_gn_cache(const float* x, int C, int HW, int cpg, const float* sc, const float* sh, const float* mr,
                     float2* sx, hipStream_t st, int act = 0);

struct GemmArgs {
    const float* A; long sam, sak, sab;
    const float* Bm; long sbk, sbn, sbb;
    float* C; long scm, scn, scb;
    const float* bias;
    const float* colbias;
    const float* R; long srb;
    int M, N, K, batch;
    float alpha, beta;
    int batch2; long sah, sbh, sch;
    const float* A2; long sab2; const float* Bm2; long sbb2;
};
void launch_gemm(const GemmArgs& g, hipStream_t st);
enum GemmAct : int { GEMM_ACT_NONE = 0, GEMM_ACT_QUICK_GELU = 1, GEMM_ACT_GELU = 2 };
void launch_gemm_fixed(const GemmArgs& g, int act, hipStream_t st);
void launch_gemm_bf16x3(const GemmArgs& g, hipStream_t st);
bool gemm_prefers_bf16x3(const GemmArgs& g);
bool gemm_rec_eligible(const GemmArgs& g);
size_t gemm_rec_ws_bytes(const GemmArgs& g);
void launch_gemm_rec(const GemmArgs& g, unsigned char* ws, hipStream_t st);

struct AttnFlashArgs {
    int T, NH, B, CH; float scale;
    const float *q, *k, *v; long hs;
    const float* P;
    const float* o;
    const float *dq, *dk, *dv; long bs_d;
    float* out; long bs_out;
    const float* go; long bs_go;
    float *gq, *gk, *gv; long bs_g;
    float* delta;
    int Lt; const float *kt, *vt;
    unsigned char* ws; size_t ws_bytes;
};
size_t attn_flash_ws_bytes(const AttnFlashArgs& a);
bool attn_flash_supported(int T, int CH);
bool attn_flash_text_supported(int T, int CH, int Lt);
void launch_attn_flash_tangent(const AttnFlashArgs& a, hipStream_t st);
void launch_attn_flash_cotangent(const AttnFlashArgs& a, hipStream_t st);

void launch_ln_fwd(const float* x, long xbs, int B, int C, int T, const float* gamma, const float* beta, float eps, float* y,
                   long ybs, float* stats, long sbs, hipStream_t st);
void launch_ln_tan(const float* dx, long dbs, const float* xprim, const float* sprim, int B, int C, int T, const float* gamma,
                   float* dy, long ybs, hipStream_t st);
void launch_ln_cot(const float* gy, long gbs, const float* xprim, const float* sprim, int B, int C, int T, const float* gamma,
                   const float* base, long base_bs, float* gx, long xbs, hipStream_t st);
struct XAttnArgs {
    int T, NH, B, CH, L, Lp, fwd;
    float alpha;
    const float* X; long x_bs;
    const float* K1; const float* K2;
    float* P; long p_bs;
    float* O; long o_bs;
};
bool xattn_fused_supported(int T, int CH, int L, int Lp);
void launch_xattn_fused(const XAttnArgs& a, hipStream_t st);
void launch_geglu(int kind, const float* in, long in_bs, const float* fprim, int B, long n4, float* out, long out_bs,
                  hipStream_t st);

void launch_gn_stats(const float* x, long bs, int B, int C, int HW, int G, float eps,
                     const float* gamma, const float* beta,
                     float* mr, float* sc, float* sh, long stats_bs, double* scratch, hipStream_t st,
                     const float* ss_scale = nullptr, const float* ss_shift = nullptr);
void launch_gn_fused_finalize_cat(const float* partA, int C1, int ntA, const float* partB, int ntB, int B, int C, int HW, int G,
                                  float eps, const float* gamma, const float* beta, float* mr, float* sc, float* sh,
                                  long stats_bs, hipStream_t st);
void launch_gn_fused_finalize(const float* part, int ntile, int B, int C, int HW, int G, float eps, const float* gamma,
                              const float* beta, float* mr, float* sc, float* sh, long stats_bs, const float* ss_scale,
                              const float* ss_shift, hipStream_t st);
void launch_gn_lin_fused_finalize(int kind, const float* partA, int C1, int ntA, const float* partB, int ntB, int B, int C, int HW,
                                  int G, const float* mr, float* tst, float* tc, long tst_bs, hipStream_t st);
void launch_conv_splitk_reduce_stats(const ConvArgs& a, int kind, int G, float eps, const float* gamma, const float* beta,
                                     float* mr, float* sc, float* sh, long stats_bs, const float* ss_scale,
                                     const float* ss_shift, const float* prim, const float* sc_prim, const float* sh_prim,
                                     const float* mr_prim, float* tst, float* tc, long tst_bs, double* scratch,
// ... 80 lines not shown
```

Baseline: 19.93 edit-directions/s.

## Add polyphase 2x2-tap path for upsample and zero-insert 3x3 convolutions

Rewrites nearest-upsample + 3x3 convs and zero-inserted transposed (dgrad) convs as four 2x2 polyphase sub-convolutions. Each runs on the low-resolution input with its own pre-combined weight set, picked per output phase, and writes strided outputs. This removes the redundant MACs on duplicated or zero-inserted pixels (9 taps become 4 effective taps per phase). In exchange it needs extra phase weight storage, a strided scalar epilogue store instead of vector nontemporal stores, and a narrow gate that aborts on unsupported configs.

New measurement: 19.94 edit-directions/s (median of 3 runs). Within noise of the previous version (+0.1%).

```diff
diff --git a/loco-edit_amd/csrc/conv_bf16.hip b/loco-edit_amd/csrc/conv_bf16.hip
--- a/loco-edit_amd/csrc/conv_bf16.hip
+++ b/loco-edit_amd/csrc/conv_bf16.hip
@@ -10,6 +10,7 @@
 template <int PR, int MODE> void launch_pair_b(const ConvArgs& a, hipStream_t st);
 template <int PR, int MODE> void launch_dual_b(const ConvArgs& a, hipStream_t st);
 void launch_conv_gemm(const ConvArgs& a, hipStream_t st);
+template <int PR> void launch_poly_b(const ConvArgs& a, hipStream_t st);
 
 template <int PR>
 static void launch_lowp(const ConvArgs& a, int taps, hipStream_t st) {
@@ -22,6 +23,14 @@
 #endif
     if constexpr (PR == PR_BF16X3) {
         if (taps == 1 && a.gemm) { launch_conv_gemm(a, st); return; }
+    }
+    if (taps == 4) {
+        if (!a.poly || a.mode != CM_NONE || a.nsplit != 1 || a.upsample || a.zins || a.stride != 1) {
+            fprintf(stderr, "loco: a 2x2-tap launch outside the polyphase gate (poly %d, mode %d, nsplit %d)\n", a.poly, a.mode, a.nsplit);
+            abort();
+        }
+        launch_poly_b<PR>(a, st);
+        return;
     }
     if (taps == 9 && a.Cin2 > 0) {
         if (a.mode == CM_GN_SILU) launch_kcat_b<PR, CM_GN_SILU>(a, st);
diff --git a/loco-edit_amd/csrc/conv_bf16_inst_l.hip b/loco-edit_amd/csrc/conv_bf16_inst_l.hip
--- /dev/null
+++ b/loco-edit_amd/csrc/conv_bf16_inst_l.hip
@@ -0,0 +1,5 @@
+#include "conv_bf16_kernel.h"
+
+namespace loco {
+template void launch_poly_b<PR_BF16X3>(const ConvArgs&, hipStream_t);
+}
diff --git a/loco-edit_amd/csrc/conv_bf16_inst_l_f16.hip b/loco-edit_amd/csrc/conv_bf16_inst_l_f16.hip
--- /dev/null
+++ b/loco-edit_amd/csrc/conv_bf16_inst_l_f16.hip
@@ -0,0 +1,5 @@
+#include "conv_bf16_kernel.h"
+
+namespace loco {
+template void launch_poly_b<PR_F16>(const ConvArgs&, hipStream_t);
+}
diff --git a/loco-edit_amd/csrc/conv_bf16_kernel.h b/loco-edit_amd/csrc/conv_bf16_kernel.h
--- a/loco-edit_amd/csrc/conv_bf16_kernel.h
+++ b/loco-edit_amd/csrc/conv_bf16_kernel.h
@@ -70,6 +70,7 @@
 
 constexpr int max_halo(int NT, int taps, bool s2) {
     if (taps == 1) return NT;
+    if (taps == 4) return (NT >= 128 ? NT / 32 + 1 : 3) * 33;
     if (NT >= 128) {
         int th = NT / 32;
         return s2 ? (2 * th + 1) * 65 : (th + 2) * 34;
@@ -98,36 +99,36 @@
 }
 
 constexpr int EPI_COT1 = 1, EPI_STATS = 2;
-template <int WM, int WN, int TM, int TN, int EPI = EPI_STATS, class StageRound>
+template <int WM, int WN, int TM, int TN, int EPI = EPI_STATS, bool POLY = false, class StageRound>
 __device__ __forceinline__ void conv_lowp_epilogue_staged(const ConvArgs& a, StageRound&& stage_round, unsigned char* smem_b, const int co0,
                                                           const int oy0, const int ox0, const int TW, const int tile_id, const int b,
-                                                          const int split);
+                                                          const int split, const int pp = 0);
 template <int WM, int WN, int TM, int TN>
 __device__ __forceinline__ void conv_lowp_epilogue_direct(const ConvArgs& a, f32x16 (&acc)[TM][TN], const int co0, const int oy0,
                                                           const int ox0, const int TW, const int b, const int split);
-template <int WM, int WN, int TM, int TN, int EPI = EPI_STATS>
+template <int WM, int WN, int TM, int TN, int EPI = EPI_STATS, bool POLY = false>
 __device__ __forceinline__ void conv_lowp_epilogue(const ConvArgs& a, f32x16 (&acc)[TM][TN], unsigned char* smem_b, const int co0,
                                                    const int oy0, const int ox0, const int TW, const int tile_id, const int b,
-                                                   const int split) {
+                                                   const int split, const int pp = 0) {
     constexpr int NT = WN * TN * 32;
     const int lane = threadIdx.x & 63, wave = threadIdx.x >> 6;
     const int l31 = lane & 31, khalf = lane >> 5, wm = wave / WN, wn = wave % WN;
-    if (co0 + WM * TM * 32 <= a.Cout) {
-        conv_lowp_epilogue_staged<WM, WN, TM, TN, EPI>(a, [&](const int h, float* S) {
+    if (POLY || co0 + WM * TM * 32 <= a.Cout) {
+        conv_lowp_epilogue_staged<WM, WN, TM, TN, EPI, POLY>(a, [&](const int h, float* S) {
 #pragma unroll
             for (int j = 0; j < TN; ++j)
 #pragma unroll
                 for (int r = 0; r < 16; ++r)
                     S[(wm * 32 + (r & 3) + 8 * (r >> 2) + 4 * khalf) * NT + (wn * TN + j) * 32 + l31] = acc[h][j][r];
-        }, smem_b, co0, oy0, ox0, TW, tile_id, b, split);
+        }, smem_b, co0, oy0, ox0, TW, tile_id, b, split, pp);
         return;
     }
-    conv_lowp_epilogue_direct<WM, WN, TM, TN>(a, acc, co0, oy0, ox0, TW, b, split);
-}
-template <int WM, int WN, int TM, int TN, int EPI, class StageRound>
+    if constexpr (!POLY) conv_lowp_epilogue_direct<WM, WN, TM, TN>(a, acc, co0, oy0, ox0, TW, b, split);
+}
+template <int WM, int WN, int TM, int TN, int EPI, bool POLY, class StageRound>
 __device__ __forceinline__ void conv_lowp_epilogue_staged(const ConvArgs& a, StageRound&& stage_round, unsigned char* smem_b, const int co0,
                                                           const int oy0, const int ox0, const int TW, const int tile_id, const int b,
-                                                          const int split) {
+                                                          const int split, const int pp) {
     constexpr int NTHR = WM * WN * 64;
     constexpr bool COT1 = (EPI & EPI_COT1) != 0, STATS = (EPI & EPI_STATS) != 0;
     constexpr int MT = WM * TM * 32;
@@ -158,7 +159,16 @@
         constexpr int RSTEP = NTHR / NQ;
         static_assert(NTHR % NQ == 0 && 32 % RSTEP == 0, "epilogue task rows");
         const int row0 = tid / NQ, quad0 = tid & (NQ - 1);
-        const unsigned pix0 = (unsigned)((oy0 + ((quad0 * 4) >> twsh)) * a.Wout + ox0 + ((quad0 * 4) & (TW - 1)));
+        const unsigned pix0 = POLY ? (unsigned)((2 * (oy0 + ((quad0 * 4) >> twsh)) + (pp >> 1)) * a.Wout + 2 * (ox0 + ((quad0 * 4) & (TW - 1))) + (pp & 1))
+                                   : (unsigned)((oy0 + ((quad0 * 4) >> twsh)) * a.Wout + ox0 + ((quad0 * 4) & (TW - 1)));
+        auto ld4 = [&](const float* p) -> f32x4 {
+            if constexpr (POLY) return f32x4{p[0], p[2], p[4], p[6]};
+            else return *reinterpret_cast<const f32x4*>(p);
+        };
+        auto st4 = [&](float* p, const f32x4 v4) {
+            if constexpr (POLY) { p[0] = v4[0]; p[2] = v4[1]; p[4] = v4[2]; p[6] = v4[3]; }
+            else __builtin_nontemporal_store(v4, reinterpret_cast<f32x4*>(p));
+        };
         auto co_of = [&](int h, int q) -> int { return co0 + row0 + (((q * RSTEP) >> 5) * TM + h) * 32 + ((q * RSTEP) & 31); };
         auto off_of = [&](int h, int q) -> unsigned {
             const unsigned crow = (unsigned)((((q * RSTEP) >> 5) * TM + h) * 32 + ((q * RSTEP) & 31));
@@ -192,11 +202,17 @@
                 for (int q = 0; q < NTASK; ++q) {
                     const unsigned o = off_of(h, q);
                     if (lin_cot) {
+                        if constexpr (POLY) {
+                            const float2 r0 = a.st_sx[o], r1 = a.st_sx[o + 2], r2 = a.st_sx[o + 4], r3 = a.st_sx[o + 6];
+                            xs[q][0] = f32x4{r0.x, r0.y, r1.x, r1.y};
+                            xs[q][1] = f32x4{r2.x, r2.y, r3.x, r3.y};
+                        } else {
                         const f32x4* sp4 = reinterpret_cast<const f32x4*>(a.st_sx + o);
                         xs[q][0] = sp4[0];
                         xs[q][1] = sp4[1];
+                        }
                     } else {
-                        xs[q][0] = *reinterpret_cast<const f32x4*>(a.st_x + o);
+                        xs[q][0] = ld4(a.st_x + o);
                     }
                 }
             }
@@ -209,8 +225,8 @@
 #pragma unroll
                 for (int q = 0; q < NTASK; ++q) {
                     f32x4 t4 = {0.f, 0.f, 0.f, 0.f};
-                    if (rb) t4 = a.res_scale * *reinterpret_cast<const f32x4*>(rb + off_of(h, q));
-                    if (accu) t4 += *reinterpret_cast<const f32x4*>(ob + off_of(h, q));
+                    if (rb) t4 = a.res_scale * ld4(rb + off_of(h, q));
+                    if (accu) t4 += ld4(ob + off_of(h, q));
                     rv[q] = t4;
                 }
 #pragma unroll
@@ -235,7 +251,7 @@
                 if (b1) add += b1[co_of(h, q)];
                 if (b2) add += b2[co_of(h, q)];
                 v[q] += add;
-                __builtin_nontemporal_store(v[q], reinterpret_cast<f32x4*>(ob + off_of(h, q)));
+                st4(ob + off_of(h, q), v[q]);
             }
             if constexpr (STATS) if (lin_st) {
 #pragma unroll
@@ -457,9 +473,11 @@
     constexpr int NPC = RB / 16;
     constexpr int MT = WM * TM * 32;
     constexpr int NT = WN * TN * 32;
-    constexpr int KS = (TAPS == 9) ? 3 : 1;
+    constexpr int KS = (TAPS == 9) ? 3 : (TAPS == 4 ? 2 : 1);
     constexpr int NTS = KS;
-    constexpr int NROW = (TAPS == 9) ? 3 : 1;
+    constexpr int NROW = KS;
+    constexpr bool POLY = (TAPS == 4);
+    static_assert(!POLY || (MODE == CM_NONE && STG == 1 && PHASE == 0), "the polyphase form: raw input, per-pixel staging");
     constexpr bool NEEDP = (MODE == CM_TAN_SILU || MODE == CM_COT_SILU);
     constexpr bool PERS = (PHASE == 3);
     constexpr bool GEN = (STG == 1 || STG == 2);
@@ -494,9 +512,9 @@
 
     const int S = a.stride;
     const int TW = (TAPS == 1 && PHASE == 0 && a.stride == 1 && !a.upsample && !a.zins && (a.Wout & (a.Wout - 1)) == 0)
-                       ? (a.Wout < NT ? a.Wout : NT) : (a.Wout < 32 ? a.Wout : 32);
+                       ? (a.Wout < NT ? a.Wout : NT) : (POLY ? 32 : (a.Wout < 32 ? a.Wout : 32));
     const int TH = NT / TW;
-    const int tiles_x = a.Wout / TW;
+    const int tiles_x = (POLY ? a.Win : a.Wout) / TW;
     int tile_id, cot_id, zid;
     {
         const int ntile = (a.Hout * a.Wout) / NT, ncot = (a.Cout + MT - 1) / MT, Z = PERS ? a.pers_groups : a.B * a.nsplit;
@@ -518,8 +536,15 @@
     }
     int ty0_, tx0_;
     idivmod_small(tile_id, tiles_x, ty0_, tx0_);
-    const int oy0 = __builtin_amdgcn_readfirstlane(ty0_ * TH);
+    int oy0 = __builtin_amdgcn_readfirstlane(ty0_ * TH);
     const int ox0 = __builtin_amdgcn_readfirstlane(tx0_ * TW);
+    int pphase = 0, ppady = 0, ppadx = 0;
+    if constexpr (POLY) {
+        pphase = __builtin_amdgcn_readfirstlane(idiv_small(oy0, a.Hin));
+        oy0 -= pphase * a.Hin;
+        ppady = (a.poly >> (1 + 2 * pphase)) & 1;
+        ppadx = (a.poly >> (2 + 2 * pphase)) & 1;
+    }
     const int co0 = cot_id * MT;
     int zb_, zs_;
     idivmod_small(zid, a.nsplit, zb_, zs_);
@@ -579,6 +604,7 @@
             int hy, hx;
             idivmod_small(pos, halo_w, hy, hx);
             int Y = oy0 * S - a.pad + hy, X = ox0 * S - a.pad + hx;
+            if constexpr (POLY) { Y = oy0 - ppady + hy; X = ox0 - ppadx + hx; }
             if (Y >= 0 && Y < LH && X >= 0 && X < LW) {
                 if (a.upsample) off = (Y >> 1) * a.Win + (X >> 1);
                 else if (a.zins) off = ((Y | X) & 1) ? -1 : (Y >> 1) * a.Win + (X >> 1);
@@ -671,7 +697,8 @@
     const float* scb = (MODE == CM_GN_SILU || MODE == CM_GN || MODE == CM_GN_GELU) ? a.sc + (long)b * a.scsh_bs : nullptr;
     const float* shb = (MODE == CM_GN_SILU || MODE == CM_GN || MODE == CM_GN_GELU) ? a.sh + (long)b * a.scsh_bs : nullptr;
     const int wpitch = (a.Cout + 31) & ~31;
-    const uint4* wg = reinterpret_cast<const uint4*>(a.wb);
+    const uint4* wg = reinterpret_cast<const uint4*>(reinterpret_cast<const unsigned char*>(a.wb) +
+                                                     (POLY ? (size_t)pphase * ((size_t)((a.Cin + BKC - 1) / BKC) * TAPS * wpitch * RB) : (size_t)0));
 
     float hv[NITEM][8];
     float2 pv[NEEDP ? NITEM : 1][8];
@@ -793,7 +820,7 @@
     auto load_regs = [&](float (&hvd)[NITEM][8], int chunk) {
         const int c0 = chunk * BKC;
         if (c0 + BKC <= a.Cin) {
-            if constexpr (TAPS == 9 && !NEEDP) {
+            if constexpr (TAPS != 1 && !NEEDP) {
                 const unsigned lm = pf_live ? 0xffffffffu : 0u;
                 const long pb4 = in_plane * 4;
                 const unsigned char* pk = reinterpret_cast<const unsigned char*>(inb) + (long)c0 * pb4;
@@ -912,7 +939,7 @@
     constexpr int NLO = PR == PR_BF16X3 ? 1 : 0;
     struct Frag { s16x8 ah[TM], al[NLO ? TM : 1], bh[TN], bl[NLO ? TN : 1]; };
     auto load_frag = [&](Frag& f, int row, int tp) {
-        const int tapoff = (TAPS == 9) ? row * halo_w + tp : 0;
+        const int tapoff = (TAPS != 1) ? row * halo_w + tp : 0;
 #pragma unroll
         for (int i = 0; i < TM; ++i) {
             f.ah[i] = *reinterpret_cast<const s16x8*>(Ws + tp * MT * RB + aoff_hi[i]);
@@ -1228,7 +1255,7 @@
             unsigned char* const Hcur = Hsb + (ci & 1) * HBYTES;
             unsigned char* const Hnxt = Hsb + ((ci + 1) & 1) * HBYTES;
             constexpr bool one = (NROW == 1);
-            const int st_part = one ? 0 : (NPART == 2 ? (row == 0 ? 0 : row == 1 ? 1 : -1) : (row == 2 ? 0 : -1));
+            const int st_part = one ? 0 : (NPART == 2 ? (row == 0 ? 0 : row == 1 ? 1 : -1) : (row == NROW - 1 ? 0 : -1));
             const int ld_part = one ? 0 : (NPART == 2 ? (row == 0 ? 1 : row == 1 ? 0 : -1) : (row == 0 ? 0 : -1));
             const int ld_chunk = one ? chunk + 2 : ((NPART == 2 && row == 1) ? chunk + 2 : chunk + 1);
             constexpr bool MIDLOAD = !GEN;
@@ -1272,7 +1299,7 @@
         return;
     }
     LP_STAMP(3);
-    conv_lowp_epilogue<WM, WN, TM, TN, (TAPS == 1 && PHASE == 0) ? (EPI_COT1 | EPI_STATS) : EPI_STATS>(a, acc, smem_b, co0, oy0, ox0, TW, tile_id, b, split);
+    conv_lowp_epilogue<WM, WN, TM, TN, (TAPS == 1 && PHASE == 0) ? (EPI_COT1 | EPI_STATS) : EPI_STATS, POLY>(a, acc, smem_b, co0, oy0, ox0, TW, tile_id, b, split, pphase);
     LP_STAMP(4);
 #undef LP_STAMP
 }
@@ -1313,8 +1340,8 @@
 template <int PR, int TAPS, int WM, int WN, int TM, int TN, int MODE, int STG>
 static void launch_one_b2(const ConvArgs& a, hipStream_t st) {
     constexpr int MT = WM * TM * 32, NT = WN * TN * 32;
-    constexpr int KS = (TAPS == 9) ? 3 : 1;
-    int TW = a.Wout < 32 ? a.Wout : 32;
+    constexpr int KS = (TAPS == 9) ? 3 : (TAPS == 4 ? 2 : 1);
+    int TW = (TAPS == 4 || a.Wout >= 32) ? 32 : a.Wout;
     int TH = NT / TW;
     int halo_w = (TW - 1) * a.stride + KS, halo_h = (TH - 1) * a.stride + KS;
     const int nwb = (TAPS == 9 && STG != 2 && STG != 3) ? 3 : 2;
@@ -1382,6 +1409,12 @@
     hipLaunchKernelGGL(kern, grid, dim3(WM * WN * 64), lds, st, a);
 }
 
+template <int PR>
+void launch_poly_b(const ConvArgs& a, hipStream_t st) {
+    if (a.tile == 2) launch_one_b2<PR, 4, 1, 4, 1, 1, CM_NONE, 1>(a, st);
+    else launch_one_b2<PR, 4, 2, 4, 2, 2, CM_NONE, 1>(a, st);
+}
+
 template <int PR, int TAPS, int MODE>
 void launch_tile_b(const ConvArgs& a, hipStream_t st) {
     switch (a.tile) {
diff --git a/loco-edit_amd/csrc/conv_plan.hip b/loco-edit_amd/csrc/conv_plan.hip
--- a/loco-edit_amd/csrc/conv_plan.hip
+++ b/loco-edit_amd/csrc/conv_plan.hip
@@ -176,6 +176,21 @@
     }
     if ((ns > 1 ? (size_t)ns * a.B * a.Cout * HW : 0) + rec_floats > a.partial_floats) return;
     a.gemm = 1; a.gemm_tm = tm; a.nsplit = ns;
+}
+
+bool conv_polyphase_apply(const ConvEnv& e, ConvArgs& a) {
+    static const bool on = env_int("LOCO_CONV_POLYPHASE", 1) != 0;
+    if (!on || e.prec < 1 || !a.poly_code || !(e.prec == 2 ? a.wph : a.wp) || !(a.upsample || a.zins) || a.stride != 1 ||
+        a.mode != CM_NONE || a.Cin2 > 0 || a.cot_d || a.res || (a.Cin % BKC) != 0 || a.Hin < 32 || a.Win < 32 || (a.Win % 32) != 0 ||
+        a.Hout != 2 * a.Hin || a.Wout != 2 * a.Win)
+        return false;
+    if (conv_bf16_pick_nsplit(a.Cin, a.Cout, a.Hout, a.Wout, a.B, e.chip_share, 9, e.lanes) != 1) return false;
+    const int tile = conv_bf16_pick_tile(a.Cout, a.Hout * a.Wout, a.B, -1);
+    if ((tile != 5 && tile != 2) || (a.Cout % kMT[tile]) != 0 || (a.Hin % (kNT[tile] / 32)) != 0) return false;
+    a.poly = a.poly_code;
+    a.wb = a.wp; a.wh = a.wph;
+    a.upsample = 0; a.zins = 0; a.pad = 0;
+    return true;
 }
 
 void conv_plan_family(ConvArgs& a, int prec) {
@@ -303,7 +318,7 @@
     conv_plan_family(a, e.prec);
     a.tile = tile_for(a, e.prec, -1);
     int split = 1;
-    const int tail = e.prec >= 1 && a.nsplit == 1 && a.B >= 2 && !a.gemm && !a.pers_groups ? tail_split(a, e.partial_floats, &split) : 0;
+    const int tail = e.prec >= 1 && a.nsplit == 1 && a.B >= 2 && !a.gemm && !a.pers_groups && !a.poly ? tail_split(a, e.partial_floats, &split) : 0;
     const bool want = q && q->kind != ST_NONE && e.prec >= 1 && e.fuse_stats;
     if (!tail) {
         p.l[0] = plan_launch(e, q, want, a, 0, a.B, &p.keep_ntile);
@@ -324,7 +339,7 @@
 
 const char* conv_variant_name(const ConvArgs& a, int taps, int prec) {
     static const char* tiles[6] = {"2,2,2,2", "4,1,1,2", "1,4,1,1", "2,2,1,1", "2,2,2,4", "2,4,2,2"};
-    static char names[3][2][6][6][56];
+    static char names[3][3][6][6][56];
     static char others[5][3][6][40];
     const int mode = (a.mode < 0 || a.mode > 5) ? 2 : a.mode;
     const char* other = nullptr;
@@ -343,10 +358,14 @@
     if (t < 0 || t > 5) t = 0;
     int m = mode;
     if (taps != 9 && m != CM_NONE) m = CM_GN;
+    const int stg = taps == 4 ? 1 : -1;
     if (!prec && m == CM_GN_GELU) m = CM_GN_SILU;
-    char* n = names[prec][taps == 9 ? 0 : 1][t][m];
+    char* n = names[prec][taps == 9 ? 0 : (taps == 4 ? 2 : 1)][t][m];
     static const char* kn[3] = {"conv_mfma_f32", "conv_mfma_bf16x3", "conv_mfma_f16"};
-    if (!n[0]) snprintf(n, 56, "%s<%d,%s,%d>", kn[prec], taps, tiles[t], m);
+    if (!n[0]) {
+        if (stg >= 0) snprintf(n, 56, "%s<%d,%s,%d,%d>", kn[prec], taps, tiles[t], m, stg);
+        else snprintf(n, 56, "%s<%d,%s,%d>", kn[prec], taps, tiles[t], m);
+    }
     return n;
 }
 
diff --git a/loco-edit_amd/csrc/conv_polyphase.h b/loco-edit_amd/csrc/conv_polyphase.h
--- /dev/null
+++ b/loco-edit_amd/csrc/conv_polyphase.h
@@ -0,0 +1,47 @@
+#pragma once
+
+namespace loco {
+
+enum : int { PP_UPSAMPLE = 1, PP_ZINS = 2 };
+
+inline int polyphase_axis(int kind, int pad, int phase, int slot[3]) {
+    int d[3], dmin = 2, dmax = -2;
+    for (int t = 0; t < 3; ++t) {
+        const int m = phase - pad + t;
+        slot[t] = -1;
+        if (kind == PP_ZINS && (m & 1)) { d[t] = 9; continue; }
+        d[t] = (m >= 0 ? m : m - 1) / 2;
+        if (d[t] < dmin) dmin = d[t];
+        if (d[t] > dmax) dmax = d[t];
+    }
+    if (dmin < -1 || dmax > 1 || dmax - dmin > 1) return -1;
+    const int p = dmin < 0 ? 1 : 0;
+    for (int t = 0; t < 3; ++t) if (d[t] != 9) slot[t] = d[t] + p;
+    return p;
+}
+
+inline int polyphase_code(int kind, int pad) {
+    if (kind != PP_UPSAMPLE && kind != PP_ZINS) return 0;
+    int code = 1, s[3];
+    for (int ph = 0; ph < 4; ++ph) {
+        const int py = polyphase_axis(kind, pad, ph >> 1, s), px = polyphase_axis(kind, pad, ph & 1, s);
+        if (py < 0 || px < 0) return 0;
+        code |= (py << (1 + 2 * ph)) | (px << (2 + 2 * ph));
+    }
+    return code;
+}
+
+inline bool polyphase_weights(int kind, int pad, const float k9[9], float u16[16]) {
+    for (int ph = 0; ph < 4; ++ph) {
+        int sy[3], sx[3];
+        if (polyphase_axis(kind, pad, ph >> 1, sy) < 0 || polyphase_axis(kind, pad, ph & 1, sx) < 0) return false;
+        double acc[4] = {0.0, 0.0, 0.0, 0.0};
+        for (int ty = 0; ty < 3; ++ty)
+            for (int tx = 0; tx < 3; ++tx)
+                if (sy[ty] >= 0 && sx[tx] >= 0) acc[sy[ty] * 2 + sx[tx]] += (double)k9[ty * 3 + tx];
+        for (int i = 0; i < 4; ++i) u16[ph * 4 + i] = (float)acc[i];
+    }
+    return true;
+}
+
+}
diff --git a/loco-edit_amd/csrc/engine.hip b/loco-edit_amd/csrc/engine.hip
--- a/loco-edit_amd/csrc/engine.hip
+++ b/loco-edit_amd/csrc/engine.hip
@@ -19,6 +19,7 @@
 #endif
 #include "kernels.h"
 #include "program.h"
+#include "conv_polyphase.h"
 #ifdef LOCO_DIAG
 #include "conv_plan_text.h"
 #endif
@@ -44,6 +45,9 @@
     float* wbd = nullptr;
     float* whf = nullptr;
     float* whd = nullptr;
+    float* wpb = nullptr;
+    float* wph = nullptr;
+    int poly_code = 0; bool poly_dgrad = false;
     float* bias = nullptr;
     int cin = 0, cout = 0, taps = 0;
 };
@@ -268,7 +272,7 @@
 }
 
 int make_conv(loco_ctx* c, const std::vector<const HostParam*>& ws, const std::vector<const HostParam*>& bs,
-              ConvP* out, int row_limit = -1) {
+              ConvP* out, int row_limit = -1, int poly_kind = 0, int poly_pad = 1, bool poly_dgrad = false) {
     int cin = (int)ws[0]->shape[1], k = ws[0]->shape.size() > 2 ? (int)ws[0]->shape[2] : 1;
     int taps = ws[0]->shape.size() == 4 ? k * k : k;
     int cout = 0;
@@ -304,6 +308,28 @@
     std::vector<float> hf = build_records_f16(cin, cout, taps, fwd);
     std::vector<float> hd = build_records_f16(cout, cin, taps, dgr);
     if (upload(c, &out->whf, hf) || upload(c, &out->whd, hd)) return -1;
+    out->poly_code = 0;
+    if (poly_kind && taps == 9 && polyphase_code(poly_kind, poly_pad)) {
+        const int nin = poly_dgrad ? cout : cin, nout = poly_dgrad ? cin : cout;
+        std::vector<float> u((size_t)nin * nout * 16);
+        parallel_for(nout, u.size(), [&](int o) {
+            for (int i = 0; i < nin; ++i) {
+                float k9[9];
+                for (int t = 0; t < 9; ++t) k9[t] = poly_dgrad ? dgr(o, i, t) : fwd(o, i, t);
+                polyphase_weights(poly_kind, poly_pad, k9, &u[((size_t)o * nin + i) * 16]);
+            }
+        });
+        std::vector<float> rb, rh;
+        for (int ph = 0; ph < 4; ++ph) {
+            auto get = [&](int o, int i, int t) { return u[((size_t)o * nin + i) * 16 + ph * 4 + t]; };
+            const std::vector<float> b1 = build_records(nin, nout, 4, get), h1 = build_records_f16(nin, nout, 4, get);
+            rb.insert(rb.end(), b1.begin(), b1.end());
+            rh.insert(rh.end(), h1.begin(), h1.end());
+        }
+        if (upload(c, &out->wpb, rb) || upload(c, &out->wph, rh)) return -1;
+        out->poly_code = polyphase_code(poly_kind, poly_pad) | (poly_kind == PP_ZINS ? 512 : 0);
+        out->poly_dgrad = poly_dgrad;
+    }
     return 0;
 }
 int make_conv1(loco_ctx* c, const std::string& name, ConvP* out, int row_limit = -1) {
@@ -414,7 +440,12 @@
                 }
                 break;
             }
-            case OP_DOWN: case OP_UP: if (make_conv1(c, op.pn_conv, &ow.conv)) return -1; break;
+            case OP_DOWN: case OP_UP: {
+                const bool down = op.kind == OP_DOWN;
+                if (make_conv(c, {&c->params[op.pn_conv + ".weight"]}, {&c->params[op.pn_conv + ".bias"]}, &ow.conv, -1,
+                              down ? PP_ZINS : PP_UPSAMPLE, down ? (op.sym_down ? 1 : 2) : 1, down)) return -1;
+                break;
+            }
             case OP_XFMR: {
                 const int C = c->tens[op.in].C, NH = op.heads, CH = C / NH;
                 const std::string b = op.name + ".transformer_blocks.0";
@@ -567,6 +598,13 @@
     }
 }
 
+ConvEnv conv_env(const loco_ctx* c) {
+    ConvEnv e;
+    e.prec = c->prec; e.chip_share = c->chip_share; e.lanes = c->lanes_active; e.lane_s0 = c->lane_s0;
+    e.partial = c->partial; e.partial_floats = c->partial_floats; e.stpart = c->stpart; e.stpart_floats = c->stpart_floats;
+    e.fuse_stats = c->fuse_stats; e.fuse_lin = c->fuse_lin; e.deep1 = c->deep1; e.max_batch = c->cfg.max_batch;
+    return e;
+}
 bool run_conv(loco_ctx* c, const ConvArgs& a0, int taps, hipStream_t st, const StatReq* rq = nullptr,
               const ConvArgs* second = nullptr) {
     const size_t span = (size_t)c->cfg.max_batch * c->prog->per_sample;
@@ -576,10 +614,7 @@
     if (a.mode == CM_GN_SILU && c->cfg.act == ACT_GELU) a.mode = CM_GN_GELU;
     a.in_padded = padded(a.in);
     if (second) { sc = *second; sc.in_padded = padded(sc.in); }
-    ConvEnv e;
-    e.prec = c->prec; e.chip_share = c->chip_share; e.lanes = c->lanes_active; e.lane_s0 = c->lane_s0;
-    e.partial = c->partial; e.partial_floats = c->partial_floats; e.stpart = c->stpart; e.stpart_floats = c->stpart_floats;
-    e.fuse_stats = c->fuse_stats; e.fuse_lin = c->fuse_lin; e.deep1 = c->deep1; e.max_batch = c->cfg.max_batch;
+    const ConvEnv e = conv_env(c);
     StatAsk q;
     if (rq) {
         q.kind = rq->kind; q.norm = rq->n != nullptr; q.prim = rq->prim; q.keep = rq->keep; q.keep_floats = rq->keep_floats;
@@ -610,8 +645,8 @@
         const ConvArgs& x = l.args;
         for (int pi = 0; pi < l.nparts; ++pi) {
             const ConvArgs& y = l.parts[pi];
-            double flops = 2.0 * (y.Cin * taps + y.Cin2) * y.Cout * (double)y.Hout * y.Wout * y.B;
-            if (y.zins) flops *= 0.25;
+            double flops = 2.0 * (y.Cin * (y.poly ? 9 : taps) + y.Cin2) * y.Cout * (double)y.Hout * y.Wout * y.B;
+            if (y.zins || (y.poly & 512)) flops *= 0.25;
             timed(c->prof_on ? conv_variant_name(y, taps, c->prec) : nullptr, flops, y, [&] {
                 if (c->prec == 1) launch_conv_bf16x3(y, taps, st);
                 else if (c->prec == 2) launch_conv_f16(y, taps, st);
@@ -650,6 +685,13 @@
     a.w = dgrad ? p.wd : p.wf;
     a.wb = dgrad ? (const void*)p.wbd : (const void*)p.wbf;
     a.wh = dgrad ? (const void*)p.whd : (const void*)p.whf;
+    const bool poly = p.poly_code && dgrad == p.poly_dgrad;
+    a.poly_code = poly ? p.poly_code : 0; a.wp = poly ? p.wpb : nullptr; a.wph = poly ? p.wph : nullptr;
+}
+inline bool run_resample(loco_ctx* c, const ConvArgs& a0, hipStream_t st, const StatReq* rq = nullptr) {
+    ConvArgs a = a0;
+    const bool poly = conv_polyphase_apply(conv_env(c), a);
+    return run_conv(c, a, poly ? 4 : 9, st, rq);
 }
 
 NormP* consumer_norm(loco_ctx* c, int tid) {
@@ -1162,7 +1204,7 @@
                 if (op.kind == OP_DOWN) { a.stride = 2; a.pad = op.sym_down ? 1 : 0; } else { a.upsample = 1; }
                 a.out = p.T(op.out); a.out_bs = p.bs(); a.Cout = to.C; a.Hout = to.H; a.Wout = to.W; a.B = B;
                 const StatReq rq = next_fwd(op.out);
-                run_conv(c, a, 9, st, &rq);
+                if (op.kind == OP_UP) run_resample(c, a, st, &rq); else run_conv(c, a, 9, st, &rq);
                 break;
             }
             case OP_OUT: {
@@ -1406,7 +1448,7 @@
                 if (op.kind == OP_DOWN) { a.stride = 2; a.pad = op.sym_down ? 1 : 0; } else { a.upsample = 1; }
                 a.out = TT(op.out); a.out_bs = PS; a.Cout = to.C; a.Hout = to.H; a.Wout = to.W; a.B = B;
                 const StatReq rq = next_tan(op.out);
-                run_conv(c, a, 9, st, &rq);
+                if (op.kind == OP_UP) run_resample(c, a, st, &rq); else run_conv(c, a, 9, st, &rq);
                 break;
             }
             case OP_OUT: {
@@ -1481,7 +1523,7 @@
                 a.in = TG(op.out); a.in_bs = PS; a.Cin = to.C; a.Hin = to.H; a.Win = to.W;
                 setw(a, op.conv, true); a.zins = 1; a.pad = op.sym_down ? 1 : 2; a.accumulate = op.in_is_skip ? 1 : 0;
                 a.out = TG(op.in); a.out_bs = PS; a.Cout = ti.C; a.Hout = ti.H; a.Wout = ti.W; a.B = B;
-                run_conv(c, a, 9, st);
+                run_resample(c, a, st);
                 break;
             }
             case OP_RES: {
@@ -2401,7 +2443,9 @@
     if (finalize_params(c)) return -3;
     hipStream_t st = (hipStream_t)stream;
     const long HW = (long)H * W;
-    const long in_e = (long)cin * HW, out_e = (long)cout * HW;
+    const int rs = (taps == 9 && getenv("LOCO_BENCH_RESAMPLE")) ? atoi(getenv("LOCO_BENCH_RESAMPLE")) : 0;
+    if (rs < 0 || rs > 3 || (rs && ((H | W) & 1))) { c->err = "bench_conv: bad LOCO_BENCH_RESAMPLE"; return -2; }
+    const long in_e = (long)cin * (rs ? HW / 4 : HW), out_e = (long)cout * HW;
     if ((in_e + out_e) * B > (long)c->cfg.max_batch * c->prog->per_sample || 2 * in_e > (long)c->prog->per_sample ||
         in_e > c->prog->sx_total) { c->err = "bench_conv: shape exceeds the arenas"; return -2; }
     float* in = c->arenaT;
@@ -2413,12 +2457,13 @@
     launch_fill_random(reinterpret_cast<float*>(c->sxcache), 2 * in_e, 3u, zs, st);
     launch_fill_random(c->statsP, c->prog->stats_per_sample, 4u, 1.0f, st);
     launch_fill_random(c->statsT, c->prog->stats_per_sample * B, 5u, 0.01f, st);
-    size_t wfl = (size_t)((cin + 15) / 16) * 16 * taps * ((cout + 31) & ~31);
+    const int wtaps = rs ? 16 : taps;
+    size_t wfl = (size_t)((cin + 15) / 16) * 16 * wtaps * ((cout + 31) & ~31);
     if (wfl * 2 > c->partial_floats) { c->err = "bench_conv: weights exceed workspace"; return -2; }
     float* wf = c->partial + c->partial_floats - wfl * 2;
     launch_fill_random(wf, (long)wfl * 2, 6u, 0.05f * zw, st);
     if (c->prec == 1) {
-        const long nrec = (long)((cin + 15) / 16) * taps * ((cout + 31) & ~31);
+        const long nrec = (long)((cin + 15) / 16) * wtaps * ((cout + 31) & ~31);
         hipLaunchKernelGGL(diag_fill_records, dim3((unsigned)((nrec + 255) / 256)), dim3(256), 0, st,
                            reinterpret_cast<unsigned char*>(wf), nrec, (cout + 31) & ~31, 7u, 0.05f * zw);
     }
@@ -2442,6 +2487,11 @@
         a.cot_d = out + out_e * B; a.cot_d_bs = out_e; a.cot_sx = c->sxcache; a.cot_tc = c->statsT; a.cot_tc_bs = c->prog->stats_per_sample;
     }
     if (getenv("LOCO_BENCH_ACC") && atoi(getenv("LOCO_BENCH_ACC"))) a.accumulate = 1;
+    if (rs) {
+        a.Hin = H / 2; a.Win = W / 2; a.upsample = rs == 1; a.zins = rs != 1; a.pad = rs == 2 ? 2 : 1;
+        a.poly_code = polyphase_code(rs == 1 ? PP_UPSAMPLE : PP_ZINS, a.pad) | (rs == 1 ? 0 : 512); a.wp = wf; a.wph = wf;
+        if (conv_polyphase_apply(conv_env(c), a)) { taps = 4; a.taps = 4; }
+    }
     conv_plan_family(a, c->prec);
     if (const char* e = getenv("LOCO_DUAL_WHATIF")) a.no_deep = atoi(e);
     ConvArgs parts[2];
@@ -2535,7 +2585,8 @@
     HostParam w2 = host_param(d->Cin2 > 0 ? d->w2 : nullptr, {d->Cout, d->Cin2 > 0 ? d->Cin2 : 1, 1, 1}), wb2 = host_param(nullptr, {d->Cout});
     ConvP cp, cp2;
     float *bias_d = nullptr, *bias2nd_d = nullptr, *small = nullptr;
-    int rc = make_conv(c, {&w}, {&wb0}, &cp);
+    const int pad_run = d->pad >= 0 ? d->pad : taps == 1 ? 0 : d->zins ? 2 : d->stride == 2 ? 0 : 1;
+    int rc = make_conv(c, {&w}, {&wb0}, &cp, -1, taps != 9 ? 0 : d->upsample ? PP_UPSAMPLE : d->zins ? PP_ZINS : 0, pad_run, d->transposed != 0);
     if (!rc && d->Cin2 > 0) rc = make_conv(c, {&w2}, {&wb2}, &cp2);
     if (!rc && d->bias) rc = upload(c, &bias_d, std::vector<float>(d->bias, d->bias + d->Cout));
     if (!rc && d->Cin2 > 0 && d->bias2nd) rc = upload(c, &bias2nd_d, std::vector<float>(d->bias2nd, d->bias2nd + d->Cout));
@@ -2554,7 +2605,7 @@
     a.bias2 = d->bias2; a.bias2_bs = d->Cout;
     a.res = d->res; a.res_bs = out_e; a.res_scale = d->res_scale;
     a.mode = d->mode; a.stride = d->stride; a.upsample = d->upsample; a.zins = d->zins; a.accumulate = d->accumulate;
-    a.pad = d->pad >= 0 ? d->pad : taps == 1 ? 0 : d->zins ? 2 : d->stride == 2 ? 0 : 1;
+    a.pad = pad_run;
     a.sc = d->sc; a.sh = d->sh; a.scsh_bs = 0; a.cpg = d->cpg;
     if (lin) {
         if (he == hipSuccess) he = copy(c->arenaP, d->prim, in_e);
@@ -2594,7 +2645,8 @@
     const int act0 = c->cfg.act;
     if (d->mode == CM_GN_GELU) c->cfg.act = ACT_GELU;
     c->plan_log = &text;
-    const bool rode = run_conv(c, a, taps, st, nullptr, d->Cin2 > 0 ? &n2 : nullptr);
+    const bool rode = (taps == 9 && (a.upsample || a.zins) && d->Cin2 <= 0) ? run_resample(c, a, st)
+                                                                            : run_conv(c, a, taps, st, nullptr, d->Cin2 > 0 ? &n2 : nullptr);
     c->plan_log = nullptr;
     c->cfg.act = act0;
     he = hipGetLastError();
diff --git a/loco-edit_amd/csrc/kernels.h b/loco-edit_amd/csrc/kernels.h
--- a/loco-edit_amd/csrc/kernels.h
+++ b/loco-edit_amd/csrc/kernels.h
@@ -77,6 +77,9 @@
     size_t partial_floats;
     int pers_groups;
     int tile, pair;
+    int poly, poly_code;
+    const void* wp;
+    const void* wph;
 };
 
 void launch_conv(const ConvArgs& a, int taps, hipStream_t st);
@@ -130,6 +133,8 @@
 ConvPlan plan_conv(const ConvEnv& env, const ConvArgs& a, int taps, const StatAsk* ask, const ConvArgs* shortcut);
 void conv_plan_family(ConvArgs& a, int prec);
 int conv_plan_parts(ConvArgs& a, int prec, int tile_override, ConvArgs parts[2]);
+
+bool conv_polyphase_apply(const ConvEnv& env, ConvArgs& a);
 
 int conv_bf16_tile_couts(const ConvArgs& a);
 const char* conv_variant_name(const ConvArgs& a, int taps, int prec);
```
